# Fierykev/RayTraceBVH

Measured on AMD Instinct MI355X. Metric: Mrays/s primary+1-bounce (BASELINE.json's metric, on its config C5: 3840x2160, the 1/2/4/8-GPU config; the metric's @1080p config C3 is the line c3_1080p); BVH build Mtris/s under build, higher is better.
Workload: dtype f32; 1 GPU; C5: synthetic 10M tris (seed 0x5EED0005, box 100x100x50), 3840x2160, primary+1 bounce; width=3840, height=2160, bounces=1, triangles=10000000, parallelism=single GPU

## Files before the change

include/rtbvh.h:

```cpp
#ifndef RTBVH_H
#define RTBVH_H

#include <stddef.h>
#include <stdint.h>

#ifdef __cplusplus
extern "C" {
#endif

#define RTBVH_ABI_VERSION 8

typedef enum {
    RTBVH_OK = 0,
    RTBVH_ERR_INVALID_ARG = 1,
    RTBVH_ERR_HIP = 2,
    RTBVH_ERR_OOM = 3,
    RTBVH_ERR_NOT_READY = 4,
    RTBVH_ERR_STACK_OVERFLOW = 5,
    RTBVH_ERR_IO = 6,
    RTBVH_ERR_NO_DEVICE = 7,
    RTBVH_ERR_COMM = 8
} rtbvh_status;


// ... 7 lines not shown
    float ambient[4];
    float diffuse[4];
    float specular[4];
    float shininess;
    float optical_density;
    float alpha;
    uint32_t specularb;
    int32_t tex_num;
} rtbvh_material;

typedef struct {
    uint32_t parent, child_l, child_r, code;
    float bb_min[3], bb_max[3];
    uint32_t index;
} rtbvh_node;

typedef struct {
    float intensity;
    float origin[3], direction[3], inv_direction[3];
    float color[4];
} rtbvh_ray_present;

typedef struct {
    uint32_t width, height;
    const uint8_t* rgba8;
} rtbvh_texture;

enum {
    RTBVH_MORTON_CPUTESTS = 0,
    RTBVH_MORTON_HLSL = 1
};
enum {
    RTBVH_DELTA_CLZ64 = 0,
    RTBVH_DELTA_CPUTESTS = 1
};
enum {
    RTBVH_FLAG_TIMING = 1u << 0,
    RTBVH_FLAG_COUNT_VISITS = 1u << 1,
    RTBVH_FLAG_REFRACT_RECORDS = 1u << 2,
    RTBVH_FLAG_SORT_BOUNCE = 1u << 3,
    RTBVH_FLAG_NEAREST_FIRST = 1u << 4,
    RTBVH_FLAG_PACKET_PRIMARY = 1u << 5,
    RTBVH_FLAG_REFILL_BOUNCE = 1u << 6,
    RTBVH_FLAG_WIDE_BVH = 1u << 7,
    RTBVH_FLAG_AUTO_WALK = 1u << 8,
    RTBVH_FLAG_BINNED_PRIMARY = 1u << 9,
    RTBVH_FLAG_CERTIFIED = 1u << 10,
    RTBVH_FLAG_MULTI_KERNEL_BUILD = 1u << 16,
    RTBVH_FLAG_SPLIT_SHIFT = 17,
    RTBVH_FLAG_GRAPH = 1u << 20
};

typedef struct {
    int32_t device;
    uint32_t morton_mode;
    uint32_t delta_mode;
    uint32_t flags;
    float scene_bb_min[3];
    float scene_bb_max[3];
    void* stream;
    uint32_t stack_limit;
    uint32_t reserved;
} rtbvh_config;

typedef struct {
    uint32_t num_tris, num_nodes, width, height;
    uint64_t primary_rays, bounce_rays;
    uint64_t internal_visits[2], leaf_visits[2], hits[2];
    uint64_t textured_hits, stack_overflows;
    uint32_t timed_builds, timed_traces;
    float ms_build, ms_trace;
    float ms_stage[8];
    uint64_t trav_wave_steps, trav_mixed_steps, trav_active_lanes;
    uint64_t trav_max_steps, trav_steps_log2[32];
    uint64_t graph_captures;
    uint32_t walk_flags;
    uint32_t walk_state;
    uint64_t packet_steps[2];
    uint64_t cert_traces, redo_total;
    uint64_t bin_entries[2];
    uint64_t redo_rays[2];
    uint64_t trav_longest;
    uint64_t redo_deferred;
} rtbvh_stats;
typedef struct rtbvh_ctx rtbvh_ctx;

void rtbvh_config_default(rtbvh_config* cfg);
rtbvh_status rtbvh_create(const rtbvh_config* cfg, rtbvh_ctx** out);
void rtbvh_destroy(rtbvh_ctx* ctx);
const char* rtbvh_last_error(const rtbvh_ctx* ctx);
int rtbvh_abi_version(void);
uint32_t rtbvh_stats_size(void);

rtbvh_status rtbvh_set_scene(rtbvh_ctx* ctx, const rtbvh_vertex* verts, uint32_t nverts,
                             const uint32_t* indices, uint32_t nidx, const uint32_t* mat_idx,
                             const rtbvh_material* mats, uint32_t nmats,
                             const rtbvh_texture* textures, uint32_t ntex);
rtbvh_status rtbvh_set_camera(rtbvh_ctx* ctx, const float wvp[16], const float wv[16]);

rtbvh_status rtbvh_build(rtbvh_ctx* ctx);
rtbvh_status rtbvh_build_async(rtbvh_ctx* ctx);
rtbvh_status rtbvh_trace(rtbvh_ctx* ctx, uint32_t width, uint32_t height, uint32_t bounces);
rtbvh_status rtbvh_trace_async(rtbvh_ctx* ctx, uint32_t width, uint32_t height, uint32_t bounces);
rtbvh_status rtbvh_compute_bvh(rtbvh_ctx* ctx, uint32_t width, uint32_t height, uint32_t bounces);
rtbvh_status rtbvh_trace_band_async(rtbvh_ctx* ctx, uint32_t width, uint32_t height, uint32_t bounces,
                                    uint32_t rank, uint32_t nranks, float* dev_out, void* stream);
uint32_t rtbvh_band_rows(uint32_t height, uint32_t rank, uint32_t nranks);
uint32_t rtbvh_deal_bands(uint32_t height, uint32_t rank, uint32_t nranks, uint32_t root_share, uint32_t* bands,
                          uint32_t capacity);
uint32_t rtbvh_deal_rows(uint32_t height, uint32_t rank, uint32_t nranks, uint32_t root_share);
rtbvh_status rtbvh_set_band_deal(rtbvh_ctx* ctx, uint32_t root_share);
rtbvh_status rtbvh_verify_walk(rtbvh_ctx* ctx, uint32_t width, uint32_t height, uint32_t bounces,
                               uint64_t* differing_pixels);
rtbvh_status rtbvh_assemble_bands(rtbvh_ctx* ctx, uint32_t width, uint32_t height, uint32_t nranks,
                                  const float* dev_bands, uint32_t stride_rows, float* dev_frame, void* stream);

#define RTBVH_COMM_ID_BYTES 128
rtbvh_status rtbvh_comm_unique_id(uint8_t id[RTBVH_COMM_ID_BYTES]);
rtbvh_status rtbvh_comm_init(rtbvh_ctx* ctx, uint32_t nranks, uint32_t rank, const uint8_t id[RTBVH_COMM_ID_BYTES],
                             void** comm);
rtbvh_status rtbvh_comm_destroy(void* comm);
rtbvh_status rtbvh_trace_tiles(rtbvh_ctx* ctx, uint32_t width, uint32_t height, uint32_t bounces, uint32_t rank,
                               uint32_t nranks, void* comm);
rtbvh_status rtbvh_synchronize(rtbvh_ctx* ctx);

rtbvh_status rtbvh_update_vertices_async(rtbvh_ctx* ctx, const float* dev_positions, uint32_t pos_stride,
                                         const float* dev_normals, uint32_t nrm_stride,
                                         uint32_t first, uint32_t count, void* stream);
rtbvh_status rtbvh_update_vertices_host(rtbvh_ctx* ctx, const float* positions, uint32_t pos_stride,
                                        const float* normals, uint32_t nrm_stride,
                                        uint32_t first, uint32_t count);
rtbvh_status rtbvh_refit_async(rtbvh_ctx* ctx);
rtbvh_status rtbvh_refit(rtbvh_ctx* ctx);

typedef struct {
    float origin[3];
    float t_max;
    float direction[3];
    uint32_t reserved;
} rtbvh_ray;
typedef struct {
    float t, u, v;
    uint32_t tri;
} rtbvh_hit;
enum {
    RTBVH_QUERY_CLOSEST = 0,
    RTBVH_QUERY_ANY = 1u << 0,
    RTBVH_QUERY_SORT = 1u << 1,
    RTBVH_QUERY_COUNT = 1u << 2,
    RTBVH_QUERY_CERTIFIED = 1u << 8
};
rtbvh_status rtbvh_query_async(rtbvh_ctx* ctx, const rtbvh_ray* dev_rays, uint64_t n, rtbvh_hit* dev_hits,
                               uint32_t mode, void* stream);
rtbvh_status rtbvh_query_host(rtbvh_ctx* ctx, const rtbvh_ray* rays, uint64_t n, rtbvh_hit* hits, uint32_t mode);
rtbvh_status rtbvh_query_counts(rtbvh_ctx* ctx, uint64_t out[4]);
rtbvh_status rtbvh_query_walk_counts(rtbvh_ctx* ctx, uint64_t out[4]);

typedef struct {
    float point[3];
    float max_dist2;
} rtbvh_point;
typedef struct {
    float point[3];
    float dist2;
    float u, v;
    uint32_t tri;
// ... 58 lines not shown
                               rtbvh_hit* dev_hits, uint32_t mode, void* stream);
rtbvh_status rtbvh_khits_host(rtbvh_ctx* ctx, const rtbvh_ray* rays, uint64_t n, uint32_t k, rtbvh_hit* hits,
                              uint32_t mode);
rtbvh_status rtbvh_khits_counts(rtbvh_ctx* ctx, uint64_t out[4]);

enum {
    RTBVH_COLLIDE_COUNT = 1u << 2,
    RTBVH_COLLIDE_TRIANGLE = 1u << 3,
    RTBVH_COLLIDE_SIZES = 1u << 4,
    RTBVH_COLLIDE_FILL = 1u << 5,
    RTBVH_COLLIDE_SYMMETRIC = 1u << 6
};
rtbvh_status rtbvh_collide_async(rtbvh_ctx* ctx, uint64_t* dev_offsets, uint32_t* dev_ids, uint64_t capacity,
                                 uint32_t mode, void* stream);
rtbvh_status rtbvh_collide_host(rtbvh_ctx* ctx, uint64_t* offsets, uint32_t* ids, uint64_t capacity, uint32_t mode);
rtbvh_status rtbvh_collide_counts(rtbvh_ctx* ctx, uint64_t out[4]);

typedef struct {
    float v0[3];
    uint32_t reserved0;
    float v1[3];
    uint32_t reserved1;
    float v2[3];
    uint32_t reserved2;
} rtbvh_tri;
enum {
    RTBVH_CROSS_SORT = 1u << 1,
    RTBVH_CROSS_COUNT = 1u << 2,
    RTBVH_CROSS_SIZES = 1u << 4,
    RTBVH_CROSS_FILL = 1u << 5
};
rtbvh_status rtbvh_cross_async(rtbvh_ctx* ctx, const rtbvh_tri* dev_tris, uint64_t n, uint64_t* dev_offsets,
                               uint32_t* dev_ids, uint64_t capacity, uint32_t mode, void* stream);
rtbvh_status rtbvh_cross_host(rtbvh_ctx* ctx, const rtbvh_tri* tris, uint64_t n, uint64_t* offsets, uint32_t* ids,
                              uint64_t capacity, uint32_t mode);
rtbvh_status rtbvh_cross_first_async(rtbvh_ctx* ctx, const rtbvh_tri* dev_tris, uint64_t n, uint32_t* dev_first,
                                     uint32_t mode, void* stream);
rtbvh_status rtbvh_cross_first_host(rtbvh_ctx* ctx, const rtbvh_tri* tris, uint64_t n, uint32_t* first,
                                    uint32_t mode);
rtbvh_status rtbvh_cross_counts(rtbvh_ctx* ctx, uint64_t out[4]);

typedef struct {
    float lo[3];
    uint32_t reserved0;
    float hi[3];
    uint32_t reserved1;
} rtbvh_box;
enum {
    RTBVH_OVERLAP_SORT = 1u << 1,
    RTBVH_OVERLAP_COUNT = 1u << 2,
    RTBVH_OVERLAP_TRIANGLE = 1u << 3,
    RTBVH_OVERLAP_SIZES = 1u << 4,
    RTBVH_OVERLAP_FILL = 1u << 5
};
rtbvh_status rtbvh_overlap_async(rtbvh_ctx* ctx, const rtbvh_box* dev_boxes, uint64_t n, uint64_t* dev_offsets,
                                 uint32_t* dev_ids, uint64_t capacity, uint32_t mode, void* stream);
rtbvh_status rtbvh_overlap_host(rtbvh_ctx* ctx, const rtbvh_box* boxes, uint64_t n, uint64_t* offsets,
                                uint32_t* ids, uint64_t capacity, uint32_t mode);
rtbvh_status rtbvh_overlap_counts(rtbvh_ctx* ctx, uint64_t out[4]);

typedef struct {
    float point[3]; float dist2;
    float u, v; uint32_t tri;
    uint32_t flags;
} rtbvh_signed;
enum { RTBVH_SIGNED_SORT = 1u << 1, RTBVH_SIGNED_COUNT = 1u << 2,
       RTBVH_SIGNED_VOTE3 = 1u << 3,
       RTBVH_SIGNED_INSIDE_ONLY = 1u << 4
        };
rtbvh_status rtbvh_signed_async(rtbvh_ctx* ctx, const rtbvh_point* dev_points, uint64_t n, rtbvh_signed* dev_out,
                                uint32_t mode, void* stream);
rtbvh_status rtbvh_signed_host(rtbvh_ctx* ctx, const rtbvh_point* points, uint64_t n, rtbvh_signed* out,
                               uint32_t mode);
rtbvh_status rtbvh_signed_counts(rtbvh_ctx* ctx, uint64_t out[4]);

rtbvh_status rtbvh_read_framebuffer(rtbvh_ctx* ctx, float* rgba);
rtbvh_status rtbvh_read_intensity(rtbvh_ctx* ctx, float* intensity);
rtbvh_status rtbvh_present(rtbvh_ctx* ctx, uint8_t* rgba8);
rtbvh_status rtbvh_save_bmp(const char* path, const uint8_t* rgba8, uint32_t width, uint32_t height);
const float* rtbvh_framebuffer_device(rtbvh_ctx* ctx);
rtbvh_status rtbvh_read_bvh(rtbvh_ctx* ctx, rtbvh_node* out, uint32_t capacity);
rtbvh_status rtbvh_read_wide(rtbvh_ctx* ctx, uint32_t* records, uint64_t capacity);
rtbvh_status rtbvh_read_qnodes(rtbvh_ctx* ctx, uint32_t* nodes, uint64_t capacity);
rtbvh_status rtbvh_read_morton(rtbvh_ctx* ctx, uint32_t* codes);
rtbvh_status rtbvh_read_sorted(rtbvh_ctx* ctx, uint32_t* sorted_codes, uint32_t* tri_ids);
rtbvh_status rtbvh_read_rays(rtbvh_ctx* ctx, rtbvh_ray_present* reflect_out, rtbvh_ray_present* refract_out);
rtbvh_status rtbvh_get_stats(rtbvh_ctx* ctx, rtbvh_stats* out);
rtbvh_status rtbvh_reset_stats(rtbvh_ctx* ctx);
rtbvh_status rtbvh_set_flags(rtbvh_ctx* ctx, uint32_t flags);
uint64_t rtbvh_bin_builds(rtbvh_ctx* ctx);
uint32_t rtbvh_bin_sets(rtbvh_ctx* ctx);

rtbvh_status rtbvh_sort_pairs_async(rtbvh_ctx* ctx, uint32_t* keys_in, uint32_t* vals_in,
                                    uint32_t* keys_out, uint32_t* vals_out, uint32_t n,
                                    uint32_t key_bits);
rtbvh_status rtbvh_sort_pairs_host(rtbvh_ctx* ctx, const uint32_t* keys, const uint32_t* vals,
                                   uint32_t* keys_out, uint32_t* vals_out, uint32_t n, uint32_t key_bits);
rtbvh_status rtbvh_build_from_codes(rtbvh_ctx* ctx, const uint32_t* sorted_codes,
                                    const float* leaf_boxes, uint32_t n, rtbvh_node* out);

rtbvh_status rtbvh_texture_load_bmp(const char* path, rtbvh_texture* out);
rtbvh_status rtbvh_texture_load_jpeg(const char* path, rtbvh_texture* out);
rtbvh_status rtbvh_texture_decode_jpeg(const uint8_t* data, size_t size, rtbvh_texture* out);
rtbvh_status rtbvh_texture_load(const char* path, rtbvh_texture* out);
void rtbvh_texture_free(rtbvh_texture* tex);
void rtbvh_srgb_table(float out[256]);
typedef struct rtbvh_scene rtbvh_scene;
rtbvh_status rtbvh_scene_load_obj(const char* path, rtbvh_scene** out);
rtbvh_status rtbvh_scene_synthetic(uint64_t seed, uint32_t ntris, const float half_extent[3],
                                   rtbvh_scene** out);
void rtbvh_scene_free(rtbvh_scene* s);
uint32_t rtbvh_scene_num_vertices(const rtbvh_scene* s);
uint32_t rtbvh_scene_num_indices(const rtbvh_scene* s);
uint32_t rtbvh_scene_num_materials(const rtbvh_scene* s);
uint32_t rtbvh_scene_num_textures(const rtbvh_scene* s);
const rtbvh_vertex* rtbvh_scene_vertices(const rtbvh_scene* s);
const uint32_t* rtbvh_scene_indices(const rtbvh_scene* s);
const uint32_t* rtbvh_scene_mat_indices(const rtbvh_scene* s);
const rtbvh_material* rtbvh_scene_materials(const rtbvh_scene* s);
const char* rtbvh_scene_texture_path(const rtbvh_scene* s, uint32_t k);
rtbvh_status rtbvh_set_scene_obj(rtbvh_ctx* ctx, const rtbvh_scene* s, const rtbvh_texture* textures,
                                 uint32_t ntex);
void rtbvh_camera_reference(uint32_t width, uint32_t height, float wvp[16], float wv[16]);
void rtbvh_camera_look(const float eye[3], uint32_t width, uint32_t height, float wvp[16], float wv[16]);
void rtbvh_camera_orbit(float eye[3], uint32_t key);

#ifdef __cplusplus
}
#endif
#endif
```

raytracebvh_amd/_lib.py:

```python
from __future__ import annotations

import ctypes
import os

import numpy as np

HERE = os.path.dirname(os.path.abspath(__file__))
LIB_PATH = os.environ.get("RTBVH_LIB") or os.path.join(HERE, "librtbvh.so")

OK, ERR_INVALID_ARG, ERR_HIP, ERR_OOM, ERR_NOT_READY, ERR_STACK_OVERFLOW, ERR_IO, ERR_NO_DEVICE = range(8)
MORTON_CPUTESTS, MORTON_HLSL = 0, 1
DELTA_CLZ64, DELTA_CPUTESTS = 0, 1
FLAG_TIMING, FLAG_COUNT_VISITS, FLAG_REFRACT_RECORDS, FLAG_SORT_BOUNCE, FLAG_NEAREST_FIRST = 1, 2, 4, 8, 16
FLAG_PACKET_PRIMARY = 1 << 5
FLAG_REFILL_BOUNCE = 1 << 6
FLAG_WIDE_BVH = 1 << 7
FLAG_BINNED_PRIMARY = 1 << 9
FLAG_CERTIFIED = 1 << 10
FLAG_MULTI_KERNEL_BUILD = 1 << 16
FLAG_AUTO_WALK = 1 << 8
FLAG_SPLIT_SHIFT = 17
FLAG_GRAPH = 1 << 20

EXPORTS = [
    "rtbvh_config_default", "rtbvh_create", "rtbvh_destroy", "rtbvh_last_error", "rtbvh_abi_version", "rtbvh_stats_size",
    "rtbvh_set_scene", "rtbvh_set_camera", "rtbvh_build", "rtbvh_build_async", "rtbvh_trace",
    "rtbvh_trace_async", "rtbvh_compute_bvh", "rtbvh_trace_band_async", "rtbvh_band_rows", "rtbvh_verify_walk",
    "rtbvh_deal_bands", "rtbvh_deal_rows", "rtbvh_set_band_deal",
    "rtbvh_synchronize", "rtbvh_read_framebuffer", "rtbvh_read_intensity", "rtbvh_framebuffer_device",
    "rtbvh_read_bvh", "rtbvh_read_wide", "rtbvh_read_qnodes", "rtbvh_read_morton", "rtbvh_read_sorted", "rtbvh_read_rays", "rtbvh_get_stats",
    "rtbvh_reset_stats", "rtbvh_set_flags", "rtbvh_bin_builds", "rtbvh_bin_sets",
    "rtbvh_sort_pairs_async", "rtbvh_sort_pairs_host", "rtbvh_build_from_codes", "rtbvh_scene_load_obj",
    "rtbvh_scene_synthetic", "rtbvh_scene_free", "rtbvh_scene_num_vertices", "rtbvh_scene_num_indices",
    "rtbvh_scene_num_materials", "rtbvh_scene_num_textures", "rtbvh_scene_vertices", "rtbvh_scene_indices",
    "rtbvh_scene_mat_indices", "rtbvh_scene_materials", "rtbvh_scene_texture_path", "rtbvh_set_scene_obj",
    "rtbvh_camera_reference", "rtbvh_camera_look", "rtbvh_camera_orbit", "rtbvh_texture_load_bmp", "rtbvh_texture_load_jpeg", "rtbvh_texture_decode_jpeg",
    "rtbvh_texture_load", "rtbvh_texture_free", "rtbvh_srgb_table",
    "rtbvh_present", "rtbvh_save_bmp", "rtbvh_assemble_bands", "rtbvh_comm_unique_id", "rtbvh_comm_init",
    "rtbvh_comm_destroy", "rtbvh_trace_tiles",
    "rtbvh_query_async", "rtbvh_query_host", "rtbvh_query_counts", "rtbvh_query_walk_counts",
    "rtbvh_nearest_async", "rtbvh_nearest_host", "rtbvh_nearest_counts",
    "rtbvh_within_async", "rtbvh_within_host", "rtbvh_within_counts",
    "rtbvh_knn_async", "rtbvh_knn_host", "rtbvh_knn_counts",
    "rtbvh_allhits_async", "rtbvh_allhits_host", "rtbvh_allhits_counts",
    "rtbvh_overlap_async", "rtbvh_overlap_host", "rtbvh_overlap_counts",
    "rtbvh_signed_async", "rtbvh_signed_host", "rtbvh_signed_counts",
    "rtbvh_khits_async", "rtbvh_khits_host", "rtbvh_khits_counts",
    "rtbvh_collide_async", "rtbvh_collide_host", "rtbvh_collide_counts",
    "rtbvh_cross_async", "rtbvh_cross_host", "rtbvh_cross_first_async", "rtbvh_cross_first_host", "rtbvh_cross_counts",
    "rtbvh_update_vertices_async", "rtbvh_update_vertices_host", "rtbvh_refit_async", "rtbvh_refit",
]
COMM_ID_BYTES = 128

NODE_DTYPE = np.dtype([("parent", "<u4"), ("child_l", "<u4"), ("child_r", "<u4"), ("code", "<u4"),
                       ("bb_min", "<f4", (3,)), ("bb_max", "<f4", (3,)), ("index", "<u4")])
MATERIAL_DTYPE = np.dtype([("ambient", "<f4", (4,)), ("diffuse", "<f4", (4,)), ("specular", "<f4", (4,)),
                           ("shininess", "<f4"), ("optical_density", "<f4"), ("alpha", "<f4"),
                           ("specularb", "<u4"), ("tex_num", "<i4")])
assert NODE_DTYPE.itemsize == 44 and MATERIAL_DTYPE.itemsize == 68
RAY_DTYPE = np.dtype([("origin", "<f4", (3,)), ("t_max", "<f4"), ("direction", "<f4", (3,)), ("reserved", "<u4")])
HIT_DTYPE = np.dtype([("t", "<f4"), ("u", "<f4"), ("v", "<f4"), ("tri", "<u4")])
assert RAY_DTYPE.itemsize == 32 and HIT_DTYPE.itemsize == 16
QUERY_CLOSEST, QUERY_ANY, QUERY_SORT, QUERY_COUNT = 0, 1, 2, 4
QUERY_CERTIFIED = 1 << 8
POINT_DTYPE = np.dtype([("point", "<f4", (3,)), ("max_dist2", "<f4")])
NEAREST_DTYPE = np.dtype([("point", "<f4", (3,)), ("dist2", "<f4"), ("u", "<f4"), ("v", "<f4"), ("tri", "<u4"),
                          ("reserved", "<u4")])
assert POINT_DTYPE.itemsize == 16 and NEAREST_DTYPE.itemsize == 32
NEAREST_SORT, NEAREST_COUNT = 2, 4
PAIR_DTYPE = np.dtype([("tri", "<u4"), ("dist2", "<f4")])
assert PAIR_DTYPE.itemsize == 8
WITHIN_SORT, WITHIN_COUNT, WITHIN_SIZES, WITHIN_FILL = 2, 4, 16, 32
KNN_SORT, KNN_COUNT = 2, 4
KNN_MAX_K = 32
ALLHITS_SORT, ALLHITS_COUNT, ALLHITS_BY_T, ALLHITS_SIZES, ALLHITS_FILL = 2, 4, 8, 16, 32
BOX_DTYPE = np.dtype([("lo", "<f4", (3,)), ("reserved0", "<u4"), ("hi", "<f4", (3,)), ("reserved1", "<u4")])
assert BOX_DTYPE.itemsize == 32
OVERLAP_SORT, OVERLAP_COUNT, OVERLAP_TRIANGLE, OVERLAP_SIZES, OVERLAP_FILL = 2, 4, 8, 16, 32
SIGNED_DTYPE = np.dtype([("point", "<f4", (3,)), ("dist2", "<f4"), ("u", "<f4"), ("v", "<f4"), ("tri", "<u4"),
                         ("flags", "<u4")])
assert SIGNED_DTYPE.itemsize == 32
SIGNED_SORT, SIGNED_COUNT, SIGNED_VOTE3, SIGNED_INSIDE_ONLY = 2, 4, 8, 16
KHITS_SORT, KHITS_COUNT = 2, 4
KHITS_MAX_K = 16
COLLIDE_COUNT, COLLIDE_TRIANGLE, COLLIDE_SIZES, COLLIDE_FILL, COLLIDE_SYMMETRIC = 4, 8, 16, 32, 64
TRI_DTYPE = np.dtype([("v0", "<f4", (3,)), ("reserved0", "<u4"), ("v1", "<f4", (3,)), ("reserved1", "<u4"),
                      ("v2", "<f4", (3,)), ("reserved2", "<u4")])
assert TRI_DTYPE.itemsize == 48
CROSS_SORT, CROSS_COUNT, CROSS_SIZES, CROSS_FILL = 2, 4, 16, 32


class Config(ctypes.Structure):
    _fields_ = [("device", ctypes.c_int32), ("morton_mode", ctypes.c_uint32), ("delta_mode", ctypes.c_uint32),
                ("flags", ctypes.c_uint32), ("scene_bb_min", ctypes.c_float * 3),
                ("scene_bb_max", ctypes.c_float * 3), ("stream", ctypes.c_void_p),
                ("stack_limit", ctypes.c_uint32), ("reserved", ctypes.c_uint32)]


class Ray(ctypes.Structure):
    _fields_ = [("origin", ctypes.c_float * 3), ("t_max", ctypes.c_float), ("direction", ctypes.c_float * 3),
                ("reserved", ctypes.c_uint32)]


class Hit(ctypes.Structure):
    _fields_ = [("t", ctypes.c_float), ("u", ctypes.c_float), ("v", ctypes.c_float), ("tri", ctypes.c_uint32)]


class Point(ctypes.Structure):
    _fields_ = [("point", ctypes.c_float * 3), ("max_dist2", ctypes.c_float)]


class Nearest(ctypes.Structure):
    _fields_ = [("point", ctypes.c_float * 3), ("dist2", ctypes.c_float), ("u", ctypes.c_float), ("v", ctypes.c_float),
                ("tri", ctypes.c_uint32), ("reserved", ctypes.c_uint32)]


class Texture(ctypes.Structure):
    _fields_ = [("width", ctypes.c_uint32), ("height", ctypes.c_uint32), ("rgba8", ctypes.c_void_p)]


class Stats(ctypes.Structure):
    _fields_ = [("num_tris", ctypes.c_uint32), ("num_nodes", ctypes.c_uint32), ("width", ctypes.c_uint32),
                ("height", ctypes.c_uint32), ("primary_rays", ctypes.c_uint64), ("bounce_rays", ctypes.c_uint64),
                ("internal_visits", ctypes.c_uint64 * 2), ("leaf_visits", ctypes.c_uint64 * 2),
                ("hits", ctypes.c_uint64 * 2), ("textured_hits", ctypes.c_uint64),
                ("stack_overflows", ctypes.c_uint64), ("timed_builds", ctypes.c_uint32),
                ("timed_traces", ctypes.c_uint32), ("ms_build", ctypes.c_float), ("ms_trace", ctypes.c_float),
                ("ms_stage", ctypes.c_float * 8), ("trav_wave_steps", ctypes.c_uint64),
                ("trav_mixed_steps", ctypes.c_uint64), ("trav_active_lanes", ctypes.c_uint64),
                ("trav_max_steps", ctypes.c_uint64), ("trav_steps_log2", ctypes.c_uint64 * 32),
                ("graph_captures", ctypes.c_uint64), ("walk_flags", ctypes.c_uint32),
                ("walk_state", ctypes.c_uint32), ("packet_steps", ctypes.c_uint64 * 2),
                ("cert_traces", ctypes.c_uint64), ("redo_total", ctypes.c_uint64),
                ("bin_entries", ctypes.c_uint64 * 2), ("redo_rays", ctypes.c_uint64 * 2),
                ("trav_longest", ctypes.c_uint64), ("redo_deferred", ctypes.c_uint64)]

    def as_dict(self) -> dict:
        d = {}
        for k, _ in self._fields_:
            v = getattr(self, k)
            d[k] = list(v) if hasattr(v, "__len__") else v
        return d


class RtbvhError(RuntimeError):
    def __init__(self, status: int, msg: str):
        super().__init__(f"rtbvh status {status}: {msg}")
        self.status = status


_lib = None


def lib() -> ctypes.CDLL:
    global _lib
    if _lib is not None:
        return _lib
    if not os.path.exists(LIB_PATH):
        raise ImportError(f"{LIB_PATH} is not built: run `python -c 'import __graft_entry__ as g; g.build()'` "
                          "(there is no CPU fallback for the HIP path)")
    try:
        import torch
    except ImportError:
        pass
    L = ctypes.CDLL(LIB_PATH)
    vp, u32, u64, i32 = ctypes.c_void_p, ctypes.c_uint32, ctypes.c_uint64, ctypes.c_int
    sig = {
        "rtbvh_config_default": (None, [ctypes.POINTER(Config)]),
        "rtbvh_create": (i32, [ctypes.POINTER(Config), ctypes.POINTER(vp)]),
        "rtbvh_destroy": (None, [vp]),
        "rtbvh_last_error": (ctypes.c_char_p, [vp]),
        "rtbvh_abi_version": (i32, []),
        "rtbvh_stats_size": (ctypes.c_uint32, []),
        "rtbvh_set_scene": (i32, [vp, vp, u32, vp, u32, vp, vp, u32, vp, u32]),
        "rtbvh_set_camera": (i32, [vp, vp, vp]),
        "rtbvh_build": (i32, [vp]),
        "rtbvh_build_async": (i32, [vp]),
        "rtbvh_trace": (i32, [vp, u32, u32, u32]),
        "rtbvh_trace_async": (i32, [vp, u32, u32, u32]),
        "rtbvh_compute_bvh": (i32, [vp, u32, u32, u32]),
        "rtbvh_trace_band_async": (i32, [vp, u32, u32, u32, u32, u32, vp, vp]),
        "rtbvh_band_rows": (u32, [u32, u32, u32]),
        "rtbvh_deal_bands": (u32, [u32, u32, u32, u32, vp, u32]),
        "rtbvh_deal_rows": (u32, [u32, u32, u32, u32]),
        "rtbvh_set_band_deal": (i32, [vp, u32]),
        "rtbvh_verify_walk": (i32, [vp, u32, u32, u32, ctypes.POINTER(u64)]),
        "rtbvh_assemble_bands": (i32, [vp, u32, u32, u32, vp, u32, vp, vp]),
        "rtbvh_comm_unique_id": (i32, [vp]),
        "rtbvh_comm_init": (i32, [vp, u32, u32, vp, ctypes.POINTER(vp)]),
        "rtbvh_comm_destroy": (i32, [vp]),
        "rtbvh_trace_tiles": (i32, [vp, u32, u32, u32, u32, u32, vp]),
        "rtbvh_synchronize": (i32, [vp]),
        "rtbvh_read_framebuffer": (i32, [vp, vp]),
        "rtbvh_read_intensity": (i32, [vp, vp]),
        "rtbvh_framebuffer_device": (vp, [vp]),
        "rtbvh_read_bvh": (i32, [vp, vp, u32]),
        "rtbvh_read_morton": (i32, [vp, vp]),
        "rtbvh_read_wide": (i32, [vp, vp, ctypes.c_uint64]),
        "rtbvh_read_qnodes": (i32, [vp, vp, ctypes.c_uint64]),
        "rtbvh_read_sorted": (i32, [vp, vp, vp]),
        "rtbvh_read_rays": (i32, [vp, vp, vp]),
        "rtbvh_get_stats": (i32, [vp, ctypes.POINTER(Stats)]),
        "rtbvh_reset_stats": (i32, [vp]),
        "rtbvh_set_flags": (i32, [vp, u32]),
        "rtbvh_bin_builds": (u64, [vp]),
        "rtbvh_bin_sets": (u32, [vp]),
        "rtbvh_sort_pairs_async": (i32, [vp, vp, vp, vp, vp, u32, u32]),
        "rtbvh_sort_pairs_host": (i32, [vp, vp, vp, vp, vp, u32, u32]),
        "rtbvh_build_from_codes": (i32, [vp, vp, vp, u32, vp]),
        "rtbvh_scene_load_obj": (i32, [ctypes.c_char_p, ctypes.POINTER(vp)]),
        "rtbvh_scene_synthetic": (i32, [u64, u32, vp, ctypes.POINTER(vp)]),
        "rtbvh_scene_free": (None, [vp]),
        "rtbvh_scene_num_vertices": (u32, [vp]),
        "rtbvh_scene_num_indices": (u32, [vp]),
        "rtbvh_scene_num_materials": (u32, [vp]),
        "rtbvh_scene_num_textures": (u32, [vp]),
        "rtbvh_scene_vertices": (vp, [vp]),
        "rtbvh_scene_indices": (vp, [vp]),
        "rtbvh_scene_mat_indices": (vp, [vp]),
        "rtbvh_scene_materials": (vp, [vp]),
        "rtbvh_scene_texture_path": (ctypes.c_char_p, [vp, u32]),
        "rtbvh_set_scene_obj": (i32, [vp, vp, vp, u32]),
        "rtbvh_camera_reference": (None, [u32, u32, vp, vp]),
        "rtbvh_camera_look": (None, [vp, u32, u32, vp, vp]),
        "rtbvh_camera_orbit": (None, [vp, u32]),
        "rtbvh_texture_load_bmp": (i32, [ctypes.c_char_p, vp]),
        "rtbvh_texture_load_jpeg": (i32, [ctypes.c_char_p, vp]),
        "rtbvh_texture_decode_jpeg": (i32, [vp, ctypes.c_size_t, vp]),
        "rtbvh_texture_load": (i32, [ctypes.c_char_p, vp]),
        "rtbvh_texture_free": (None, [vp]),
        "rtbvh_srgb_table": (None, [vp]),
        "rtbvh_present": (i32, [vp, vp]),
        "rtbvh_save_bmp": (i32, [ctypes.c_char_p, vp, u32, u32]),
        "rtbvh_query_async": (i32, [vp, vp, u64, vp, u32, vp]),
        "rtbvh_query_host": (i32, [vp, vp, u64, vp, u32]),
        "rtbvh_query_counts": (i32, [vp, vp]),
        "rtbvh_query_walk_counts": (i32, [vp, vp]),
        "rtbvh_nearest_async": (i32, [vp, vp, u64, vp, u32, vp]),
        "rtbvh_nearest_host": (i32, [vp, vp, u64, vp, u32]),
        "rtbvh_nearest_counts": (i32, [vp, vp]),
        "rtbvh_within_async": (i32, [vp, vp, u64, vp, vp, u64, u32, vp]),
        "rtbvh_within_host": (i32, [vp, vp, u64, vp, vp, u64, u32]),
        "rtbvh_within_counts": (i32, [vp, vp]),
        "rtbvh_knn_async": (i32, [vp, vp, u64, u32, vp, u32, vp]),
        "rtbvh_knn_host": (i32, [vp, vp, u64, u32, vp, u32]),
        "rtbvh_knn_counts": (i32, [vp, vp]),
        "rtbvh_signed_async": (i32, [vp, vp, u64, vp, u32, vp]),
        "rtbvh_signed_host": (i32, [vp, vp, u64, vp, u32]),
        "rtbvh_signed_counts": (i32, [vp, vp]),
        "rtbvh_khits_async": (i32, [vp, vp, u64, u32, vp, u32, vp]),
        "rtbvh_khits_host": (i32, [vp, vp, u64, u32, vp, u32]),
        "rtbvh_khits_counts": (i32, [vp, vp]),
        "rtbvh_allhits_async": (i32, [vp, vp, u64, vp, vp, u64, u32, vp]),
        "rtbvh_allhits_host": (i32, [vp, vp, u64, vp, vp, u64, u32]),
        "rtbvh_allhits_counts": (i32, [vp, vp]),
        "rtbvh_overlap_async": (i32, [vp, vp, u64, vp, vp, u64, u32, vp]),
        "rtbvh_overlap_host": (i32, [vp, vp, u64, vp, vp, u64, u32]),
        "rtbvh_overlap_counts": (i32, [vp, vp]),
        "rtbvh_collide_async": (i32, [vp, vp, vp, u64, u32, vp]),
        "rtbvh_collide_host": (i32, [vp, vp, vp, u64, u32]),
        "rtbvh_collide_counts": (i32, [vp, vp]),
        "rtbvh_cross_async": (i32, [vp, vp, u64, vp, vp, u64, u32, vp]),
        "rtbvh_cross_host": (i32, [vp, vp, u64, vp, vp, u64, u32]),
        "rtbvh_cross_first_async": (i32, [vp, vp, u64, vp, u32, vp]),
        "rtbvh_cross_first_host": (i32, [vp, vp, u64, vp, u32]),
        "rtbvh_cross_counts": (i32, [vp, vp]),
        "rtbvh_update_vertices_async": (i32, [vp, vp, u32, vp, u32, u32, u32, vp]),
        "rtbvh_update_vertices_host": (i32, [vp, vp, u32, vp, u32, u32, u32]),
        "rtbvh_refit_async": (i32, [vp]),
        "rtbvh_refit": (i32, [vp]),
    }
    for name, (res, args) in sig.items():
        f = getattr(L, name)
        f.restype = res
        f.argtypes = args
    _lib = L
    return L


def ptr(a: np.ndarray):
    if a is None:
        return None
# ... 9 lines not shown
```

raytracebvh_amd/csrc/api.hip:

```cpp
#include <dlfcn.h>
#include <rccl/rccl.h>

#include <algorithm>
#include <cstdio>
#include <cstring>
#include <deque>
#include <new>
#include <string>
#include <type_traits>
#include <utility>
#include <vector>

#include "../../include/rtbvh.h"
#include "rtbvh_internal.h"

using namespace rtbvh;

#ifndef RTBVH_MAXSPLIT
#define RTBVH_MAXSPLIT 4
#endif

template <typename H, void (*Del)(H)>
struct Owner {
    H h{};
// ... 92 lines not shown
    DevBuf<float2> hit;
    Grown<uint32_t> redo, defer;
    PbBufs pb;
    Grown<unsigned long long> pbkeys;
    uint32_t* qcount = nullptr;
    uint32_t* next = nullptr;
    unsigned long long* counters = nullptr;
    unsigned long long* ovf = nullptr;
};

struct LastTrace {
    bool traced = false;
    uint32_t W = 0, H = 0, bounces = 0, rank = 0, nranks = 1;
    uint32_t nsplit = 1;
    uint32_t slot = 0;
    size_t rec_P = 0;
    uint32_t walk = 0;
    uint32_t walk_state = 0;
    bool cert = false;
    bool frame_here = false;
    bool intensity_here = false;
};

struct rtbvh_ctx {
    rtbvh_config cfg{};
    Stream own_stream, side;
    static constexpr uint32_t MAXSPLIT = RTBVH_MAXSPLIT;
    TraceSet sets[MAXSPLIT];
    hipStream_t stream = nullptr;
    std::string err;

    uint32_t V = 0, T = 0, nmat = 0;
    DevBuf<float4> d_opos;
    DevBuf<float> d_verts;
    DevBuf<uint32_t> d_idx, d_matidx;
    DevBuf<Mat> d_mats;
    float wvp[16], wv[16];
    DevBuf<float> d_cam;
    bool cam_dirty = false;
    bool have_scene = false, have_camera = false;
    Tree tree;
    Event ev_update;
    bool update_pending = false;
    bool stale = false;

    uint32_t cap_T = 0;
    DevBuf<uint32_t> d_codes, d_ids, d_ka, d_va, d_kb, d_vb, d_sort_scratch;
    DevBuf<float4> d_tclip, d_leaf;
    Grown<float4> d_band;
    DevBuf<Inner> d_inner;
    DevBuf<uint4> d_topo;
    DevBuf<Inner> d_rec;
    DevBuf<QNode> d_qnode;
    DevBuf<uint4> d_lfp;
    DevBuf<uint32_t> d_texels;
    DevBuf<uint4> d_texinfo;
    DevBuf<float> d_srgb;
    uint32_t ntex = 0;
    Grown<float> d_refl_rec;
    Grown<float> d_refr_rec;
    DevBuf<uint32_t> d_pleaf, d_pint, d_cnt;
    DevBuf<uint32_t> d_xlist, d_xcnt;
    DevBuf<uint32_t> d_qlate;
    DevBuf<unsigned long long> d_ovf;
    Pinned<unsigned long long> h_ovf;
    unsigned long long ovf_seen = 0;
    DevBuf<float> d_bounds, d_rootbox, d_zpart;
    Event ev_leaf, ev_prim;
    DevBuf<float> d_nbox;
    bool tail_pending = false;
    bool leaf_pending = false;
    SortResult sorted{nullptr, nullptr};

    size_t cap_P = 0;
    DevBuf<float4> d_color;
    DevBuf<float> d_intensity;
    DevBuf<uint32_t> d_bkin, d_bvin, d_bka, d_bva, d_bkb, d_bvb, d_bscratch;
    DevBuf<uint32_t> d_qcount;
    DevBuf<uint32_t> d_next;
    DevBuf<unsigned long long> d_counters;
    size_t cap_split = 0;
    Event ev_fork;
    uint64_t bins_epoch = 1;
    uint64_t bin_builds = 0;
    bool knob_bins_reuse = true;
    LastTrace last;

    static constexpr int RING = 32;
    Event evb[RING][6];
    Event evt[RING][5];
    bool evt_trav[RING] = {};
    uint32_t n_builds = 0, n_traces = 0;
    Event ev_built;
    bool slots_used = false;
    hipGraph_t graph = nullptr;
    hipGraphExec_t graph_exec = nullptr;
    uint64_t graph_key[5] = {};
    bool capturing = false;
    uint64_t graph_captures = 0;
    LastTrace graph_trace;
    Tree graph_tree;
    uint64_t cert_traces = 0;
    uint64_t small_key = 0;
    uint32_t small_flags = 0;
    bool small_packet = false;
    Event ev_small[2];
    uint32_t knob_bounce_blocks = 0;
    bool knob_overlap = false, knob_side_priority = true, knob_keep_records = false, knob_no_early_shade = false,
         knob_no_small_tiles = false;
    uint32_t root_share = 16;
    struct DealTab {
        uint32_t H, nranks, share;
        DevBuf<uint32_t> d;
        std::vector<uint32_t> off;
        Pinned<uint32_t> h;
        Event ready;
    };
    std::deque<DealTab> deals;
    static constexpr size_t MAX_DEALS = 8;
    DevBuf<uint32_t> d_qscratch;
    Grown<uint32_t> d_qsort;
    Grown<uint32_t> d_qsort_scratch;
    Grown<uint32_t> d_qredo;
    Grown<unsigned long long> d_qscan;
    Grown<uint32_t> d_qorder;
    Event ev_query;
    bool query_busy = false;
    bool query_ovf = false;
    bool query_counted = false;
    uint64_t query_fallback = 0;
    bool nearest_counted = false;
    bool within_counted = false;
    bool allhits_counted = false;
    bool overlap_counted = false;
    bool knn_counted = false;
    bool signed_counted = false;
    bool khits_counted = false;
    bool collide_counted = false;
    bool cross_counted = false;
};

namespace {

std::string g_create_error;

rtbvh_status fail(rtbvh_ctx* c, rtbvh_status st, const std::string& msg) {
    if (c) c->err = msg;
    else g_create_error = msg;
    return st;
}

#define HIPC(ctx, expr)                                                                          \
    do {                                                                                         \
        hipError_t _e = (expr);                                                                  \
        if (_e != hipSuccess)                                                                    \
            return fail(ctx, _e == hipErrorOutOfMemory ? RTBVH_ERR_OOM : RTBVH_ERR_HIP,          \
                        std::string(#expr) + ": " + hipGetErrorString(_e));                      \
    } while (0)
#define TRY(expr)                                      \
    do {                                               \
        if (rtbvh_status _st = (expr)) return _st;     \
    } while (0)

void drop_graph(rtbvh_ctx* c) {
    if (c->graph_exec) (void)hipGraphExecDestroy(c->graph_exec);
    if (c->graph) (void)hipGraphDestroy(c->graph);
// ... 399 lines not shown
struct Rccl {
    bool ok = false;
    std::string err;
    ncclResult_t (*GetUniqueId)(ncclUniqueId*) = nullptr;
    ncclResult_t (*CommInitRank)(ncclComm_t*, int, ncclUniqueId, int) = nullptr;
    ncclResult_t (*CommDestroy)(ncclComm_t) = nullptr;
    ncclResult_t (*Send)(const void*, size_t, ncclDataType_t, int, ncclComm_t, hipStream_t) = nullptr;
    ncclResult_t (*Recv)(void*, size_t, ncclDataType_t, int, ncclComm_t, hipStream_t) = nullptr;
    ncclResult_t (*GroupStart)() = nullptr;
    ncclResult_t (*GroupEnd)() = nullptr;
    const char* (*GetErrorString)(ncclResult_t) = nullptr;
};
const Rccl& rccl() {
    static const Rccl lib = [] {
        Rccl r;
        void* h = dlopen("librccl.so.1", RTLD_NOW | RTLD_GLOBAL);
        if (!h) {
            const char* e = dlerror();
            r.err = std::string("RCCL not available: ") + (e ? e : "dlopen(librccl.so.1) failed");
            return r;
        }
        bool all = true;
        auto sym = [&](auto& f, const char* name) {
            f = reinterpret_cast<std::remove_reference_t<decltype(f)>>(dlsym(h, name));
            if (!f) all = false;
        };
        sym(r.GetUniqueId, "ncclGetUniqueId");
        sym(r.CommInitRank, "ncclCommInitRank");
        sym(r.CommDestroy, "ncclCommDestroy");
        sym(r.Send, "ncclSend");
        sym(r.Recv, "ncclRecv");
        sym(r.GroupStart, "ncclGroupStart");
        sym(r.GroupEnd, "ncclGroupEnd");
        sym(r.GetErrorString, "ncclGetErrorString");
        r.ok = all;
        if (!all) r.err = "RCCL: librccl.so.1 lacks a required symbol";
        return r;
    }();
    return lib;
}

rtbvh_status sync_camera(rtbvh_ctx* c, hipStream_t s) {
    if (!c->cam_dirty) return RTBVH_OK;
    TRY(wait_slots(c, c->stream));
    launch_set_camera(c->wvp, c->wv, c->d_cam, c->stream);
    HIPC(c, hipGetLastError());
    c->cam_dirty = false;
    return order_after_context(c, s);
}

rtbvh_status before_tree_write(rtbvh_ctx* c, hipStream_t s) {
    TRY(wait_slots(c, s));
    TRY(wait_queries(c, s));
    TRY(wait_update(c, s));
    TRY(sync_camera(c, s));
    c->bins_epoch++;
    return RTBVH_OK;
}

struct TailGuard {
    rtbvh_ctx* c;
    bool pending;
    void run() {
        if (pending) launch_refit_tail(build_args(c), c->stream);
        pending = false;
    }
    ~TailGuard() { run(); }
};

struct WalkPlan {
    hipStream_t s;
    uint32_t slot, bounces;
    bool cert;
    bool leaf_pending;
    bool count, timing, records;
    Walks wk;
    PrimaryKind pkind;
    Form nodes;
    uint32_t P, rows;
    uint32_t nsplit, Pg;
    uint32_t tblocks;
    uint32_t ntx, nty;
    bool inflight, fuse_tail, overlap, small_tiles, early_shade;
    uint32_t bset;
    bool fill_bins;
};

WalkPlan plan_walks(const rtbvh_ctx* c, const TraceArgs& a, uint32_t bounces, hipStream_t s, uint32_t slot,
                    uint32_t flags, bool cert, bool timed, bool tail_pending, bool leaf_pending) {
    WalkPlan p{s, slot, bounces, cert, leaf_pending};
    p.bset = slot;
    p.count = (c->cfg.flags & RTBVH_FLAG_COUNT_VISITS) != 0;
    p.timing = timed && (c->cfg.flags & RTBVH_FLAG_TIMING) != 0 && s == c->stream && !c->capturing;
    p.wk = choose_walks(flags);
    p.records = (flags & RTBVH_FLAG_REFRACT_RECORDS) != 0;
    p.P = a.W * deal_rows(a.H, a.rank, a.nranks, c->root_share);
    p.rows = p.P / a.W;
#ifndef RTBVH_BOUNCE_GRID
#define RTBVH_BOUNCE_GRID (256 * BOUNCE_WAVES)
#endif
    p.inflight = slot != 0;
    for (uint32_t k = 1; k < rtbvh_ctx::MAXSPLIT && !p.inflight && !c->capturing; k++)
        p.inflight = c->sets[k].busy && hipEventQuery(c->sets[k].done) == hipErrorNotReady;
    p.tblocks = p.P < (1u << 22) ? (!p.inflight ? 1536 : p.P < (3u << 20) ? 512 : 1024) : RTBVH_BOUNCE_GRID;
    if (c->knob_bounce_blocks) p.tblocks = c->knob_bounce_blocks;
    const bool binned = p.wk.primary == PrimaryKind::BINNED;
    p.pkind = binned && (a.W > 32768u || a.H > 32768u)
                  ? (cert ? PrimaryKind::LANE_REFERENCE : PrimaryKind::PACKET_WIDE)
                  : p.wk.primary;
    p.nsplit = trace_split(c);
    if (p.wk.sort || a.my_bands < p.nsplit || slot || c->slots_used || binned) p.nsplit = 1;
    p.Pg = p.nsplit == 1 ? p.P : a.W * 8 * ((a.my_bands + p.nsplit - 1) / p.nsplit);
    p.nodes = cert ? NBOX : RECORDS;
    p.fuse_tail = tail_pending && p.pkind == PrimaryKind::BINNED && s == c->stream && slot == 0 && p.rows > 0 &&
                  (c->tree.valid & p.nodes);
    p.overlap = p.pkind == PrimaryKind::BINNED && leaf_pending && s == c->stream && slot == 0 && p.nsplit == 1;
    p.ntx = pb_tiles_x(a.W);
    p.nty = pb_tiles_y(p.rows);
    p.small_tiles = !p.inflight && !c->knob_no_small_tiles && (size_t)a.W * p.rows < (3u << 19);
    p.early_shade = cert && !p.inflight && !c->knob_no_early_shade;
    return p;
}

rtbvh_status prepare_walks(rtbvh_ctx* c, WalkPlan& p, TraceArgs& a, const rtbvh_ctx::DealTab* deal, TailGuard& tail) {
    hipStream_t s = p.s;
    TraceSet& mine = c->sets[p.slot];
    const size_t P = p.P;
    if (p.records) {
        if (!(c->d_refl_rec.has(14 * P) && c->d_refr_rec.has(14 * P))) {
            drop_graph(c);
            HIPC(c, c->d_refl_rec.reserve(14 * P));
            HIPC(c, c->d_refr_rec.reserve(14 * P));
        }
        a.refl_rec = c->d_refl_rec;
        a.refr_rec = c->d_refr_rec;
    }
    if (!p.fuse_tail && tail.pending) {
        tail.run();
        TRY(order_after_context(c, s));
    }
    TRY(ensure_form(c, p.nodes, s));
    a.nb = p.cert;
    TRY(ensure_split_capacity(c, p.slot ? p.slot + 1 : p.nsplit, p.Pg));
    if (p.bounces > 0 && p.wk.refill && p.wk.bounce == BounceWalk::WIDE_QUANTIZED) TRY(ensure_form(c, QNODES, s));
    if (p.pkind == PrimaryKind::PACKET_REFERENCE || p.pkind == PrimaryKind::PACKET_NEAREST ||
        p.pkind == PrimaryKind::PACKET_WIDE)
        TRY(ensure_form(c, PSEUDO, s));
    if (p.cert && p.bounces > 0 && !mine.defer.has(P)) {
        drop_graph(c);
        HIPC(c, mine.defer.reserve(P));
        if (hipMemsetAsync(mine.defer, 0, sizeof(uint32_t) * P, c->stream) != hipSuccess) {
            mine.defer.reset();
            return fail(c, RTBVH_ERR_HIP, "clearing the deferred-ray list failed");
        }
        TRY(order_after_context(c, s));
    }
    if (p.cert && !mine.redo.has(P)) {
        drop_graph(c);
        HIPC(c, mine.redo.reserve(P));
    }
    if (p.pkind != PrimaryKind::BINNED || p.rows == 0) return RTBVH_OK;
    const size_t px = (size_t)a.W * p.rows;
    if (pb_keys_used() && !mine.pbkeys.has(px)) {
        drop_graph(c);
        HIPC(c, mine.pbkeys.reserve(px));
    }
// ... 25 lines not shown
    return RTBVH_OK;
}

rtbvh_status launch_walks(rtbvh_ctx* c, const WalkPlan& p, const TraceArgs& a, TailGuard& tail) {
    hipStream_t s = p.s;
    TraceSet& mine = c->sets[p.slot];
    const uint32_t bounces = p.bounces, nsplit = p.nsplit;
    const bool count = p.count, cert = p.cert, refill = p.wk.refill;
    Event* ev = c->evt[c->n_traces % rtbvh_ctx::RING];
    ZeroList z{};
    z.ptr[0] = reinterpret_cast<uint32_t*>(mine.counters);
    z.words[0] = 64 * 2;
    z.ptr[1] = mine.qcount;
    z.words[1] = 32 * nsplit;
    if (refill && bounces) {
        z.ptr[2] = mine.next;
        z.words[2] = (size_t)NEXT_WORDS * nsplit;
    }
    if (p.fill_bins) {
        z.ptr[3] = mine.pb.off;
        z.words[3] = (size_t)p.ntx * p.nty * PB_NZ + 1;
        if (a.nranks > 1) {
            z.ptr[4] = mine.pb.list;
            z.words[4] = (size_t)PB_LISTS * PB_LIST_STRIDE;
        }
    }
    hipStream_t sp = s;
    if (p.overlap) {
        sp = c->side;
        HIPC(c, hipStreamWaitEvent(sp, c->ev_leaf, 0));
    }
    launch_zero(z, sp);
    if (p.timing) HIPC(c, hipEventRecord(ev[0], sp));
    if (nsplit > 1) HIPC(c, hipEventRecord(c->ev_fork, s));
    for (uint32_t g = 0; g < nsplit; g++) {
        TraceSet& set = c->sets[p.slot + g];
        hipStream_t sg = g ? set.chain : s;
        if (g) HIPC(c, hipStreamWaitEvent(sg, c->ev_fork, 0));
        TraceArgs ag = a;
        ag.band0 = g;
        ag.bstep = nsplit;
        ag.pb_list = p.fill_bins && a.nranks > 1 ? mine.pb.list : nullptr;
        RayQ* q[2] = {set.q[0], set.q[1]};
        uint32_t* qc = set.qcount;
        const bool tg = p.timing && g == 0;
        if (p.pkind == PrimaryKind::BINNED) {
            PbBufs& pbb = c->sets[p.bset].pb;
            const PrimBins pb{pbb.off, pbb.cur, pbb.bins, mine.pbkeys, pbb.sums, pbb.cap_bins, p.ntx, p.nty};
            if (p.rows) {
                const BuildArgs ba = build_args(c);
                const Redo rd{mine.redo, &qc[16]};
                if (p.fill_bins) {
                    launch_pb_bins(ag, pb, p.rows, true, sp, p.fuse_tail ? &ba : nullptr);
                    c->bin_builds++;
                    if (c->knob_bins_reuse && !c->capturing) {
                        if (!pbb.filled) HIPC(c, hipEventCreateWithFlags(pbb.filled.out(), hipEventDisableTiming));
                        HIPC(c, hipEventRecord(pbb.filled, sp));
                        pbb.valid = true;
                    }
                }
                launch_pb_raster(ag, pb, p.rows, q[0], &qc[0], count, bounces > 0, sp, cert ? &rd : nullptr,
                                 p.small_tiles);
                if (p.fuse_tail) tail.pending = false;
            }
            if (p.overlap) {
                HIPC(c, hipEventRecord(c->ev_prim, sp));
                HIPC(c, hipStreamWaitEvent(sg, c->ev_prim, 0));
            }
            if (p.rows) launch_pb_gate(ag, pb, q[0], &qc[0], count, bounces > 0, sg, cert);
        } else
            launch_primary(ag, q[0], &qc[0], count, bounces > 0, p.pkind, sg);
        if (tg) HIPC(c, hipEventRecord(ev[1], sg));
        for (uint32_t b = 0; b < bounces; b++) {
            const uint32_t* perm = nullptr;
            if (p.wk.sort) {
                launch_bounce_keys(q[b & 1], &qc[b], c->d_rootbox, p.P, c->d_bkin, c->d_bvin, sg);
                perm = radix_sort_pairs(c->d_bkin, c->d_bvin, c->d_bka, c->d_bva, c->d_bkb, c->d_bvb, p.P, 30,
                                        c->d_bscratch, sg).vals;
            }
            if (refill) {
                if (tg && b == 0) HIPC(c, hipEventRecord(ev[3], sg));
                uint32_t* nxb = set.next + (size_t)NEXT_SEGS * NEXT_STRIDE * b;
                const BounceShade es{q[(b + 1) & 1], &qc[b + 1], b + 1 < bounces, mine.redo, &qc[17 + b], p.Pg};
                launch_bounce_traverse(ag, q[b & 1], &qc[b], perm, count, p.wk.bounce, set.hit, nxb, p.tblocks, sg, cert,
                                       mine.defer, p.early_shade ? &es : nullptr);
                if (tg && b == 0) HIPC(c, hipEventRecord(ev[4], sg));
                const Redo rd{mine.redo, &qc[17 + b], mine.defer, nxb};
                launch_bounce_shade(ag, q[b & 1], &qc[b], set.hit, q[(b + 1) & 1], &qc[b + 1], count, b + 1 < bounces,
                                    p.Pg, sg, cert ? &rd : nullptr);
            } else
                launch_bounce(ag, q[b & 1], &qc[b], perm, q[(b + 1) & 1], &qc[b + 1], count, b + 1 < bounces,
                              p.wk.nearest, sg);
        }
        if (g) {
            HIPC(c, hipEventRecord(set.join, sg));
            HIPC(c, hipStreamWaitEvent(s, set.join, 0));
        }
    }
    HIPC(c, hipMemcpyAsync(mine.ovf, c->d_ovf, sizeof(unsigned long long), hipMemcpyDeviceToHost, s));
    if (p.timing) {
        HIPC(c, hipEventRecord(ev[2], s));
        c->evt_trav[c->n_traces % rtbvh_ctx::RING] = refill && bounces > 0;
        c->n_traces++;
    }
    return RTBVH_OK;
}

rtbvh_status enqueue_walks(rtbvh_ctx* c, uint32_t W, uint32_t H, uint32_t bounces, uint32_t rank, uint32_t nranks,
                           float4* color, float* inten, hipStream_t s, uint32_t slot, uint32_t flags, bool timed,
                           uint32_t walk_state, bool cert = false) {
    const bool leaf_pending = c->leaf_pending;
    c->leaf_pending = false;
    TailGuard tail{c, c->tail_pending};
    c->tail_pending = false;
    if (!c->tree.built) return fail(c, RTBVH_ERR_NOT_READY, "trace before build");
    if (c->stale) return fail_stale(c, "trace");
    if (W == 0 || H == 0 || nranks == 0 || rank >= nranks || bounces > 14)
        return fail(c, RTBVH_ERR_INVALID_ARG, "bad trace dimensions");
    TRY(ensure_trace_capacity(c, (size_t)W * H));
    if (!color) color = c->d_color;
    TraceArgs a = trace_args(c, W, H, rank, nranks, color, inten);
    const rtbvh_ctx::DealTab* deal = nullptr;
    TRY(get_deal(c, H, nranks, &deal, s));
    if (deal) {
        a.my_bands = deal->off[rank + 1] - deal->off[rank];
        a.band_list = deal->d + deal->off[rank];
        a.band_slots = deal->d + (H + 7) / 8;
    }
    a.counters = c->sets[slot].counters;
    if ((flags & RTBVH_FLAG_REFRACT_RECORDS) && slot)
        return fail(c, RTBVH_ERR_INVALID_ARG, "ray records are traced on the context stream only");
    WalkPlan p = plan_walks(c, a, bounces, s, slot, flags, cert, timed, tail.pending, leaf_pending);
    TRY(prepare_walks(c, p, a, deal, tail));
    TRY(launch_walks(c, p, a, tail));
    const bool frame_here = color == c->d_color && nranks == 1;
    c->last = LastTrace{true, W, H, bounces, rank, nranks, p.nsplit, slot, p.records ? p.P : 0, flags & WALK_FLAGS,
                        walk_state, cert, frame_here, frame_here && inten != nullptr};
    return check_launch(c, "trace kernels");
}

struct TracePlan {
    uint32_t flags;
    bool cert;
    uint32_t state;
};
TracePlan plan_trace(const rtbvh_ctx* c, uint32_t f) {
    if (!(f & (RTBVH_FLAG_AUTO_WALK | RTBVH_FLAG_CERTIFIED))) return TracePlan{f, false, 0};
    const uint32_t ref = f & ~WALK_FLAGS;
    const bool limited = c->cfg.stack_limit != 0 && c->cfg.stack_limit < (uint32_t)STACK_SIZE;
    const bool want = (f & RTBVH_FLAG_CERTIFIED) || auto_checked(c);
    if (!want || !c->tree.clz64 || limited) return TracePlan{ref, false, 0};
    return TracePlan{ref | RTBVH_FLAG_NEAREST_FIRST | RTBVH_FLAG_REFILL_BOUNCE | RTBVH_FLAG_WIDE_BVH |
                         RTBVH_FLAG_BINNED_PRIMARY,
                     true, 2};
}

rtbvh_status enqueue_trace(rtbvh_ctx* c, uint32_t W, uint32_t H, uint32_t bounces, uint32_t rank, uint32_t nranks,
                           float4* color, float* inten, hipStream_t s, uint32_t slot = 0) {
    if (!c->tree.built) return fail(c, RTBVH_ERR_NOT_READY, "trace before build");
    if (c->stale) return fail_stale(c, "trace");
    TRY(sync_camera(c, s));
    TracePlan p = plan_trace(c, c->cfg.flags);
    if (p.cert && !c->capturing) c->cert_traces++;
    const uint32_t f = c->cfg.flags;
    const bool limited = c->cfg.stack_limit != 0 && c->cfg.stack_limit < (uint32_t)STACK_SIZE;
    if ((f & RTBVH_FLAG_AUTO_WALK) && !p.cert && c->tree.clz64 && !limited) {
        const uint64_t key = (uint64_t)W << 48 | (uint64_t)H << 32 | c->T;
        const uint32_t fw = f & (WALK_FLAGS | RTBVH_FLAG_AUTO_WALK | RTBVH_FLAG_CERTIFIED | RTBVH_FLAG_SORT_BOUNCE);
        if ((c->small_key != key || c->small_flags != fw) && !c->capturing && s == c->stream && slot == 0 &&
            nranks == 1) {
            Event* ev = c->ev_small;
            for (int k = 0; k < 2; k++)
                if (!ev[k]) HIPC(c, hipEventCreate(ev[k].out()));
            float best[2] = {INFINITY, INFINITY};
            for (int round = 0; round < 2; round++)
                for (int k = 0; k < 2; k++) {
                    HIPC(c, hipEventRecord(ev[0], s));
                    TRY(enqueue_walks(c, W, H, 0, 0, 1, color, inten, s, 0,
                                      p.flags | (k ? RTBVH_FLAG_PACKET_PRIMARY : 0u), false, p.state));
                    HIPC(c, hipEventRecord(ev[1], s));
                    HIPC(c, hipEventSynchronize(ev[1]));
                    float ms = 0.f;
                    HIPC(c, hipEventElapsedTime(&ms, ev[0], ev[1]));
                    best[k] = std::min(best[k], ms);
                }
            c->small_packet = best[1] < 0.95f * best[0];
            c->small_key = key;
            c->small_flags = fw;
        }
        if (c->small_key == key && c->small_flags == fw && c->small_packet) p.flags |= RTBVH_FLAG_PACKET_PRIMARY;
    }
    return enqueue_walks(c, W, H, bounces, rank, nranks, color, inten, s, slot, p.flags, true, p.state, p.cert);
}

}

extern "C" {

int rtbvh_abi_version(void) { return RTBVH_ABI_VERSION; }
uint32_t rtbvh_stats_size(void) { return (uint32_t)sizeof(rtbvh_stats); }

void rtbvh_config_default(rtbvh_config* cfg) {
    if (!cfg) return;
    memset(cfg, 0, sizeof(*cfg));
    cfg->device = 0;
    cfg->morton_mode = RTBVH_MORTON_CPUTESTS;
    cfg->delta_mode = RTBVH_DELTA_CLZ64;
    for (int k = 0; k < 3; k++) {
        cfg->scene_bb_min[k] = -700.f;
        cfg->scene_bb_max[k] = 700.f;
    }
}

rtbvh_status rtbvh_create(const rtbvh_config* cfg, rtbvh_ctx** out) {
    if (!out) return fail(nullptr, RTBVH_ERR_INVALID_ARG, "out is NULL");
    *out = nullptr;
    rtbvh_ctx* c = new (std::nothrow) rtbvh_ctx();
    if (!c) return fail(nullptr, RTBVH_ERR_OOM, "host allocation failed");
    if (cfg) c->cfg = *cfg;
    else rtbvh_config_default(&c->cfg);
    if (c->cfg.morton_mode > 1 || c->cfg.delta_mode > 1 || c->cfg.reserved != 0) {
        delete c;
        return fail(nullptr, RTBVH_ERR_INVALID_ARG, "bad morton/delta mode");
    }
    int ndev = 0;
    if (hipGetDeviceCount(&ndev) != hipSuccess || ndev <= 0) {
        delete c;
        return fail(nullptr, RTBVH_ERR_NO_DEVICE, "no HIP device");
    }
    if (c->cfg.device < 0 || c->cfg.device >= ndev || hipSetDevice(c->cfg.device) != hipSuccess) {
        delete c;
        return fail(nullptr, RTBVH_ERR_NO_DEVICE, "bad device ordinal");
    }
    if (c->cfg.stream) {
        c->stream = (hipStream_t)c->cfg.stream;
    } else {
        if (hipStreamCreateWithFlags(c->own_stream.out(), hipStreamNonBlocking) != hipSuccess) {
            delete c;
            return fail(nullptr, RTBVH_ERR_HIP, "hipStreamCreate failed");
        }
        c->stream = c->own_stream;
    }
    bool ev_ok = true;
    for (auto& row : c->evb)
        for (auto& e : row) ev_ok = ev_ok && hipEventCreate(e.out()) == hipSuccess;
    for (auto& row : c->evt)
        for (auto& e : row) ev_ok = ev_ok && hipEventCreate(e.out()) == hipSuccess;
    if (!ev_ok) {
        rtbvh_destroy(c);
        return fail(nullptr, RTBVH_ERR_HIP, "hipEventCreate failed");
    }
    if (hipEventCreateWithFlags(c->ev_built.out(), hipEventDisableTiming) != hipSuccess) {
        rtbvh_destroy(c);
        return fail(nullptr, RTBVH_ERR_HIP, "hipEventCreate failed");
    }
    if (c->d_ovf.alloc(1) != hipSuccess || hipMemset(c->d_ovf, 0, sizeof(unsigned long long)) != hipSuccess ||
        c->h_ovf.alloc(rtbvh_ctx::MAXSPLIT) != hipSuccess) {
        rtbvh_destroy(c);
        return fail(nullptr, RTBVH_ERR_OOM, "overflow counter allocation failed");
    }
    memset(c->h_ovf, 0, sizeof(unsigned long long) * rtbvh_ctx::MAXSPLIT);
    for (uint32_t b = 0; b < rtbvh_ctx::MAXSPLIT; b++) c->sets[b].ovf = c->h_ovf + b;
    if (c->d_cam.alloc(32) != hipSuccess ||
        hipMemset(c->d_cam, 0, 32 * sizeof(float)) != hipSuccess) {
        rtbvh_destroy(c);
        return fail(nullptr, RTBVH_ERR_OOM, "camera buffer allocation failed");
    }
    if (const char* e = getenv("RTBVH_BOUNCE_BLOCKS")) c->knob_bounce_blocks = (uint32_t)std::max(0, atoi(e));
    if (const char* e = getenv("RTBVH_OVERLAP")) c->knob_overlap = atoi(e) != 0;
    if (const char* e = getenv("RTBVH_SIDE_PRIORITY")) c->knob_side_priority = atoi(e) != 0;
    if (const char* e = getenv("RTBVH_KEEP_RECORDS")) c->knob_keep_records = atoi(e) != 0;
    if (const char* e = getenv("RTBVH_EARLY_SHADE")) c->knob_no_early_shade = atoi(e) == 0;
    if (const char* e = getenv("RTBVH_PB_SMALL_TILES")) c->knob_no_small_tiles = atoi(e) == 0;
    if (const char* e = getenv("RTBVH_BINS_REUSE")) c->knob_bins_reuse = atoi(e) != 0;
    *out = c;
    return RTBVH_OK;
}

void rtbvh_destroy(rtbvh_ctx* c) {
    if (!c) return;
    (void)hipSetDevice(c->cfg.device);
    (void)sync_all(c);
    drop_graph(c);
    delete c;
}

const char* rtbvh_last_error(const rtbvh_ctx* c) { return c ? c->err.c_str() : g_create_error.c_str(); }

rtbvh_status rtbvh_set_scene(rtbvh_ctx* c, const rtbvh_vertex* verts, uint32_t nverts, const uint32_t* indices,
                             uint32_t nidx, const uint32_t* mat_idx, const rtbvh_material* mats, uint32_t nmats,
                             const rtbvh_texture* textures, uint32_t ntex) {
    if (!c) return RTBVH_ERR_INVALID_ARG;
    drop_graph(c);
    if (ntex && !textures) return fail(c, RTBVH_ERR_INVALID_ARG, "set_scene: ntex > 0 without textures");
    for (uint32_t k = 0; k < ntex; k++)
        if (textures[k].width == 0 || textures[k].height == 0 || !textures[k].rgba8)
            return fail(c, RTBVH_ERR_INVALID_ARG, "set_scene: empty texture");
    if (!verts || !indices || !mat_idx || !mats || nverts == 0 || nidx == 0 || nidx % 3 != 0 || nmats == 0)
        return fail(c, RTBVH_ERR_INVALID_ARG, "set_scene: empty or ragged input");
    const uint32_t T = nidx / 3;
    if (T >= (1u << 30)) return fail(c, RTBVH_ERR_INVALID_ARG, "set_scene: too many triangles");
    for (uint32_t i = 0; i < nidx; i++)
        if (indices[i] >= nverts) return fail(c, RTBVH_ERR_INVALID_ARG, "set_scene: index out of range");
    for (uint32_t t = 0; t < T; t++)
        if (mat_idx[t] >= nmats) return fail(c, RTBVH_ERR_INVALID_ARG, "set_scene: material index out of range");
    HIPC(c, hipSetDevice(c->cfg.device));
    TRY(sync_all(c));
    c->query_busy = false;
    reset_tree(c);
    try {
        std::vector<float4> opos(nverts);
        for (uint32_t i = 0; i < nverts; i++)
            opos[i] = make_float4(verts[i].position[0], verts[i].position[1], verts[i].position[2], 0.f);
        HIPC(c, c->d_opos.alloc(nverts));
        HIPC(c, c->d_verts.alloc((size_t)nverts * 8));
        HIPC(c, c->d_idx.alloc(nidx));
        HIPC(c, c->d_matidx.alloc(T));
        HIPC(c, c->d_mats.alloc(nmats));
        HIPC(c, hipMemcpy(c->d_opos, opos.data(), sizeof(float4) * nverts, hipMemcpyHostToDevice));
        HIPC(c, hipMemcpy(c->d_verts, verts, sizeof(rtbvh_vertex) * nverts, hipMemcpyHostToDevice));
        HIPC(c, hipMemcpy(c->d_idx, indices, sizeof(uint32_t) * nidx, hipMemcpyHostToDevice));
        HIPC(c, hipMemcpy(c->d_matidx, mat_idx, sizeof(uint32_t) * T, hipMemcpyHostToDevice));
        HIPC(c, hipMemcpy(c->d_mats, mats, sizeof(rtbvh_material) * nmats, hipMemcpyHostToDevice));
        std::vector<uint4> info(ntex ? ntex : 1);
        size_t total = 0;
        for (uint32_t k = 0; k < ntex; k++) {
            info[k] = make_uint4((uint32_t)total, textures[k].width, textures[k].height, 0u);
            total += (size_t)textures[k].width * textures[k].height;
        }
        if (total >= (1ull << 32)) return fail(c, RTBVH_ERR_INVALID_ARG, "set_scene: textures too large");
        HIPC(c, c->d_texels.alloc(total ? total : 1));
        HIPC(c, c->d_texinfo.alloc(info.size()));
        for (uint32_t k = 0; k < ntex; k++)
            HIPC(c, hipMemcpy(c->d_texels + info[k].x, textures[k].rgba8,
                              (size_t)textures[k].width * textures[k].height * 4, hipMemcpyHostToDevice));
        HIPC(c, hipMemcpy(c->d_texinfo, info.data(), sizeof(uint4) * info.size(), hipMemcpyHostToDevice));
        if (!c->d_srgb) {
            float tab[256];
            rtbvh_srgb_table(tab);
            HIPC(c, c->d_srgb.alloc(256));
            HIPC(c, hipMemcpy(c->d_srgb, tab, sizeof(tab), hipMemcpyHostToDevice));
        }
        c->ntex = ntex;
    } catch (const std::bad_alloc&) {
        return fail(c, RTBVH_ERR_OOM, "set_scene: host allocation failed");
    }
    static_assert(sizeof(rtbvh_material) == sizeof(Mat), "material layout");
    c->V = nverts;
    c->T = T;
    c->nmat = nmats;
    TRY(ensure_build_capacity(c, T));
    if (c->cfg.morton_mode == RTBVH_MORTON_CPUTESTS) {
        BuildArgs a = build_args(c);
        launch_bounds(a, c->stream);
        TRY(check_launch(c, "mesh bounds"));
        HIPC(c, hipStreamSynchronize(c->stream));
    }
// ... 37 lines not shown
        c->leaf_pending = false;
        c->tail_pending = false;
        if (timing) for (int k = 1; k <= 5; k++) HIPC(c, hipEventRecord(ev[k], s));
        if (timing) c->n_builds++;
        if (!c->capturing) HIPC(c, hipEventRecord(c->ev_built, s));
        c->tree = Tree{true, clz64, RECORDS, RECORDS | PSEUDO | (qnodes ? QNODES : 0u)};
        c->stale = false;
        return check_launch(c, "build kernel");
    }
    if (timing) HIPC(c, hipEventRecord(ev[1], s));
    const Form nodes = records_skipped(c) ? NBOX : RECORDS;
    a.rec_on = nodes == RECORDS ? 1u : 0u;
    a.nbox = nodes == NBOX ? c->d_nbox.h : nullptr;
    if (c->T <= small_sort_max() && !(c->cfg.flags & RTBVH_FLAG_MULTI_KERNEL_BUILD)) {
        c->sorted = SortResult{c->d_ka, c->d_va};
        a.sorted_keys = c->d_ka;
        a.sorted_vals = c->d_va;
        launch_morton_sort_small(a, s);
        if (timing) HIPC(c, hipEventRecord(ev[2], s));
    } else {
        launch_morton(a, s);
        if (timing) HIPC(c, hipEventRecord(ev[2], s));
        c->sorted = radix_sort_pairs(c->d_codes, c->d_ids, c->d_ka, c->d_va, c->d_kb, c->d_vb, c->T, 30,
                                     c->d_sort_scratch, s);
    }
    if (timing) HIPC(c, hipEventRecord(ev[3], s));
    a.sorted_keys = c->sorted.keys;
    a.sorted_vals = c->sorted.vals;
    launch_karras(a, s);
    if (timing) HIPC(c, hipEventRecord(ev[4], s));
    launch_refit_leaves(a, s);
    c->leaf_pending = false;
    if (handoff & LEAF_EVENT) {
        if (!c->side) {
            int lo = 0, hi = 0;
            HIPC(c, hipDeviceGetStreamPriorityRange(&lo, &hi));
            if (!c->knob_side_priority) hi = lo;
            HIPC(c, hipStreamCreateWithPriority(c->side.out(), hipStreamNonBlocking, hi));
        }
        if (!c->ev_leaf) HIPC(c, hipEventCreateWithFlags(c->ev_leaf.out(), hipEventDisableTiming));
        if (!c->ev_prim) HIPC(c, hipEventCreateWithFlags(c->ev_prim.out(), hipEventDisableTiming));
        HIPC(c, hipEventRecord(c->ev_leaf, s));
        c->leaf_pending = true;
    }
    if ((handoff & TAIL_TO_TRACE) && !c->leaf_pending) c->tail_pending = true;
    else launch_refit_tail(a, s);
    if (timing) HIPC(c, hipEventRecord(ev[5], s));
    if (timing) c->n_builds++;
    if (!c->capturing) HIPC(c, hipEventRecord(c->ev_built, s));
    c->tree = Tree{true, clz64, nodes, (uint32_t)nodes | (a.pseudo ? PSEUDO : 0u) | QNODES};
    c->stale = false;
    return check_launch(c, "build kernels");
}

rtbvh_status rtbvh_build_async(rtbvh_ctx* c) { return c ? build_tree(c, 0) : RTBVH_ERR_INVALID_ARG; }

rtbvh_status rtbvh_build(rtbvh_ctx* c) {
    TRY(rtbvh_build_async(c));
    return rtbvh_synchronize(c);
}

rtbvh_status rtbvh_trace_async(rtbvh_ctx* c, uint32_t W, uint32_t H, uint32_t bounces) {
    if (!c) return RTBVH_ERR_INVALID_ARG;
    HIPC(c, hipSetDevice(c->cfg.device));
    TRY(ensure_trace_capacity(c, (size_t)W * H));
    return enqueue_trace(c, W, H, bounces, 0, 1, c->d_color, c->d_intensity, c->stream);
}

rtbvh_status rtbvh_trace(rtbvh_ctx* c, uint32_t W, uint32_t H, uint32_t bounces) {
    TRY(rtbvh_trace_async(c, W, H, bounces));
    return rtbvh_synchronize(c);
}

static rtbvh_status flush_tail(rtbvh_ctx* c, rtbvh_status st) {
    if (c->tail_pending) {
        launch_refit_tail(build_args(c), c->stream);
        c->tail_pending = false;
    }
    return st;
}

static rtbvh_status enqueue_frame(rtbvh_ctx* c, uint32_t W, uint32_t H, uint32_t bounces) {
    rtbvh_status st = build_tree(c, TAIL_TO_TRACE | (c->knob_overlap ? LEAF_EVENT : 0u));
    if (!st) st = rtbvh_trace_async(c, W, H, bounces);
    return flush_tail(c, st);
}

static rtbvh_status compute_graph(rtbvh_ctx* c, uint32_t W, uint32_t H, uint32_t bounces) {
    const uint64_t key[5] = {W, H, bounces, (uint64_t)c->cfg.flags | (uint64_t)c->T << 32,
                             (uint64_t)c->slots_used | (uint64_t)c->cfg.stack_limit << 1};
    if (!c->graph_exec || memcmp(key, c->graph_key, sizeof(key)) != 0) {
        drop_graph(c);
        rtbvh_status st = enqueue_frame(c, W, H, bounces);
        if (!st) st = rtbvh_synchronize(c);
        if (st && st != RTBVH_ERR_STACK_OVERFLOW) return st;
        HIPC(c, hipStreamBeginCapture(c->stream, hipStreamCaptureModeThreadLocal));
        c->capturing = true;
        st = enqueue_frame(c, W, H, bounces);
        hipGraph_t g = nullptr;
        const hipError_t e = hipStreamEndCapture(c->stream, &g);
        c->capturing = false;
        if (st || e != hipSuccess) {
            if (g) (void)hipGraphDestroy(g);
            return st ? st : fail(c, RTBVH_ERR_HIP, std::string("hipStreamEndCapture: ") + hipGetErrorString(e));
        }
        c->graph = g;
        HIPC(c, hipGraphInstantiate(&c->graph_exec, g, nullptr, nullptr, 0));
        memcpy(c->graph_key, key, sizeof(key));
        c->graph_trace = c->last;
        c->graph_tree = c->tree;
        c->graph_captures++;
    }
    TRY(before_tree_write(c, c->stream));
    HIPC(c, hipGraphLaunch(c->graph_exec, c->stream));
    HIPC(c, hipEventRecord(c->ev_built, c->stream));
    c->tree = c->graph_tree;
    c->stale = false;
    c->last = c->graph_trace;
    if (c->last.cert) c->cert_traces++;
    return rtbvh_synchronize(c);
}

rtbvh_status rtbvh_compute_bvh(rtbvh_ctx* c, uint32_t W, uint32_t H, uint32_t bounces) {
    if (!c) return RTBVH_ERR_INVALID_ARG;
    if (c->cfg.flags & RTBVH_FLAG_GRAPH) return compute_graph(c, W, H, bounces);
    TRY(enqueue_frame(c, W, H, bounces));
    return rtbvh_synchronize(c);
}

static rtbvh_status check_update(rtbvh_ctx* c, const float* positions, uint32_t pos_stride, const float* normals,
                                 uint32_t nrm_stride, uint32_t first, uint32_t count) {
    if (!positions) return fail(c, RTBVH_ERR_INVALID_ARG, "update_vertices: NULL positions");
    if (pos_stride < 3 || (normals && nrm_stride < 3))
        return fail(c, RTBVH_ERR_INVALID_ARG, "update_vertices: a stride below 3 floats");
    if (!c->have_scene) return fail(c, RTBVH_ERR_NOT_READY, "update_vertices before set_scene");
    if (first > c->V || count > c->V - first)
        return fail(c, RTBVH_ERR_INVALID_ARG, "update_vertices: first + count exceeds the scene's vertices");
    return RTBVH_OK;
}

rtbvh_status rtbvh_update_vertices_async(rtbvh_ctx* c, const float* dev_positions, uint32_t pos_stride,
                                         const float* dev_normals, uint32_t nrm_stride, uint32_t first,
                                         uint32_t count, void* stream) {
    if (!c) return RTBVH_ERR_INVALID_ARG;
    if (count == 0) return RTBVH_OK;
    TRY(check_update(c, dev_positions, pos_stride, dev_normals, nrm_stride, first, count));
    HIPC(c, hipSetDevice(c->cfg.device));
    hipStream_t s = stream ? (hipStream_t)stream : c->stream;
    if (!c->ev_update) HIPC(c, hipEventCreateWithFlags(c->ev_update.out(), hipEventDisableTiming));
    TRY(wait_slots(c, s));
    TRY(order_after_context(c, s));
    TRY(wait_update(c, s));
    VertexUpdate u{};
    u.pos = dev_positions;
    u.pos_stride = pos_stride;
    u.nrm = dev_normals;
    u.nrm_stride = nrm_stride;
    u.first = first;
    u.count = count;
    u.opos = c->d_opos;
    u.verts = c->d_verts;
    u.bounds = c->cfg.morton_mode == RTBVH_MORTON_CPUTESTS ? c->d_bounds.h : nullptr;
    u.V = c->V;
    launch_update_vertices(u, s);
    const rtbvh_status st = check_launch(c, "vertex update");
    HIPC(c, hipEventRecord(c->ev_update, s));
    c->update_pending = true;
// ... 365 lines not shown

rtbvh_status rtbvh_get_stats(rtbvh_ctx* c, rtbvh_stats* out) {
    if (!c || !out) return RTBVH_ERR_INVALID_ARG;
    memset(out, 0, sizeof(*out));
    if (rtbvh_status st = sync_all(c)) return st;
    out->num_tris = c->T;
    out->num_nodes = c->T ? 2 * c->T - 1 : 0;
    const LastTrace& t = c->last;
    const TraceSet& set = c->sets[t.slot];
    out->width = t.W;
    out->height = t.H;
    const uint32_t nb = c->n_builds < (uint32_t)rtbvh_ctx::RING ? c->n_builds : rtbvh_ctx::RING;
    for (uint32_t k = 0; k < nb; k++) {
        float ms;
        HIPC(c, hipEventElapsedTime(&ms, c->evb[k][0], c->evb[k][5]));
        out->ms_build += ms / nb;
        for (int st = 0; st < 5; st++) {
            HIPC(c, hipEventElapsedTime(&ms, c->evb[k][st], c->evb[k][st + 1]));
            out->ms_stage[st] += ms / nb;
        }
    }
    out->timed_builds = nb;
    const uint32_t nt = c->n_traces < (uint32_t)rtbvh_ctx::RING ? c->n_traces : rtbvh_ctx::RING;
    for (uint32_t k = 0; k < nt; k++) {
        float ms;
        HIPC(c, hipEventElapsedTime(&ms, c->evt[k][0], c->evt[k][2]));
        out->ms_trace += ms / nt;
        HIPC(c, hipEventElapsedTime(&ms, c->evt[k][0], c->evt[k][1]));
        out->ms_stage[5] += ms / nt;
        HIPC(c, hipEventElapsedTime(&ms, c->evt[k][1], c->evt[k][2]));
        out->ms_stage[6] += ms / nt;
        if (c->evt_trav[k]) {
            HIPC(c, hipEventElapsedTime(&ms, c->evt[k][3], c->evt[k][4]));
            out->ms_stage[7] += ms / nt;
        }
    }
    out->timed_traces = nt;
    if (t.traced && set.counters) {
        unsigned long long cnt[64];
        uint32_t q[32 * rtbvh_ctx::MAXSPLIT];
        HIPC(c, hipMemcpy(cnt, set.counters, sizeof(cnt), hipMemcpyDeviceToHost));
        HIPC(c, hipMemcpy(q, set.qcount, sizeof(uint32_t) * 32 * t.nsplit, hipMemcpyDeviceToHost));
        out->primary_rays = (uint64_t)t.W * deal_rows(t.H, t.rank, t.nranks, c->root_share);
        uint64_t b = 0;
        for (uint32_t g = 0; g < t.nsplit; g++)
            for (uint32_t k = 0; k < t.bounces; k++) b += q[32 * g + k];
        out->bounce_rays = b;
        for (int p = 0; p < 2; p++) {
            out->internal_visits[p] = cnt[2 + 3 * p];
            out->leaf_visits[p] = cnt[3 + 3 * p];
            out->hits[p] = cnt[4 + 3 * p];
        }
        out->stack_overflows = cnt[8];
        out->textured_hits = cnt[9];
        out->trav_wave_steps = cnt[10];
        out->trav_max_steps = cnt[13];
        out->trav_longest = cnt[20];
        for (int k = 0; k < 32; k++) out->trav_steps_log2[k] = cnt[32 + k];
        out->trav_mixed_steps = cnt[11];
        out->trav_active_lanes = cnt[12];
        for (int p = 0; p < 2; p++) {
            out->packet_steps[p] = cnt[14 + p];
            out->bin_entries[p] = cnt[16 + p];
        }
    }
    out->graph_captures = c->graph_captures;
    out->walk_flags = t.walk;
    out->walk_state = t.walk_state;
    out->cert_traces = c->cert_traces;
    if (t.traced && t.cert && set.qcount) {
        uint32_t q[32];
        HIPC(c, hipMemcpy(q, set.qcount, sizeof(q), hipMemcpyDeviceToHost));
        out->redo_rays[0] = q[16];
        for (uint32_t k = 0; k < t.bounces && k < 15; k++) out->redo_rays[1] += q[17 + k];
        for (uint32_t k = 0; k < t.bounces && k < 15; k++) {
            uint32_t nd = 0;
            HIPC(c, hipMemcpy(&nd, set.next + (size_t)NEXT_SEGS * NEXT_STRIDE * k + DEFER_COUNT, sizeof(nd),
                              hipMemcpyDeviceToHost));
            out->redo_rays[1] += nd;
            out->redo_deferred += nd;
        }
    }
    out->redo_total = out->redo_rays[0] + out->redo_rays[1];
    return RTBVH_OK;
}

uint64_t rtbvh_bin_builds(rtbvh_ctx* c) { return c ? c->bin_builds : 0; }

uint32_t rtbvh_bin_sets(rtbvh_ctx* c) {
    uint32_t n = 0;
    for (uint32_t k = 0; c && k < rtbvh_ctx::MAXSPLIT; k++) n += c->sets[k].pb.bins ? 1u : 0u;
    return n;
}

rtbvh_status rtbvh_set_flags(rtbvh_ctx* c, uint32_t flags) {
    if (!c) return RTBVH_ERR_INVALID_ARG;
    c->cfg.flags = flags;
    return RTBVH_OK;
}

rtbvh_status rtbvh_reset_stats(rtbvh_ctx* c) {
    if (!c) return RTBVH_ERR_INVALID_ARG;
    HIPC(c, hipStreamSynchronize(c->stream));
    c->n_builds = 0;
    c->n_traces = 0;
    return RTBVH_OK;
}

rtbvh_status rtbvh_sort_pairs_async(rtbvh_ctx* c, uint32_t* kin, uint32_t* vin, uint32_t* kout, uint32_t* vout,
                                    uint32_t n, uint32_t key_bits) {
    if (!c || (n && (!kin || !vin || !kout || !vout)) || key_bits == 0 || key_bits > 32)
        return RTBVH_ERR_INVALID_ARG;
    if (n == 0) return RTBVH_OK;
    HIPC(c, hipSetDevice(c->cfg.device));
    const uint32_t passes = (key_bits + RADIX_BITS - 1) / RADIX_BITS;
    uint32_t *tk = nullptr, *tv = nullptr, *scratch = nullptr;
    HIPC(c, hipMallocAsync((void**)&scratch, sort_scratch_words(n) * 4, c->stream));
    if (passes > 1) {
        HIPC(c, hipMallocAsync((void**)&tk, (size_t)n * 4, c->stream));
        HIPC(c, hipMallocAsync((void**)&tv, (size_t)n * 4, c->stream));
    }
    if (passes & 1) radix_sort_pairs(kin, vin, kout, vout, tk, tv, n, key_bits, scratch, c->stream);
    else radix_sort_pairs(kin, vin, tk, tv, kout, vout, n, key_bits, scratch, c->stream);
    rtbvh_status st = check_launch(c, "sort kernels");
    (void)hipFreeAsync(scratch, c->stream);
    if (tk) (void)hipFreeAsync(tk, c->stream);
    if (tv) (void)hipFreeAsync(tv, c->stream);
    return st;
}

rtbvh_status rtbvh_sort_pairs_host(rtbvh_ctx* c, const uint32_t* keys, const uint32_t* vals, uint32_t* kout,
                                   uint32_t* vout, uint32_t n, uint32_t key_bits) {
    if (!c || (n && (!keys || !vals || !kout || !vout))) return RTBVH_ERR_INVALID_ARG;
    if (n == 0) return RTBVH_OK;
    HIPC(c, hipSetDevice(c->cfg.device));
    uint32_t* d = nullptr;
    HIPC(c, hipMalloc((void**)&d, (size_t)n * 16));
    uint32_t *dk = d, *dv = d + n, *ok = d + 2 * (size_t)n, *ov = d + 3 * (size_t)n;
    rtbvh_status st = RTBVH_OK;
    if (hipMemcpy(dk, keys, (size_t)n * 4, hipMemcpyHostToDevice) != hipSuccess ||
        hipMemcpy(dv, vals, (size_t)n * 4, hipMemcpyHostToDevice) != hipSuccess)
        st = fail(c, RTBVH_ERR_HIP, "sort_pairs_host: upload failed");
    if (!st) st = rtbvh_sort_pairs_async(c, dk, dv, ok, ov, n, key_bits);
    if (!st && hipStreamSynchronize(c->stream) != hipSuccess) st = fail(c, RTBVH_ERR_HIP, "sort_pairs_host: sync");
    if (!st && (hipMemcpy(kout, ok, (size_t)n * 4, hipMemcpyDeviceToHost) != hipSuccess ||
                hipMemcpy(vout, ov, (size_t)n * 4, hipMemcpyDeviceToHost) != hipSuccess))
        st = fail(c, RTBVH_ERR_HIP, "sort_pairs_host: download failed");
    (void)hipFree(d);
    return st;
}

rtbvh_status rtbvh_build_from_codes(rtbvh_ctx* c, const uint32_t* sorted_codes, const float* leaf_boxes, uint32_t n,
                                    rtbvh_node* out) {
    if (!c || !sorted_codes || !leaf_boxes || !out || n == 0 || n >= (1u << 30)) return RTBVH_ERR_INVALID_ARG;
    HIPC(c, hipSetDevice(c->cfg.device));
    if (c->ev_query) HIPC(c, hipEventSynchronize(c->ev_query));
    c->query_busy = false;
    TRY(ensure_build_capacity(c, n));
    DevBuf<float> d_boxes;
    DevBuf<rtbvh_node> d_out;
    HIPC(c, d_boxes.alloc((size_t)n * 6));
    HIPC(c, d_out.alloc(2 * (size_t)n - 1));
    reset_tree(c);
    HIPC(c, hipMemcpy(c->d_ka, sorted_codes, (size_t)n * 4, hipMemcpyHostToDevice));
    HIPC(c, hipMemcpy(d_boxes, leaf_boxes, (size_t)n * 24, hipMemcpyHostToDevice));
    BuildArgs a = build_args(c);
// ... 1175 lines not shown
```

raytracebvh_amd/csrc/build.hip:

```cpp
#include "rtbvh_internal.h"

namespace rtbvh {
namespace {

#ifndef RTBVH_NT_STORES
#define RTBVH_NT_STORES 7
#endif
template <int BIT>
__device__ __forceinline__ void st_out(float4* p, float4 v) {
    typedef float v4 __attribute__((ext_vector_type(4)));
    if (RTBVH_NT_STORES & BIT) __builtin_nontemporal_store(v4{v.x, v.y, v.z, v.w}, reinterpret_cast<v4*>(p));
    else *p = v;
}

constexpr uint32_t BLOCK = 256;
#ifndef RTBVH_REFIT_BLOCK
#define RTBVH_REFIT_BLOCK 512
#endif
constexpr uint32_t RBLOCK = RTBVH_REFIT_BLOCK;
#ifndef RTBVH_REFIT_PROBE
#define RTBVH_REFIT_PROBE 0
#endif
#ifndef RTBVH_QSKIP
#define RTBVH_QSKIP 1
// ... 616 lines not shown
    if (n == 3) P[3] = E[0];
    const bool absent1 = n == 2, absent3 = n < 4;
    float lx[4], ly[4], lz[4], hx[4], hy[4], hz[4];
    uint32_t id[4];
#pragma unroll
    for (int k = 0; k < 4; k++) {
        lx[k] = P[k].b[0]; ly[k] = P[k].b[1]; lz[k] = P[k].b[2];
        hx[k] = P[k].b[3]; hy[k] = P[k].b[4]; hz[k] = P[k].b[5];
        id[k] = (P[k].id & LEAF_BIT) ? P[k].id : P[k].slot;
    }
    if (absent1) id[1] = INVALID;
    if (absent3) id[3] = INVALID;
#pragma unroll
    for (int k = 0; k < 4; k++) ent[k] = P[k].id;
    if (absent1) ent[1] = INVALID;
    if (absent3) ent[3] = INVALID;
    qnode_words(lx, ly, lz, hx, hy, hz, make_uint4(id[0], id[1], id[2], id[3]), edge, out);
}
__device__ __forceinline__ void record_kids(const Inner* __restrict__ rec, uint32_t slot, QEnt& c0, QEnt& c1) {
    const float4* r = reinterpret_cast<const float4*>(rec + slot);
    const float4 w0 = r[0], w1 = r[1], w2 = r[2], w3 = r[3];
    const uint32_t own = __float_as_uint(w3.z);
    c0.id = __float_as_uint(w3.x);
    c1.id = __float_as_uint(w3.y);
    c0.slot = 2 * own;
    c1.slot = 2 * own + 1;
    c0.b[0] = w0.x; c0.b[1] = w0.y; c0.b[2] = w2.x; c0.b[3] = w0.z; c0.b[4] = w0.w; c0.b[5] = w2.y;
    c1.b[0] = w1.x; c1.b[1] = w1.y; c1.b[2] = w2.z; c1.b[3] = w1.z; c1.b[4] = w1.w; c1.b[5] = w2.w;
}
__device__ __forceinline__ void nbox_kids(const BuildArgs& a, uint32_t k, QEnt& c0, QEnt& c1) {
    const uint4 t = a.topo[k];
    c0.id = t.x;
    c1.id = t.y;
    c0.slot = 2 * k;
    c1.slot = 2 * k + 1;
    child_box(a, t.x, c0.b);
    child_box(a, t.y, c1.b);
}
template <bool PSEUDO_NOGRID = false>
__device__ __forceinline__ void qnode_from_records(Inner* __restrict__ rec, uint32_t slot, float E, QNode* dst) {
    QEnt e0, e1;
    record_kids(rec, slot, e0, e1);
    float4 w[4];
    uint32_t ent[4];
    greedy_qnode_words(e0, e1, [&](const QEnt& e, QEnt& c0, QEnt& c1) { record_kids(rec, e.slot, c0, c1); }, E, w,
                       ent);
    store4(dst, w);
    if (PSEUDO_NOGRID && w[0].w == 0.f) {
        f3 lo, hi;
        if (e0.id & LEAF_BIT) { ld_box(e0.b, lo, hi); store_pseudo_record(rec + e0.slot, e0.id, lo, hi); }
        if (e1.id & LEAF_BIT) { ld_box(e1.b, lo, hi); store_pseudo_record(rec + e1.slot, e1.id, lo, hi); }
    }
}

__global__ __launch_bounds__(BLOCK) void k_qnodes(Inner* __restrict__ rec, const uint32_t* __restrict__ pint,
                                                  const Inner* __restrict__ inner, QNode* __restrict__ qn, uint32_t T) {
    const uint32_t k = blockIdx.x * BLOCK + threadIdx.x;
    if (k + 1 >= T) return;
    const uint32_t slot = slot_of(pint[k], T);
    qnode_from_records(rec, slot, __uint_as_float(inner[k].aux0), qn + slot);
}

__device__ __forceinline__ void qnode_cross(const BuildArgs& a, uint32_t k) {
    const uint32_t slot = slot_of(a.pint[k], a.T);
    const float E = *node_edge(a, k);
    if (!a.rec_on) {
        QEnt e0, e1;
        nbox_kids(a, k, e0, e1);
        float4 w[4];
        uint32_t ent[4];
        greedy_qnode_words(e0, e1, [&](const QEnt& e, QEnt& c0, QEnt& c1) { nbox_kids(a, e.id, c0, c1); }, E, w, ent);
        store4(a.qnode + slot, w);
    } else if (a.pseudo) {
        qnode_from_records<false>(a.rec, slot, E, a.qnode + slot);
    } else {
        qnode_from_records<true>(a.rec, slot, E, a.qnode + slot);
    }
}
__global__ __launch_bounds__(BLOCK) void k_qnodes_late(BuildArgs a) {
    const uint32_t n = a.qlate[0];
    for (uint32_t j = blockIdx.x * BLOCK + threadIdx.x; j < n; j += gridDim.x * BLOCK) qnode_cross(a, a.qlate[1 + j]);
}

__global__ __launch_bounds__(BLOCK) void k_records(BuildArgs a) {
    const uint32_t k = blockIdx.x * BLOCK + threadIdx.x;
    if (k + 1 >= a.T) return;
    const uint4 t = a.topo[k];
    float l[6], r[6];
    child_box(a, t.x, l);
    child_box(a, t.y, r);
    f3 l0, l1, r0, r1;
    ld_box(l, l0, l1);
    ld_box(r, r0, r1);
    const uint32_t slot = slot_of(a.pint[k], a.T);
    store_record(a.rec + slot, l0, l1, r0, r1, t.x, t.y, k);
    if (a.qnode && reinterpret_cast<const float4*>(a.qnode + slot)[0].w == 0.f) {
        if (t.x & LEAF_BIT) store_leaf_record(a.rec, k, 0, t.x, l0, l1);
        if (t.y & LEAF_BIT) store_leaf_record(a.rec, k, 1, t.y, r0, r1);
    }
}
__global__ __launch_bounds__(BLOCK) void k_nbox(BuildArgs a) {
    const uint32_t k = blockIdx.x * BLOCK + threadIdx.x;
    if (k + 1 >= a.T) return;
    const Inner* r = a.rec + slot_of(a.pint[k], a.T);
    float l[6], q[6];
    record_box(r, 0, l);
    record_box(r, 1, q);
    f3 l0, l1, r0, r1;
    ld_box(l, l0, l1);
    ld_box(q, r0, r1);
    st_nbox(a.nbox, k, vmin(l0, r0), vmax(l1, r1));
}

template <bool PSEUDO>
__global__ __launch_bounds__(RBLOCK) void k_refit(BuildArgs a) {
    __shared__ uint32_t s_cnt[RBLOCK];
    __shared__ __align__(16) float s_box[RBLOCK * 12 >= RTBVH_REFIT_STAGE_SLOTS * 16 ? RBLOCK
                                                                                  : RTBVH_REFIT_STAGE_SLOTS * 16 / 12 + 1][2][6];
    static_assert(sizeof(float) * 12 * RBLOCK >= 16 * 128 * (RBLOCK / 64), "leaf staging fits in s_box");
    __shared__ uint4 s_topo[RBLOCK];
    __shared__ uint32_t s_pint[RBLOCK];
    __shared__ uint32_t s_xn;
    __shared__ uint32_t s_own[RTBVH_REFIT_STAGE_SLOTS / 32];
    __shared__ float s_topo_z[3 * (RBLOCK / 64)];
    const uint32_t T = a.T;
    const uint32_t base = blockIdx.x * RBLOCK, tid = threadIdx.x;
    const uint32_t i = base + tid;
    const uint32_t end = base + RBLOCK;
    s_cnt[tid] = 0;
    if (tid == 0) s_xn = 0;
    if (i == 0 && a.qlate) a.qlate[0] = 0;
    if (i + 1 < T) {
        s_topo[tid] = a.topo[i];
        s_pint[tid] = a.pint[i];
    }
    f3 lo = mk(0.f, 0.f, 0.f), hi = lo;
    uint32_t e = INVALID;
    float emax = 0.f;
    {
        float4 r[4] = {};
        if (i < T) {
            leaf_record_words(a, i, lo, hi, r);
            float zkey;
#if RTBVH_REFIT_PROBE == 5
            zkey = lo.z;
#else
            leaf_margin(r, lo.z, hi.z, emax, zkey);
            a.lfp[i] = leaf_footprint(lo, hi, zkey);
#endif
        }
        const uint32_t w0 = base + (tid & ~63u);
        if (RTBVH_REFIT_PROBE != 4) staged_records(a.leaf + 4 * (size_t)w0, T > w0 ? min(64u, T - w0) : 0u, r,
                       reinterpret_cast<float4*>(&s_box[0][0][0]) + 128 * (tid >> 6));
    }
    if (i < T) {
        if (T == 1) st_rootbox(a, lo, hi);
        else e = a.pleaf[i];
    }
    {
        float zl = i < T ? lo.z : INFINITY, zh = i < T ? hi.z : -INFINITY, em = emax < INFINITY ? emax : 0.f;
        reduce_zrange_block<RBLOCK / 64>(zl, zh, em, s_topo_z);
        if (tid == 0) {
            a.zpart[ZPART * blockIdx.x] = zl;
            a.zpart[ZPART * blockIdx.x + 1] = zh;
            a.zpart[ZPART * blockIdx.x + 2] = em;
        }
// ... 568 lines not shown
    if (r < T) {
        e = T == 1 ? INVALID : a.pleaf[r];
        o.child_l = INVALID;
        o.child_r = INVALID;
        o.code = a.sorted_keys[r];
        o.index = a.leaf ? 3u * (__float_as_uint(a.leaf[4 * (size_t)r + 2].y) & ~LEAF_BIT) : 0u;
    } else {
        const uint32_t k = r - T;
        e = a.pint[k];
        const uint32_t cl = a.topo[k].x, cr = a.topo[k].y;
        o.child_l = (cl & LEAF_BIT) ? (cl & ~LEAF_BIT) : T + cl;
        o.child_r = (cr & LEAF_BIT) ? (cr & ~LEAF_BIT) : T + cr;
        o.code = 0;
        o.index = 0;
    }
    if (e == INVALID) {
        o.parent = INVALID;
        for (int k = 0; k < 6; k++) box[k] = a.rootbox[k];
    } else {
        o.parent = (e >> 1) + T;
        if (a.rec_on) record_box(a.rec + slot_of(a.pint[e >> 1], T), e & 1u, box);
        else child_box(a, r < T ? LEAF_BIT | r : r - T, box);
    }
    for (int k = 0; k < 3; k++) { o.bb_min[k] = box[k]; o.bb_max[k] = box[3 + k]; }
    out[r] = o;
}

inline uint32_t blocks_for(size_t n) { return (uint32_t)((n + BLOCK - 1) / BLOCK); }

}

void launch_bounds(const BuildArgs& a, hipStream_t s) {
    uint32_t blocks = blocks_for(a.V);
    if (blocks > BOUNDS_BLOCKS) blocks = BOUNDS_BLOCKS;
    if (blocks == 0) blocks = 1;
    hipLaunchKernelGGL(k_bounds, dim3(blocks), dim3(BLOCK), 0, s, a.opos, a.V, a.bounds);
    hipLaunchKernelGGL(k_bounds_final, dim3(1), dim3(BLOCK), 0, s, a.bounds, blocks);
}
void launch_update_vertices(const VertexUpdate& u, hipStream_t s) {
    uint32_t blocks = blocks_for(u.count);
    if (blocks > BOUNDS_BLOCKS) blocks = BOUNDS_BLOCKS;
    if (u.bounds && u.first == 0 && u.count == u.V) {
        hipLaunchKernelGGL(k_update_vertices<true>, dim3(blocks), dim3(BLOCK), 0, s, u);
        hipLaunchKernelGGL(k_bounds_final, dim3(1), dim3(BLOCK), 0, s, u.bounds, blocks);
        return;
    }
    hipLaunchKernelGGL(k_update_vertices<false>, dim3(blocks), dim3(BLOCK), 0, s, u);
    if (u.bounds) {
        BuildArgs a{};
        a.opos = u.opos;
        a.V = u.V;
        a.bounds = u.bounds;
        launch_bounds(a, s);
    }
}
void launch_morton(const BuildArgs& a, hipStream_t s) {
    hipLaunchKernelGGL(k_morton<true>, dim3(blocks_for(a.T)), dim3(BLOCK), 0, s, a);
}
void launch_clip(const BuildArgs& a, hipStream_t s) {
    hipLaunchKernelGGL(k_morton<false>, dim3(blocks_for(a.T)), dim3(BLOCK), 0, s, a);
}
void launch_karras(const BuildArgs& a, hipStream_t s) {
    if (a.T < 2) return;
    if (a.delta_mode == 0) hipLaunchKernelGGL(k_karras<0>, dim3(blocks_for(a.T)), dim3(BLOCK), 0, s, a);
    else hipLaunchKernelGGL(k_karras<1>, dim3(blocks_for(a.T)), dim3(BLOCK), 0, s, a);
}
uint32_t small_build_max() { return SMALL_T; }
uint32_t small_sort_max() { return 8 * SMALL_BLOCK; }
static void launch_one_workgroup(void (*kernel)(BuildArgs, uint32_t*, uint32_t*), const BuildArgs& a, hipStream_t s) {
    hipLaunchKernelGGL(kernel, dim3(1), dim3(SMALL_BLOCK), 0, s, a, const_cast<uint32_t*>(a.sorted_keys),
                       const_cast<uint32_t*>(a.sorted_vals));
}
void launch_morton_sort_small(const BuildArgs& a, hipStream_t s) {
    launch_one_workgroup(a.T <= 4 * SMALL_BLOCK ? k_morton_sort_small<4> : k_morton_sort_small<8>, a, s);
}
void launch_build_small(const BuildArgs& a, hipStream_t s) {
    launch_one_workgroup(a.delta_mode == 0 ? k_build_small<0> : k_build_small<1>, a, s);
}
void launch_qnodes(const BuildArgs& a, hipStream_t s) {
    if (a.T > 1)
        hipLaunchKernelGGL(k_qnodes, dim3((a.T - 1 + BLOCK - 1) / BLOCK), dim3(BLOCK), 0, s, a.rec, a.pint, a.inner,
                           a.qnode, a.T);
}
uint32_t refit_blocks(uint32_t T) { return (T + RBLOCK - 1) / RBLOCK; }
__global__ __launch_bounds__(1024) void k_zrange(const float* __restrict__ zpart, uint32_t nb, float* __restrict__ rootbox) {
    __shared__ float s_z[3 * 16];
    float zl = INFINITY, zh = -INFINITY, em = 0.f;
    for (uint32_t b = threadIdx.x; b < nb; b += 1024) {
        zl = fminf(zl, zpart[ZPART * b]);
        zh = fmaxf(zh, zpart[ZPART * b + 1]);
        em = fmaxf(em, zpart[ZPART * b + 2]);
    }
    reduce_zrange_block<16>(zl, zh, em, s_z);
    if (threadIdx.x == 0) {
        rootbox[6] = zl;
        rootbox[7] = zh;
        rootbox[8] = em;
    }
}
void launch_refit_leaves(const BuildArgs& a, hipStream_t s) {
    const uint32_t nb = refit_blocks(a.T);
    if (a.pseudo) hipLaunchKernelGGL(k_refit<true>, dim3(nb), dim3(RBLOCK), 0, s, a);
    else hipLaunchKernelGGL(k_refit<false>, dim3(nb), dim3(RBLOCK), 0, s, a);
    hipLaunchKernelGGL(k_zrange, dim3(1), dim3(1024), 0, s, a.zpart, nb, a.rootbox);
}
static uint32_t launch_refit_group(const BuildArgs& a, hipStream_t s) {
    if (a.T <= RBLOCK) return 0;
    const uint32_t nb = refit_blocks(a.T);
    hipLaunchKernelGGL(k_refit_group, dim3((nb + RGROUP - 1) / RGROUP), dim3(GBLOCK), 0, s, a);
    return min(1024u, (nb + 15) / 16);
}
void launch_pb_count_top(const BuildArgs& b, const TraceArgs& a, uint32_t* off, uint32_t* cur, uint4* bins, uint32_t cap,
                         uint32_t ntx, uint32_t leaf_blocks, hipStream_t s) {
    const uint32_t nlate = launch_refit_group(b, s);
    hipLaunchKernelGGL(k_pb_count_late, dim3(nlate + leaf_blocks), dim3(BLOCK), 0, s, b, a, nlate, off, cur, bins, cap, ntx);
}
void launch_refit_tail(const BuildArgs& a, hipStream_t s) {
    const uint32_t nlate = launch_refit_group(a, s);
    if (nlate) hipLaunchKernelGGL(k_qnodes_late, dim3(nlate), dim3(BLOCK), 0, s, a);
}
__global__ __launch_bounds__(BLOCK) void k_pseudo(const float4* __restrict__ leaf, const uint32_t* __restrict__ pleaf,
                                                  Inner* __restrict__ rec, uint32_t T) {
    const uint32_t j = blockIdx.x * BLOCK + threadIdx.x;
    if (j >= T) return;
    const float4 b0 = leaf[4 * (size_t)j + 2], b1 = leaf[4 * (size_t)j + 3];
    store_pseudo_record(rec + pleaf[j], LEAF_BIT | j, mk(b0.z, b0.w, b1.x), mk(b1.y, b1.z, b1.w));
}
void launch_pseudo(const BuildArgs& a, hipStream_t s) {
    if (a.T > 1) hipLaunchKernelGGL(k_pseudo, dim3((a.T + BLOCK - 1) / BLOCK), dim3(BLOCK), 0, s, a.leaf, a.pleaf, a.rec, a.T);
}
void launch_records(const BuildArgs& a, hipStream_t s) {
    if (a.T > 1) hipLaunchKernelGGL(k_records, dim3(blocks_for(a.T - 1)), dim3(BLOCK), 0, s, a);
}
void launch_nbox(const BuildArgs& a, hipStream_t s) {
    if (a.T > 1) hipLaunchKernelGGL(k_nbox, dim3(blocks_for(a.T - 1)), dim3(BLOCK), 0, s, a);
}
void launch_export(const BuildArgs& a, void* out, hipStream_t s) {
    hipLaunchKernelGGL(k_export, dim3(blocks_for(2 * (size_t)a.T - 1)), dim3(BLOCK), 0, s, a, (RefNode*)out);
}
void launch_from_codes(const BuildArgs& a, const float* leaf_boxes, hipStream_t s) {
    launch_karras(a, s);
    if (a.T > 1) (void)hipMemsetAsync(a.refit_cnt, 0, sizeof(uint32_t) * (a.T - 1), s);
    hipLaunchKernelGGL(k_refit_boxes, dim3(blocks_for(a.T)), dim3(BLOCK), 0, s, a, leaf_boxes);
    launch_qnodes(a, s);
}

}
```

raytracebvh_amd/csrc/rtbvh_internal.h:

```cpp
#pragma once
#include <hip/hip_runtime.h>
#include <stdint.h>

#include "rtbvh_device.h"

namespace rtbvh {

#ifndef RTBVH_BOUNCE_WAVES
#define RTBVH_BOUNCE_WAVES 8
#endif
constexpr uint32_t BOUNCE_WAVES = RTBVH_BOUNCE_WAVES;

constexpr uint32_t SORT_BLOCK = 256;
#ifndef RTBVH_SORT_ITEMS
#define RTBVH_SORT_ITEMS 16
#endif
constexpr uint32_t SORT_ITEMS = RTBVH_SORT_ITEMS;
constexpr uint32_t SORT_TILE = SORT_BLOCK * SORT_ITEMS;
#ifndef RTBVH_RADIX_BITS
#define RTBVH_RADIX_BITS 8
#endif
constexpr uint32_t RADIX_BITS = RTBVH_RADIX_BITS;
constexpr uint32_t RADIX = 1u << RADIX_BITS;
constexpr size_t BOUNDS_WORDS = 8 + 6 * 1024;
constexpr uint32_t ROOTBOX_WORDS = 16;
constexpr uint32_t ZPART = 3;

inline uint32_t sort_tiles(uint32_t n) { return (n + SORT_TILE - 1) / SORT_TILE; }
inline size_t sort_scratch_words(uint32_t n) { return (size_t)RADIX * sort_tiles(n) + RADIX; }

struct SortResult { uint32_t* keys; uint32_t* vals; };
SortResult radix_sort_pairs(const uint32_t* kin, const uint32_t* vin, uint32_t* ka, uint32_t* va, uint32_t* kb,
                            uint32_t* vb, uint32_t n, uint32_t key_bits, uint32_t* scratch, hipStream_t s);

struct BuildArgs {
    const float4* opos;
    const uint32_t* idx;
    const uint32_t* matidx;
    uint32_t V, T;
    int morton_mode, delta_mode;
    const float* cam;
    float smin[3], smax[3];
    float* bounds;
    uint32_t* keys;
    uint32_t* vals;
    float4* tclip;
    const uint32_t* sorted_keys;
    const uint32_t* sorted_vals;
    float4* leaf;
    Inner* inner;
    uint4* topo;
    Inner* rec;
    uint32_t* pleaf;
    uint32_t* pint;
    uint32_t* refit_cnt;
    uint32_t* xlist;
    uint32_t* xcnt;
    float* rootbox;
    QNode* qnode;
    uint4* lfp;
    float* zpart;
    uint32_t pseudo;
    uint32_t rec_on;
    uint32_t* qlate;
    float* nbox;
};
void launch_bounds(const BuildArgs& a, hipStream_t s);
void launch_morton(const BuildArgs& a, hipStream_t s);
void launch_clip(const BuildArgs& a, hipStream_t s);
struct VertexUpdate {
    const float* pos;
    uint32_t pos_stride;
    const float* nrm;
    uint32_t nrm_stride;
    uint32_t first, count;
    float4* opos;
    float* verts;
    float* bounds;
    uint32_t V;
};
void launch_update_vertices(const VertexUpdate& u, hipStream_t s);
void launch_karras(const BuildArgs& a, hipStream_t s);
void launch_refit_leaves(const BuildArgs& a, hipStream_t s);
void launch_refit_tail(const BuildArgs& a, hipStream_t s);
void launch_pseudo(const BuildArgs& a, hipStream_t s);
uint32_t refit_blocks(uint32_t T);
void launch_qnodes(const BuildArgs& a, hipStream_t s);
uint32_t small_build_max();
void launch_build_small(const BuildArgs& a, hipStream_t s);
uint32_t small_sort_max();
void launch_morton_sort_small(const BuildArgs& a, hipStream_t s);
void launch_records(const BuildArgs& a, hipStream_t s);
void launch_nbox(const BuildArgs& a, hipStream_t s);
void launch_export(const BuildArgs& a, void* out_nodes, hipStream_t s);
void launch_from_codes(const BuildArgs& a, const float* leaf_boxes, hipStream_t s);

struct TraceArgs {
    const Inner* inner;
    const uint4* topo;
    const float* nbox;
    bool nb;
    const float4* leaf;
    const float4* tclip;
    const float* verts;
    const uint32_t* idx;
    const uint32_t* matidx;
    const Mat* mats;
    const uint32_t* texels;
    const uint4* texinfo;
    const float* srgb;
    uint32_t ntex;
    uint32_t T, W, H, rank, nranks;
    uint32_t band0, bstep;
    uint32_t my_bands;
    const uint32_t* band_list;
    const uint32_t* band_slots;
    const uint32_t* pb_gate;
    uint32_t pb_cap, pb_ntx;
    const float* rootbox;
    const uint4* lfp;
    const float* cam;
    float4* color;
    float* intensity;
    unsigned long long* counters;
    unsigned long long* overflow;
    int stack_limit, stack_limit4;
    int stack_limit4b;
    bool limited;
    bool acyclic;
    float* refl_rec;
    float* refr_rec;
    const QNode* qnode;
    uint32_t* pb_list;
};
enum class PrimaryKind { LANE_REFERENCE, LANE_NEAREST, PACKET_REFERENCE, PACKET_NEAREST, PACKET_WIDE, BINNED };
enum class BounceWalk { REFERENCE, NEAREST, WIDE_QUANTIZED };
void launch_primary(const TraceArgs& a, RayQ* q, uint32_t* qcount, bool count, bool emit, PrimaryKind kind,
                    hipStream_t s);
struct Redo {
    uint32_t* list;
    uint32_t* count;
    uint32_t* defer = nullptr;
    const uint32_t* dnext = nullptr;
};
constexpr uint32_t REDO_BLOCKS = 512;
constexpr uint32_t PB_TILE = 32;
constexpr uint32_t PB_NZ = 16;
constexpr uint32_t PB_LEAVES = 1024;
constexpr uint32_t PB_LISTS = 16, PB_LIST_STRIDE = 32;
inline __host__ __device__ uint32_t pb_list_cap(uint32_t T) {
    return ((T + PB_LEAVES - 1) / PB_LEAVES + PB_LISTS - 1) / PB_LISTS * PB_LEAVES;
}
inline size_t pb_list_words(uint32_t T) { return (size_t)PB_LISTS * PB_LIST_STRIDE + (size_t)PB_LISTS * pb_list_cap(T); }
struct PrimBins {
    uint32_t* off;
    uint32_t* cur;
    uint4* bins;
    unsigned long long* keys;
    uint32_t* sums;
    uint32_t cap, ntx, nty;
};
inline uint32_t pb_tiles_x(uint32_t W) { return (W + PB_TILE - 1) / PB_TILE; }
inline uint32_t pb_tiles_y(uint32_t rows) { return (rows + PB_TILE - 1) / PB_TILE; }
void launch_pb_bins(const TraceArgs& a, const PrimBins& pb, uint32_t rows, bool zeroed, hipStream_t s,
                    const BuildArgs* tail = nullptr);
void launch_pb_raster(const TraceArgs& a, const PrimBins& pb, uint32_t rows, RayQ* q, uint32_t* qcount, bool count,
                      bool emit, hipStream_t s, const Redo* redo = nullptr, bool small_tiles = false);
bool pb_keys_used();
void launch_pb_count_top(const BuildArgs& b, const TraceArgs& a, uint32_t* off, uint32_t* cur, uint4* bins, uint32_t cap,
                         uint32_t ntx, uint32_t leaf_blocks, hipStream_t s);
void launch_pb_gate(const TraceArgs& a, const PrimBins& pb, RayQ* q, uint32_t* qcount, bool count, bool emit,
                    hipStream_t s, bool reference);
struct ZeroList {
    static constexpr int N = 5;
    uint32_t* ptr[N];
    size_t words[N];
};
void launch_zero(const ZeroList& z, hipStream_t s);
void launch_bounce(const TraceArgs& a, const RayQ* qin, const uint32_t* qin_count, const uint32_t* perm, RayQ* qout,
                   uint32_t* qout_count, bool count, bool emit, bool nearest, hipStream_t s);
#ifndef RTBVH_NEXT_SEGS
#define RTBVH_NEXT_SEGS 64
#endif
constexpr uint32_t NEXT_SEGS = RTBVH_NEXT_SEGS;
constexpr uint32_t NEXT_STRIDE = 32;
constexpr uint32_t NEXT_WORDS = 16 * NEXT_SEGS * NEXT_STRIDE;
constexpr uint32_t DEFER_CLAIM = 1, DEFER_COUNT = 2;
constexpr uint32_t DEFER_VALID = 0x80000000u;
struct BounceShade {
    RayQ* qout;
    uint32_t* qout_count;
    bool emit;
    uint32_t* redo;
    uint32_t* redo_count;
    uint32_t P;
};
void launch_bounce_traverse(const TraceArgs& a, const RayQ* qin, const uint32_t* qin_count, const uint32_t* perm,
                            bool count, BounceWalk walk, float2* hitrec, uint32_t* next, uint32_t blocks,
                            hipStream_t s, bool cert = false, uint32_t* defer = nullptr, const BounceShade* es = nullptr);
void launch_bounce_shade(const TraceArgs& a, const RayQ* qin, const uint32_t* qin_count, const float2* hitrec,
                         RayQ* qout, uint32_t* qout_count, bool count, bool emit, uint32_t P, hipStream_t s,
                         const Redo* redo = nullptr);
struct CameraWords { float w[32]; };
void launch_set_camera(const float* wvp, const float* wv, float* cam, hipStream_t s);
void launch_count_diff(const float4* a, const float4* b, size_t n, unsigned long long* diff, hipStream_t s);
void launch_assemble(const float4* bands, const uint32_t* slots, uint32_t stride_rows, uint32_t W, uint32_t H,
                     uint32_t nranks,
                     float4* frame, hipStream_t s);
void launch_present(const float4* color, uint32_t W, uint32_t H, uint32_t* out, hipStream_t s);
void launch_bounce_keys(const RayQ* q, const uint32_t* count, const float* box, uint32_t P, uint32_t* keys,
                        uint32_t* vals, hipStream_t s);

struct QueryArgs {
    const Inner* inner;
    const uint4* topo;
    const float* nbox;
    bool nb;
    const float4* leaf;
    uint32_t T;
    const float4* rays;
    float4* hits;
    uint32_t n;
    const uint32_t* perm;
    uint32_t* next;
    unsigned long long* counts;
    unsigned long long* overflow;
    int stack_limit;
    const uint32_t* n_dev;
    const QNode* qnode;
    const float4* tclip;
    uint32_t* redo;
    uint32_t* redo_n;
    uint32_t* next2;
    unsigned long long* walk;
};
constexpr uint32_t QUERY_COUNT_WORDS = 4;
constexpr uint32_t QUERY_COUNTS_AT = NEXT_SEGS * NEXT_STRIDE, QUERY_WALK_AT = QUERY_COUNTS_AT + 2 * QUERY_COUNT_WORDS;
constexpr uint32_t QUERY_REDO_N_AT = QUERY_WALK_AT + 2 * QUERY_COUNT_WORDS;
constexpr uint32_t QUERY_NEXT2_AT = QUERY_REDO_N_AT + NEXT_STRIDE;
constexpr uint32_t QUERY_SCRATCH_WORDS = QUERY_NEXT2_AT + NEXT_SEGS * NEXT_STRIDE;
void launch_query(const QueryArgs& a, bool any, bool count, hipStream_t s);
void launch_query_certified(const QueryArgs& a, bool any, bool count, hipStream_t s);
void launch_query_keys(const float4* rays, uint32_t n, const float* box, uint32_t* keys, uint32_t* vals,
                       hipStream_t s);

struct NearestArgs {
    const Inner* inner;
    const uint4* topo;
    const float* nbox;
    bool nb;
    const float4* leaf;
    uint32_t T;
    const float4* points;
    float4* out;
    uint32_t n;
    const uint32_t* perm;
    uint32_t* next;
    unsigned long long* counts;
    unsigned long long* overflow;
    int stack_limit;
};
constexpr uint32_t QUERY_NEAREST_AT = QUERY_SCRATCH_WORDS;
static_assert(QUERY_NEAREST_AT % 2 == 0, "the count block's 8-byte words");
void launch_nearest(const NearestArgs& a, bool count, hipStream_t s);
void launch_nearest_keys(const float4* points, uint32_t n, const float* box, uint32_t* keys, uint32_t* vals,
                         hipStream_t s);

struct WithinArgs {
    const Inner* inner;
    const uint4* topo;
    const float* nbox;
    bool nb;
    const float4* leaf;
    uint32_t T;
    const float4* points;
    unsigned long long* offsets;
    uint2* pairs;
    unsigned long long capacity;
    uint32_t n;
    const uint32_t* perm;
    uint32_t* next;
    unsigned long long* counts;
// ... 188 lines not shown
```

raytracebvh_amd/csrc/trace.hip:

```cpp
#include "rtbvh_internal.h"

#include <type_traits>

namespace rtbvh {
namespace {

constexpr uint32_t BLOCK = 256;
constexpr float EPSILON = 0.01f;

struct Counts { uint32_t internal, leaf, overflow, wint, wleaf; };

typedef float f2v __attribute__((ext_vector_type(2)));
typedef float v4f __attribute__((ext_vector_type(4)));

__device__ __forceinline__ uint32_t child_slot(uint32_t id, uint32_t own, uint32_t side) {
    return (id & LEAF_BIT) ? id : 2 * own + side;
}
__device__ __forceinline__ uint32_t root_slot(uint32_t T) { return T == 1 ? LEAF_BIT : 2 * T - 2; }

__device__ __forceinline__ void pin(float4& a) {
    float x = a.x, y = a.y, z = a.z, w = a.w;
    asm volatile("" : "+v"(x), "+v"(y), "+v"(z), "+v"(w));
    a = make_float4(x, y, z, w);
}
// ... 1395 lines not shown
        const HitInfo h = shade_hit_tri(a, tri, o, d, t);
        tex = h.textured;
        col = make_float4(lerpf(col.x, h.color.x, intensity), lerpf(col.y, h.color.y, intensity),
                          lerpf(col.z, h.color.z, intensity), lerpf(col.w, h.color.w, intensity));
        intensity *= h.shininess / 1000.f * 1;
        const f3 ro = add(h.hitp, mul(h.nrm, .0001f));
        const f3 rd = normalize(reflect(d, h.nrm));
        e.intensity = intensity;
        e.ox = ro.x; e.oy = ro.y; e.oz = ro.z;
        e.dx = rd.x; e.dy = rd.y; e.dz = rd.z;
        live = 0 < intensity;
        if (a.refl_rec) put_record(a.refl_rec, e.idx, intensity, true, ro, rd, col);
    } else {
        col = make_float4(lerpf(col.x, .5f, intensity), lerpf(col.y, .5f, intensity),
                          lerpf(col.z, .5f, intensity), lerpf(col.w, 1.f, intensity));
        intensity = 0.f;
        if (a.refl_rec) {
            float* r = a.refl_rec + 14 * (size_t)e.idx;
            r[0] = 0.f;
            r[10] = col.x; r[11] = col.y; r[12] = col.z; r[13] = col.w;
        }
    }
    a.color[e.idx] = col;
    if (a.intensity) a.intensity[e.idx] = intensity;
    return live;
}

__device__ __forceinline__ void leaf_clip_box(const float4* __restrict__ tclip, uint32_t tri, f3& lo, f3& hi) {
    const float4* P = tclip + TCS * (size_t)tri;
    const float4 a0 = P[0], a1 = P[1], a2 = P[2];
    const f3 v0 = mk(a0.x, a0.y, a0.z), v1 = mk(a1.x, a1.y, a1.z), v2 = mk(a2.x, a2.y, a2.z);
    lo = vmin(vmin(v0, v1), v2);
    hi = vmax(vmax(v0, v1), v2);
}
__device__ __forceinline__ bool leaf_certified(const TraceArgs& a, uint32_t tri, f3 o, f3 inv, float t) {
    f3 lo, hi;
    leaf_clip_box(a.tclip, tri, lo, hi);
    float tm;
    return ray_box(o, inv, lo.x, lo.y, lo.z, hi.x, hi.y, hi.z, true, t, tm);
}

template <bool CERT>
__device__ __forceinline__ void bounce_shade_ray(const TraceArgs& a, const RayQ* __restrict__ qin, uint32_t i, float2 h2,
                                                 bool valid, RayQ& e, bool& live, bool& flagged, uint32_t& hits,
                                                 uint32_t& tex) {
    live = false;
    flagged = false;
    if (!valid) return;
    e = qin[i];
    uint32_t tri = __float_as_uint(h2.y);
    bool skip = false;
    if (CERT) {
        flagged = hit_flagged(tri);
        tri = (tri & LEAF_BIT) ? INVALID : tri & ~HIT_FLAG;
        if (signbit(h2.x)) {
            skip = flagged;
            flagged = false;
            h2.x = -h2.x;
        } else if (!flagged && tri != INVALID) {
            f3 o, d, inv;
            load_ray(&e, o, d, inv);
            flagged = !leaf_certified(a, tri, o, inv, h2.x);
        }
    }
    if (!flagged && !skip) live = bounce_apply(a, e, tri, h2.x, hits, tex);
}
template <bool CERT>
__device__ __forceinline__ void bounce_shade_emit(const TraceArgs& a, const RayQ* qin, uint32_t i, float2 h2, bool valid,
                                                  RayQ* qout, uint32_t* qout_count, int emit, uint32_t* redo,
                                                  uint32_t* redo_count, uint32_t& hits, uint32_t& tex) {
    RayQ e;
    bool live, flagged;
    uint32_t h1 = 0, t1 = 0;
    bounce_shade_ray<CERT>(a, qin, i, h2, valid, e, live, flagged, h1, t1);
    hits += h1;
    tex += t1;
    if (CERT) {
        const uint32_t rs = wave_append(flagged, redo_count);
        if (flagged) redo[rs] = i;
    }
    const uint32_t qs = wave_append(emit && live, qout_count);
    if (emit && live) qout[qs] = e;
}
template <bool COUNT, int MODE, bool LIM, bool GUARD, bool CERT = false, bool ES = false>
__global__ __launch_bounds__(BLOCK, BOUNCE_WAVES) void k_bounce_trav(const Inner* __restrict__ inner,
                                                          const QNode* __restrict__ qn,
                                                          const float4* __restrict__ leaf, uint32_t T,
                                                          const RayQ* __restrict__ qin,
                                                          const uint32_t* __restrict__ qin_count,
                                                          const uint32_t* __restrict__ perm,
                                                          float2* __restrict__ hitrec, uint32_t* __restrict__ next,
                                                          unsigned long long* __restrict__ counters,
                                                          unsigned long long* __restrict__ overflow, int stack_limit,
                                                          uint32_t* __restrict__ defer, const uint4* __restrict__ topo,
                                                          const float* __restrict__ nbox, uint32_t nwalk, TraceArgs ta,
                                                          RayQ* __restrict__ qout, uint32_t* __restrict__ qout_count,
                                                          int emit, uint32_t* __restrict__ redo,
                                                          uint32_t* __restrict__ redo_count) {
    constexpr bool NEAREST = MODE >= 1, WIDE = MODE == 2;
    static_assert(!CERT || (WIDE && !LIM), "the certified walk is the 4-wide one, without a stack limit");
    const int limit = LIM ? stack_limit : WIDE ? STACK4B : STACK_SIZE;
    const uint32_t n = *qin_count;
    if (n == 0) return;
    const uint32_t lane = lane_id();
    Counts c = {0, 0, 0, 0, 0};
    constexpr bool wt = CERT && ES && RTBVH_EARLY_SHADE;
    if (CERT && ES && RTBVH_EARLY_SHADE && blockIdx.x >= nwalk) {
        const uint32_t b0 = (blockIdx.x - nwalk) * ESHADE_RAYS;
        uint32_t hits = 0, tex = 0;
        for (uint32_t base = b0; base < b0 + ESHADE_RAYS && base < n; base += BLOCK) {
            const uint32_t i = base + threadIdx.x;
            bool valid = false;
            float2 h2 = make_float2(0.f, 0.f);
            if (i < n) {
                unsigned long long* hp = reinterpret_cast<unsigned long long*>(hitrec + i);
                const unsigned long long v = __hip_atomic_load(hp, __ATOMIC_RELAXED, __HIP_MEMORY_SCOPE_AGENT);
                const uint32_t xb = (uint32_t)v, yb = (uint32_t)(v >> 32);
                const bool ready = xb != HIT_NOT_READY && xb != HIT_SHADED &&
                                   !(xb == 0xFF800000u && yb == (INVALID ^ HIT_FLAG));
                if (ready) {
                    unsigned long long exp = v;
                    valid = __hip_atomic_compare_exchange_strong(
                        hp, &exp, (unsigned long long)HIT_SHADED | (unsigned long long)yb << 32, __ATOMIC_RELAXED,
                        __ATOMIC_RELAXED, __HIP_MEMORY_SCOPE_AGENT);
                }
                h2 = make_float2(__uint_as_float(xb), __uint_as_float(yb));
            }
            bounce_shade_emit<true>(ta, qin, i, h2, valid, qout, qout_count, emit, redo, redo_count, hits, tex);
        }
        if (COUNT) flush_counts<COUNT>(ta, c, hits, tex, 5);
        return;
    }
#ifdef RTBVH_TAIL_PROBE
    const uint64_t t_start = __builtin_amdgcn_s_memrealtime();
#endif
    if (CERT && DEFER_WORKERS && blockIdx.x < DEFER_WORKERS && gridDim.x > 2 * DEFER_WORKERS && threadIdx.x < 64) {
        for (;;) {
            defer_walk_all<COUNT>(next, defer, inner, topo, nbox, leaf, T, qin, hitrec, c, wt);
            bool used = true;
            for (uint32_t seg = lane; seg < NEXT_SEGS; seg += 64) {
                uint32_t s0, len;
                segment_bounds(n, seg, s0, len);
                used = used && __hip_atomic_load(next + NEXT_STRIDE * seg, __ATOMIC_RELAXED, __HIP_MEMORY_SCOPE_AGENT) >= len;
            }
            if (__ballot(!used) == 0) break;
            __builtin_amdgcn_s_sleep(64);
        }
        defer_walk_all<COUNT>(next, defer, inner, topo, nbox, leaf, T, qin, hitrec, c, wt);
        if (COUNT) {
            unsigned long long v[2] = {c.internal, c.leaf};
            wave_sum(v);
            if (lane == 0) {
                atomicAdd(&counters[5], v[0]);
                atomicAdd(&counters[6], v[1]);
            }
        }
        return;
    }
    bool has = false, qfast = false;
    uint32_t r = 0;
    Walk w{0u, INVALID, 0, false, 0.f, 0u, 0u};
    uint32_t& node = w.node;
    int& sp = w.sp;
    uint32_t& guard = w.guard;
    uint32_t btri = 0;
    uint64_t key = NO_HIT;
    f3 o = mk(0.f, 0.f, 0.f), d = o, inv = o;
    const MtNodeK nk = mt_node_consts();
    bool flg = false;
    __shared__ uint32_t s_stk[WIDE ? 1 : SB][WIDE ? 1 : BLOCK];
    uint32_t stack[WIDE ? 1 : STACK_SIZE - SB];
    const uint32_t tid = threadIdx.x;
    BlockStack st{&s_stk[0][0] + (WIDE ? 0u : tid), stack};
#define RTBVH_WIDE_PART 1
#include "wide_walk.inc"
    Refill rf;
    unsigned long long wsteps = 0, mixed = 0, active_lanes = 0;
    while (true) {
        refill_claim(rf, next, n, has, [&](uint32_t p) {
            r = perm ? perm[p] : p;
            load_ray(qin + r, o, d, inv);
            qfast = WIDE && qnode_fast_ray(o, inv);
            has = true;
            w = walk_start(root_slot(T), T);
            key = NO_HIT;
            if (CERT) {
                flg = !(qfast && dot(d, d) <= MT_DD);
                if (flg) {
                    const float2 mk_def = make_float2(-__builtin_inff(), __uint_as_float(INVALID ^ HIT_FLAG));
                    if (wt) st_hitrec(hitrec + r, mk_def);
                    else hitrec[r] = mk_def;
                    const uint32_t k = atomicAdd(next + DEFER_COUNT, 1u);
                    __hip_atomic_store(defer + k, r | DEFER_VALID, __ATOMIC_RELEASE, __HIP_MEMORY_SCOPE_AGENT);
                    has = false;
                    flg = false;
                }
            }
        });
        if (__ballot(has) == 0 && rf.drained) break;
        if (COUNT) {
            const uint64_t act = __ballot(has);
            const uint64_t lf = __ballot(has && (node & LEAF_BIT) != 0);
            wsteps++;
            active_lanes += (uint32_t)__popcll(act);
            mixed += (lf != 0 && lf != act);
        }
        if (!has) continue;
        bool done = false;
        if (WIDE) {
#ifdef RTBVH_DEBUG_PIXEL
            const bool wide_dbg = COUNT && qin[r].idx == (uint32_t)RTBVH_DEBUG_PIXEL;
#endif
#define RTBVH_WIDE_PART 2
#include "wide_walk.inc"
        } else {
            const bool isleaf = (node & LEAF_BIT) != 0;
            const v4f* rr = isleaf ? reinterpret_cast<const v4f*>(leaf + 4 * (size_t)(node & ~LEAF_BIT))
                                   : reinterpret_cast<const v4f*>(inner + node);
            v4f q0 = rr[0], q1 = rr[1], q2 = rr[2], q3 = rr[3];
            pin(q0); pin(q1); pin(q2); pin(q3);
            if (GUARD && --guard == 0) {
                c.overflow++;
                done = true;
            } else {
                if (isleaf) {
                    if (walk_leaf<COUNT>(w, st, WalkRule<NEAREST>{}, c, o, d, node & ~LEAF_BIT, mk(q0.x, q0.y, q0.z),
                                         mk(q0.w, q1.x, q1.y), mk(q1.z, q1.w, q2.x)))
                        btri = __float_as_uint(q2.y) & ~LEAF_BIT;
                } else {
                    const uint32_t own = __float_as_uint(q3.z);
                    walk_node<COUNT>(w, st, WalkRule<NEAREST>{}, c, o, inv, limit,
                                     record_children(q0, q1, q2, child_slot(__float_as_uint(q3.x), own, 0),
                                                     child_slot(__float_as_uint(q3.y), own, 1)));
                }
                done = sp == -1;
            }
        }
        if (done) {
            if (WIDE) {
                uint32_t id = key != NO_HIT ? btri : INVALID;
                if (CERT && flg) id ^= HIT_FLAG;
// ... 2060 lines not shown
    if (most == 0) return;
    size_t blocks = (most + BLOCK - 1) / BLOCK;
    if (blocks > 1024) blocks = 1024;
    hipLaunchKernelGGL(k_zero, dim3((uint32_t)blocks, ZeroList::N), dim3(BLOCK), 0, s, z);
}

bool pb_keys_used() { return !RTBVH_PB_FUSE; }

void launch_pb_bins(const TraceArgs& a, const PrimBins& pb, uint32_t rows, bool zeroed, hipStream_t s,
                    const BuildArgs* tail) {
    if (rows == 0 || a.W == 0 || a.T == 0) return;
    const uint32_t keys = pb.ntx * pb.nty * PB_NZ;
    if (!zeroed) (void)hipMemsetAsync(pb.off, 0, ((size_t)keys + 1) * sizeof(uint32_t), s);
    if (!zeroed && a.pb_list) (void)hipMemsetAsync(a.pb_list, 0, (size_t)PB_LISTS * PB_LIST_STRIDE * sizeof(uint32_t), s);
    const dim3 lg((a.T + PB_LEAVES - 1) / PB_LEAVES);
    if (tail) launch_pb_count_top(*tail, a, pb.off, pb.cur, pb.bins, pb.cap, pb.ntx, lg.x, s);
    else hipLaunchKernelGGL((k_pb_bin<false>), lg, dim3(BLOCK), 0, s, a, pb.off, pb.cur, pb.bins, pb.cap, pb.ntx);
    const uint32_t sb = (keys + PB_SCAN - 1) / PB_SCAN;
    hipLaunchKernelGGL(k_pb_sums, dim3(sb), dim3(PB_SCAN), 0, s, pb.off, pb.sums, keys);
    hipLaunchKernelGGL(k_pb_scan, dim3(sb), dim3(PB_SCAN), 0, s, pb.off, pb.cur, pb.sums, keys);
    hipLaunchKernelGGL((k_pb_bin<true>), lg, dim3(BLOCK), 0, s, a, pb.off, pb.cur, pb.bins, pb.cap, pb.ntx);
}

void launch_pb_raster(const TraceArgs& a, const PrimBins& pb, uint32_t rows, RayQ* q, uint32_t* qcount, bool count,
                      bool emit, hipStream_t s, const Redo* redo, bool small_tiles) {
    if (rows == 0 || a.W == 0 || a.T == 0) return;
    const dim3 grid(pb.ntx, pb.nty);
    uint32_t* rl = redo ? redo->list : nullptr;
    uint32_t* rc = redo ? redo->count : nullptr;
    const bool rec = a.refl_rec || a.refr_rec;
    const auto raster = [&](auto* kernel, uint32_t rb) {
        hipLaunchKernelGGL(kernel, grid, dim3(rb), 0, s, a, pb.off, pb.bins, pb.cap, pb.ntx, rows, pb.keys, q, qcount,
                           (int)emit, rl, rc);
    };
#if RTBVH_PB_FUSE
    with_bools([&](auto COUNT, auto CERT) {
        if (rec) raster(k_primary_binned<COUNT, CERT, true, true>, PB_RASTER_BLOCK);
        else if (small_tiles)
            raster(k_primary_binned<COUNT, CERT, true, false, PB_RASTER_BLOCK_SMALL>, PB_RASTER_BLOCK_SMALL);
        else raster(k_primary_binned<COUNT, CERT, true, false>, PB_RASTER_BLOCK);
    }, count, redo != nullptr);
#else
    (void)rec;
    (void)small_tiles;
    with_bools([&](auto COUNT) { raster(k_primary_binned<COUNT, false, false, true>, PB_RASTER_BLOCK); }, count);
    with_bools([&](auto COUNT, auto CERT) {
        hipLaunchKernelGGL((k_pb_shade<COUNT, CERT>), grid, dim3(PB_SHADE_BLOCK), 0, s, a, pb.off, pb.cap, pb.ntx, rows,
                           pb.keys, q, qcount, (int)emit, rl, rc);
    }, count, redo != nullptr);
#endif
    if (redo) {
        with_bools([&](auto COUNT) {
            hipLaunchKernelGGL((k_primary_redo<COUNT>), dim3(REDO_BLOCKS), dim3(BLOCK), 0, s, a, rl, rc, q, qcount, (int)emit);
        }, count);
    }
}

void launch_pb_gate(const TraceArgs& a, const PrimBins& pb, RayQ* q, uint32_t* qcount, bool count, bool emit,
                    hipStream_t s, bool reference) {
    if (a.W == 0 || a.T == 0) return;
    TraceArgs g = a;
    g.pb_gate = pb.off;
    g.pb_cap = pb.cap;
    g.pb_ntx = pb.ntx;
    launch_primary(g, q, qcount, count, emit, reference ? PrimaryKind::LANE_REFERENCE : PrimaryKind::LANE_NEAREST, s);
}

void launch_bounce(const TraceArgs& a, const RayQ* qin, const uint32_t* qin_count, const uint32_t* perm, RayQ* qout,
                   uint32_t* qout_count, bool count, bool emit, bool nearest, hipStream_t s) {
    const uint32_t blocks = 2048;
    with_bools([&](auto COUNT, auto NEAREST, auto LIM) {
        hipLaunchKernelGGL((k_bounce<COUNT, NEAREST, LIM>), dim3(blocks), dim3(BLOCK), 0, s, a, qin, qin_count, perm, qout,
                           qout_count, (int)emit);
    }, count, nearest, a.limited);
}

void launch_bounce_keys(const RayQ* q, const uint32_t* count, const float* box, uint32_t P, uint32_t* keys,
                        uint32_t* vals, hipStream_t s) {
    hipLaunchKernelGGL(k_bounce_keys, dim3((P + BLOCK - 1) / BLOCK), dim3(BLOCK), 0, s, q, count, box, P, keys, vals);
}

void launch_bounce_traverse(const TraceArgs& a, const RayQ* qin, const uint32_t* qin_count, const uint32_t* perm,
                            bool count, BounceWalk walk, float2* hitrec, uint32_t* next, uint32_t blocks,
                            hipStream_t s, bool cert, uint32_t* defer, const BounceShade* es) {
    if (blocks == 0) blocks = 2048;
    const bool wide = walk == BounceWalk::WIDE_QUANTIZED;
    const bool certified = wide && cert;
    const bool early = RTBVH_EARLY_SHADE && certified && es;
    const uint32_t nshade = early ? (es->P + ESHADE_RAYS - 1) / ESHADE_RAYS : 0u;
    if (early) hipLaunchKernelGGL(k_hit_init, dim3(1024), dim3(BLOCK), 0, s, hitrec, qin_count);
    const auto launch = [&](auto* kernel) {
        hipLaunchKernelGGL(kernel, dim3(blocks + nshade), dim3(BLOCK), 0, s, a.inner, a.qnode, a.leaf, a.T, qin, qin_count,
                           perm, hitrec, next, a.counters, a.overflow, wide ? a.stack_limit4b : a.stack_limit, defer,
                           a.topo, a.nb ? a.nbox : nullptr, blocks, a, early ? es->qout : nullptr,
                           early ? es->qout_count : nullptr, early ? (int)es->emit : 0, early ? es->redo : nullptr,
                           early ? es->redo_count : nullptr);
    };
    const bool guard = count || !a.acyclic;
    if (certified)
        with_bools([&](auto COUNT, auto GUARD, auto ES) { launch(k_bounce_trav<COUNT, 2, false, GUARD, true, ES>); }, count,
                   guard, early);
    else if (wide)
        with_bools([&](auto COUNT, auto LIM, auto GUARD) { launch(k_bounce_trav<COUNT, 2, LIM, GUARD>); }, count, a.limited,
                   guard);
    else
        with_bools([&](auto COUNT, auto NEAREST, auto LIM, auto GUARD) {
            launch(k_bounce_trav<COUNT, NEAREST ? 1 : 0, LIM, GUARD>);
        }, count, walk == BounceWalk::NEAREST, a.limited, guard);
}

void launch_bounce_shade(const TraceArgs& a, const RayQ* qin, const uint32_t* qin_count, const float2* hitrec,
                         RayQ* qout, uint32_t* qout_count, bool count, bool emit, uint32_t P, hipStream_t s,
                         const Redo* redo) {
    if (P == 0) return;
    uint32_t* rl = redo ? redo->list : nullptr;
    uint32_t* rc = redo ? redo->count : nullptr;
    const dim3 g((P + BLOCK - 1) / BLOCK);
    with_bools([&](auto COUNT, auto CERT) {
        hipLaunchKernelGGL((k_bounce_shade<COUNT, CERT>), g, dim3(BLOCK), 0, s, a, qin, qin_count, hitrec, qout, qout_count,
                           (int)emit, rl, rc);
    }, count, redo != nullptr);
    if (redo)
        with_bools([&](auto COUNT) {
            hipLaunchKernelGGL((k_bounce_redo<COUNT>), dim3(REDO_BLOCKS), dim3(BLOCK), 0, s, a, qin, rl, rc, qout,
                               qout_count, (int)emit, redo->defer, redo->dnext);
        }, count);
}

void launch_assemble(const float4* bands, const uint32_t* slots, uint32_t stride_rows, uint32_t W, uint32_t H,
                     uint32_t nranks, float4* frame, hipStream_t s) {
    const size_t n = (size_t)W * H;
    hipLaunchKernelGGL(k_assemble, dim3((uint32_t)((n + BLOCK - 1) / BLOCK)), dim3(BLOCK), 0, s, bands, slots,
                       stride_rows, W, H, nranks, frame);
}

void launch_present(const float4* color, uint32_t W, uint32_t H, uint32_t* out, hipStream_t s) {
    const size_t n = (size_t)W * H;
    if (n) hipLaunchKernelGGL(k_present, dim3((uint32_t)((n + BLOCK - 1) / BLOCK)), dim3(BLOCK), 0, s, color, W, H, out);
}

__global__ __launch_bounds__(64) void k_set_camera(CameraWords m, float* __restrict__ cam) {
    if (threadIdx.x < 32) cam[threadIdx.x] = m.w[threadIdx.x];
}

void launch_set_camera(const float* wvp, const float* wv, float* cam, hipStream_t s) {
    CameraWords m;
    for (int i = 0; i < 16; i++) {
        m.w[i] = wvp[i];
        m.w[16 + i] = wv[i];
    }
    hipLaunchKernelGGL(k_set_camera, dim3(1), dim3(64), 0, s, m, cam);
}

void launch_count_diff(const float4* a, const float4* b, size_t n, unsigned long long* diff, hipStream_t s) {
    if (n == 0) return;
    size_t blocks = (n + BLOCK - 1) / BLOCK;
    if (blocks > 4096) blocks = 4096;
    hipLaunchKernelGGL(k_count_diff, dim3((uint32_t)blocks), dim3(BLOCK), 0, s, reinterpret_cast<const uint4*>(a),
                       reinterpret_cast<const uint4*>(b), n, diff);
}

}
```

raytracebvh_amd/graphics.py:

```python
from __future__ import annotations

import ctypes
import os

import numpy as np

from . import _lib as _L
from .scene import EYE_REFERENCE, Scene, camera_look, camera_orbit, camera_reference


def _is_tensor(x) -> bool:
    return type(x).__module__.split(".")[0] == "torch" and hasattr(x, "data_ptr")


def make_rays(origins, directions, t_max=float("inf")):
    if _is_tensor(origins) or _is_tensor(directions):
        import torch
        dev = origins.device if _is_tensor(origins) else directions.device
        o = torch.as_tensor(origins, dtype=torch.float32, device=dev).reshape(-1, 3)
        d = torch.as_tensor(directions, dtype=torch.float32, device=dev).reshape(-1, 3)
        if o.shape != d.shape:
            raise ValueError(f"make_rays: {tuple(o.shape)} origins and {tuple(d.shape)} directions")
        rays = torch.zeros((o.shape[0], 8), dtype=torch.float32, device=dev)
        rays[:, 0:3] = o
# ... 906 lines not shown
        if hasattr(stream, "cuda_stream"):
            return stream
        return torch.cuda.ExternalStream(int(stream), device=device) if int(stream) else torch.cuda.default_stream(device)

    def _signed_on_stream(self, pts, mode, stream, read):
        import torch
        ts = self._torch_stream(stream, pts.device)
        with torch.cuda.stream(ts):
            rec = torch.empty((len(pts), 8), dtype=torch.float32, device=pts.device)
            self.signed(pts, None, mode, out=rec, stream=ts)
            return read(rec)

    def signed_distance(self, points, max_dist2=None, mode: int = 0, stream=None):
        mode = mode & ~_L.SIGNED_INSIDE_ONLY
        if _is_tensor(points):
            import torch
            _, pts = check_nearest_points(points, float("inf") if max_dist2 is None else max_dist2,
                                          getattr(self, "device", None))

            def read(rec):
                d2 = rec[:, 3]
                d = torch.where(d2 < 0, torch.full_like(d2, float("nan")), torch.sqrt(d2.clamp(min=0)))
                inside = (rec[:, 7].contiguous().view(torch.int32) & 1) != 0
                return torch.where(inside, -d, d)
            return self._signed_on_stream(pts, mode, stream, read)
        rec = self.signed(points, max_dist2, mode)
        with np.errstate(invalid="ignore"):
            d = np.where(rec["tri"] == 0xFFFFFFFF, np.float32(np.nan), np.sqrt(rec["dist2"]))
        return np.where(rec["flags"] & 1, -d, d).astype(np.float32)

    def inside(self, points, vote3: bool = False, mode: int = 0, stream=None):
        mode = mode | _L.SIGNED_INSIDE_ONLY | (_L.SIGNED_VOTE3 if vote3 else 0)
        if _is_tensor(points):
            import torch
            _, pts = check_nearest_points(points, float("inf"), getattr(self, "device", None))
            return self._signed_on_stream(pts, mode, stream,
                                          lambda rec: (rec[:, 7].contiguous().view(torch.int32) & 1) != 0)
        return (self.signed(points, None, mode)["flags"] & 1).astype(bool)

    def signed_counts(self) -> dict:
        out = np.zeros(4, np.uint64)
        self._check(_L.lib().rtbvh_signed_counts(self._h, _L.ptr(out)))
        return dict(zip(("points", "inside", "internal_steps", "leaf_steps"), (int(v) for v in out)))

    def read_framebuffer(self) -> np.ndarray:
        out = np.zeros((self.height, self.width, 4), np.float32)
        self._check(_L.lib().rtbvh_read_framebuffer(self._h, _L.ptr(out)))
        return out

    def read_rays(self):
        refl = np.zeros((self.height, self.width, 14), np.float32)
        refr = np.zeros((self.height, self.width, 14), np.float32)
        self._check(_L.lib().rtbvh_read_rays(self._h, _L.ptr(refl), _L.ptr(refr)))
        return refl, refr

    def present(self) -> np.ndarray:
        out = np.zeros((self.height, self.width, 4), np.uint8)
        self._check(_L.lib().rtbvh_present(self._h, _L.ptr(out)))
        return out

    def read_intensity(self) -> np.ndarray:
        out = np.zeros((self.height, self.width), np.float32)
        self._check(_L.lib().rtbvh_read_intensity(self._h, _L.ptr(out)))
        return out

    def framebuffer_device_ptr(self) -> int:
        return _L.lib().rtbvh_framebuffer_device(self._h) or 0

    def read_bvh(self) -> np.ndarray:
        out = np.zeros(2 * self.num_tris - 1, dtype=_L.NODE_DTYPE)
        self._check(_L.lib().rtbvh_read_bvh(self._h, ctypes.c_void_p(out.ctypes.data), len(out)))
        return out

    def read_wide(self) -> np.ndarray:
        out = np.zeros((max(2 * (self.num_tris - 1), 0), 16), np.uint32)
        self._check(_L.lib().rtbvh_read_wide(self._h, _L.ptr(out), len(out)))
        return out

    def read_qnodes(self) -> np.ndarray:
        out = np.zeros((max(2 * self.num_tris - 1, 0) if self.num_tris > 1 else 0, 16), np.uint32)
        self._check(_L.lib().rtbvh_read_qnodes(self._h, _L.ptr(out), len(out)))
        return out

    def read_morton(self) -> np.ndarray:
        out = np.zeros(self.num_tris, np.uint32)
        self._check(_L.lib().rtbvh_read_morton(self._h, _L.ptr(out)))
        return out

    def read_sorted(self):
        keys = np.zeros(self.num_tris, np.uint32)
        ids = np.zeros(self.num_tris, np.uint32)
        self._check(_L.lib().rtbvh_read_sorted(self._h, _L.ptr(keys), _L.ptr(ids)))
        return keys, ids

    def stats(self) -> dict:
        s = _L.Stats()
        self._check(_L.lib().rtbvh_get_stats(self._h, ctypes.byref(s)))
        return s.as_dict()

    def reset_stats(self):
        self._check(_L.lib().rtbvh_reset_stats(self._h))

    def set_flags(self, flags: int):
        self._check(_L.lib().rtbvh_set_flags(self._h, flags))

    def bin_builds(self) -> int:
        return int(_L.lib().rtbvh_bin_builds(self._h))

    def bin_sets(self) -> int:
        return int(_L.lib().rtbvh_bin_sets(self._h))

    def sort_pairs(self, keys: np.ndarray, vals: np.ndarray, key_bits: int = 32):
        keys = np.ascontiguousarray(keys, np.uint32)
        vals = np.ascontiguousarray(vals, np.uint32)
        ko = np.zeros_like(keys)
        vo = np.zeros_like(vals)
        self._check(_L.lib().rtbvh_sort_pairs_host(self._h, _L.ptr(keys), _L.ptr(vals), _L.ptr(ko), _L.ptr(vo),
                                                   len(keys), key_bits))
        return ko, vo

    def sort_pairs_device(self, keys_ptr: int, vals_ptr: int, keys_out_ptr: int, vals_out_ptr: int, n: int,
                          key_bits: int = 32):
        self._check(_L.lib().rtbvh_sort_pairs_async(self._h, ctypes.c_void_p(keys_ptr), ctypes.c_void_p(vals_ptr),
                                                    ctypes.c_void_p(keys_out_ptr), ctypes.c_void_p(vals_out_ptr),
                                                    n, key_bits))

    def build_from_codes(self, sorted_codes: np.ndarray, leaf_boxes: np.ndarray) -> np.ndarray:
        codes = np.ascontiguousarray(sorted_codes, np.uint32)
        boxes = np.ascontiguousarray(leaf_boxes, np.float32).reshape(-1, 6)
        out = np.zeros(2 * len(codes) - 1, dtype=_L.NODE_DTYPE)
        self._check(_L.lib().rtbvh_build_from_codes(self._h, _L.ptr(codes), _L.ptr(boxes), len(codes),
                                                    ctypes.c_void_p(out.ctypes.data)))
        return out


class Graphics:

    def __init__(self, width: int = 800, height: int = 800, bounces: int = 3, **ctx_kwargs):
        self.width, self.height, self.bounces = width, height, bounces
        self.eye = np.array(EYE_REFERENCE, np.float32)
        self.ctx = Context(**ctx_kwargs)

    def onInit(self, scene: Scene):
        self.ctx.set_scene(scene)

    def onUpdate(self):
        wvp, wv = camera_look(self.eye, self.width, self.height)
        self.ctx.set_camera(wvp, wv)
        self.computeBVH()

    def onKeyDown(self, key: int):
        self.eye = camera_orbit(self.eye, key)

    def computeBVH(self):
        self.ctx.compute_bvh(self.width, self.height, self.bounces)

    def framebuffer(self) -> np.ndarray:
        return self.ctx.read_framebuffer()

    def onRender(self) -> np.ndarray:
        return self.ctx.present()

    def save_bmp(self, path: str):
        save_bmp(path, self.onRender())

    def onDestroy(self):
# ... 17 lines not shown
```

Before: 5223 Mrays/s.

## Build binned-SAH walk tree after repeated traces and use it for bounce traversal

Adds a second, higher-quality BVH built top-down with binned SAH splits per level on the GPU. It is built lazily once a scene has been traced a set number of times (default 512) and is then used by the bounce traversal kernel in place of the Morton-built tree. The goal is fewer node visits for incoherent bounce rays, at the cost of a one-off build, extra device memory, and a fallback path when allocation fails. It is skipped inside enqueue_frame, during graph capture, or when certified tracing is off.

```diff
diff --git a/include/rtbvh.h b/include/rtbvh.h
--- a/include/rtbvh.h
+++ b/include/rtbvh.h
@@ -113,6 +113,8 @@
     uint64_t redo_rays[2];
     uint64_t trav_longest;
     uint64_t redo_deferred;
+    uint32_t walk_tree_state;
+    uint32_t walk_tree_depth;
 } rtbvh_stats;
 typedef struct rtbvh_ctx rtbvh_ctx;
 
@@ -337,6 +339,8 @@
 rtbvh_status rtbvh_read_bvh(rtbvh_ctx* ctx, rtbvh_node* out, uint32_t capacity);
 rtbvh_status rtbvh_read_wide(rtbvh_ctx* ctx, uint32_t* records, uint64_t capacity);
 rtbvh_status rtbvh_read_qnodes(rtbvh_ctx* ctx, uint32_t* nodes, uint64_t capacity);
+rtbvh_status rtbvh_read_walk_tree(rtbvh_ctx* ctx, uint32_t* children, float* boxes, uint32_t* parents, uint32_t* perm,
+                                  uint32_t* qnodes);
 rtbvh_status rtbvh_read_morton(rtbvh_ctx* ctx, uint32_t* codes);
 rtbvh_status rtbvh_read_sorted(rtbvh_ctx* ctx, uint32_t* sorted_codes, uint32_t* tri_ids);
 rtbvh_status rtbvh_read_rays(rtbvh_ctx* ctx, rtbvh_ray_present* reflect_out, rtbvh_ray_present* refract_out);
diff --git a/raytracebvh_amd/_lib.py b/raytracebvh_amd/_lib.py
--- a/raytracebvh_amd/_lib.py
+++ b/raytracebvh_amd/_lib.py
@@ -28,7 +28,7 @@
     "rtbvh_trace_async", "rtbvh_compute_bvh", "rtbvh_trace_band_async", "rtbvh_band_rows", "rtbvh_verify_walk",
     "rtbvh_deal_bands", "rtbvh_deal_rows", "rtbvh_set_band_deal",
     "rtbvh_synchronize", "rtbvh_read_framebuffer", "rtbvh_read_intensity", "rtbvh_framebuffer_device",
-    "rtbvh_read_bvh", "rtbvh_read_wide", "rtbvh_read_qnodes", "rtbvh_read_morton", "rtbvh_read_sorted", "rtbvh_read_rays", "rtbvh_get_stats",
+    "rtbvh_read_bvh", "rtbvh_read_wide", "rtbvh_read_qnodes", "rtbvh_read_walk_tree", "rtbvh_read_morton", "rtbvh_read_sorted", "rtbvh_read_rays", "rtbvh_get_stats",
     "rtbvh_reset_stats", "rtbvh_set_flags", "rtbvh_bin_builds", "rtbvh_bin_sets",
     "rtbvh_sort_pairs_async", "rtbvh_sort_pairs_host", "rtbvh_build_from_codes", "rtbvh_scene_load_obj",
     "rtbvh_scene_synthetic", "rtbvh_scene_free", "rtbvh_scene_num_vertices", "rtbvh_scene_num_indices",
@@ -133,7 +133,8 @@
                 ("walk_state", ctypes.c_uint32), ("packet_steps", ctypes.c_uint64 * 2),
                 ("cert_traces", ctypes.c_uint64), ("redo_total", ctypes.c_uint64),
                 ("bin_entries", ctypes.c_uint64 * 2), ("redo_rays", ctypes.c_uint64 * 2),
-                ("trav_longest", ctypes.c_uint64), ("redo_deferred", ctypes.c_uint64)]
+                ("trav_longest", ctypes.c_uint64), ("redo_deferred", ctypes.c_uint64),
+                ("walk_tree_state", ctypes.c_uint32), ("walk_tree_depth", ctypes.c_uint32)]
 
     def as_dict(self) -> dict:
         d = {}
@@ -198,6 +199,7 @@
         "rtbvh_read_morton": (i32, [vp, vp]),
         "rtbvh_read_wide": (i32, [vp, vp, ctypes.c_uint64]),
         "rtbvh_read_qnodes": (i32, [vp, vp, ctypes.c_uint64]),
+        "rtbvh_read_walk_tree": (i32, [vp, vp, vp, vp, vp, vp]),
         "rtbvh_read_sorted": (i32, [vp, vp, vp]),
         "rtbvh_read_rays": (i32, [vp, vp, vp]),
         "rtbvh_get_stats": (i32, [vp, ctypes.POINTER(Stats)]),
diff --git a/raytracebvh_amd/csrc/api.hip b/raytracebvh_amd/csrc/api.hip
--- a/raytracebvh_amd/csrc/api.hip
+++ b/raytracebvh_amd/csrc/api.hip
@@ -198,6 +198,24 @@
     size_t cap_split = 0;
     Event ev_fork;
     uint64_t bins_epoch = 1;
+    struct WalkTree {
+        uint32_t cap_T = 0;
+        DevBuf<float4> item[2];
+        DevBuf<uint32_t> own[2], act[2], range, bins, ctl, wperm;
+        DevBuf<uint4> dec, wtopo;
+        DevBuf<unsigned long long> flags, sums;
+        DevBuf<float> wbox;
+        DevBuf<QNode> wqnode;
+        uint64_t epoch = 0;
+        uint64_t counted = 0;
+        uint32_t traces = 0;
+        uint64_t no_memory = 0;
+        hipStream_t stream = nullptr;
+        Event ready;
+    } wt;
+    uint32_t knob_walk_tree = 512;
+    uint32_t knob_walk_tree_maxdepth = WT_MAX_DEPTH;
+    bool in_frame = false;
     uint64_t bin_builds = 0;
     bool knob_bins_reuse = true;
     LastTrace last;
@@ -763,6 +781,7 @@
     uint32_t tblocks;
     uint32_t ntx, nty;
     bool inflight, fuse_tail, overlap, small_tiles, early_shade;
+    bool walk_tree;
     uint32_t bset;
     bool fill_bins;
 };
@@ -954,8 +973,9 @@
                 if (tg && b == 0) HIPC(c, hipEventRecord(ev[3], sg));
                 uint32_t* nxb = set.next + (size_t)NEXT_SEGS * NEXT_STRIDE * b;
                 const BounceShade es{q[(b + 1) & 1], &qc[b + 1], b + 1 < bounces, mine.redo, &qc[17 + b], p.Pg};
+                const WalkTreeUse wu{c->wt.wqnode, c->wt.ctl + WT_STATE};
                 launch_bounce_traverse(ag, q[b & 1], &qc[b], perm, count, p.wk.bounce, set.hit, nxb, p.tblocks, sg, cert,
-                                       mine.defer, p.early_shade ? &es : nullptr);
+                                       mine.defer, p.early_shade ? &es : nullptr, p.walk_tree ? &wu : nullptr);
                 if (tg && b == 0) HIPC(c, hipEventRecord(ev[4], sg));
                 const Redo rd{mine.redo, &qc[17 + b], mine.defer, nxb};
                 launch_bounce_shade(ag, q[b & 1], &qc[b], set.hit, q[(b + 1) & 1], &qc[b + 1], count, b + 1 < bounces,
@@ -980,7 +1000,7 @@
 
 rtbvh_status enqueue_walks(rtbvh_ctx* c, uint32_t W, uint32_t H, uint32_t bounces, uint32_t rank, uint32_t nranks,
                            float4* color, float* inten, hipStream_t s, uint32_t slot, uint32_t flags, bool timed,
-                           uint32_t walk_state, bool cert = false) {
+                           uint32_t walk_state, bool cert = false, bool walk_tree = false) {
     const bool leaf_pending = c->leaf_pending;
     c->leaf_pending = false;
     TailGuard tail{c, c->tail_pending};
@@ -1003,6 +1023,7 @@
     if ((flags & RTBVH_FLAG_REFRACT_RECORDS) && slot)
         return fail(c, RTBVH_ERR_INVALID_ARG, "ray records are traced on the context stream only");
     WalkPlan p = plan_walks(c, a, bounces, s, slot, flags, cert, timed, tail.pending, leaf_pending);
+    p.walk_tree = walk_tree;
     TRY(prepare_walks(c, p, a, deal, tail));
     TRY(launch_walks(c, p, a, tail));
     const bool frame_here = color == c->d_color && nranks == 1;
@@ -1025,6 +1046,88 @@
     return TracePlan{ref | RTBVH_FLAG_NEAREST_FIRST | RTBVH_FLAG_REFILL_BOUNCE | RTBVH_FLAG_WIDE_BVH |
                          RTBVH_FLAG_BINNED_PRIMARY,
                      true, 2};
+}
+
+rtbvh_status ensure_walk_tree_capacity(rtbvh_ctx* c, uint32_t T) {
+    rtbvh_ctx::WalkTree& w = c->wt;
+    if (T <= w.cap_T && w.wqnode) return RTBVH_OK;
+    w.cap_T = 0;
+    const size_t n = T;
+    for (int k = 0; k < 2; k++) {
+        HIPC(c, w.item[k].alloc(2 * n));
+        HIPC(c, w.own[k].alloc(n));
+        HIPC(c, w.act[k].alloc(n / 2 + 1));
+    }
+    HIPC(c, w.range.alloc(16 * n));
+    HIPC(c, w.bins.alloc(walk_tree_table_words(T)));
+    HIPC(c, w.ctl.alloc(WT_CTL_WORDS));
+    HIPC(c, w.wperm.alloc(n));
+    HIPC(c, w.dec.alloc(n));
+    HIPC(c, w.wtopo.alloc(n));
+    HIPC(c, w.flags.alloc(n + 1));
+    HIPC(c, w.sums.alloc(scan_sums_words(T)));
+    HIPC(c, w.wbox.alloc(6 * n));
+    HIPC(c, w.wqnode.alloc(2 * n));
+    w.cap_T = T;
+    return RTBVH_OK;
+}
+WalkTreeArgs walk_tree_args(rtbvh_ctx* c) {
+    rtbvh_ctx::WalkTree& w = c->wt;
+    WalkTreeArgs a{};
+    a.leaf = c->d_leaf;
+    a.T = c->T;
+    a.maxdepth = c->knob_walk_tree_maxdepth;
+    for (int k = 0; k < 2; k++) {
+        a.item[k] = w.item[k];
+        a.own[k] = w.own[k];
+        a.act[k] = w.act[k];
+    }
+    a.range = w.range;
+    a.dec = w.dec;
+    a.flags = w.flags;
+    a.sums = w.sums;
+    a.bins = w.bins;
+    a.ctl = w.ctl;
+    a.wtopo = w.wtopo;
+    a.wbox = w.wbox;
+    a.wperm = w.wperm;
+    return a;
+}
+bool walk_tree_current(const rtbvh_ctx* c) { return c->wt.epoch == c->bins_epoch && c->tree.built && !c->stale; }
+
+rtbvh_status use_walk_tree(rtbvh_ctx* c, const TracePlan& p, uint32_t bounces, hipStream_t s, bool* use) {
+    *use = false;
+    rtbvh_ctx::WalkTree& w = c->wt;
+    if (!p.cert || bounces == 0 || c->knob_walk_tree == 0 || c->capturing || c->in_frame || c->T < 2) return RTBVH_OK;
+    if (w.counted != c->bins_epoch) {
+        w.counted = c->bins_epoch;
+        w.traces = 0;
+    }
+    ++w.traces;
+    if (w.epoch != c->bins_epoch && w.traces >= c->knob_walk_tree && w.no_memory != c->bins_epoch) {
+        if (ensure_walk_tree_capacity(c, c->T) != RTBVH_OK) {
+            w = rtbvh_ctx::WalkTree{};
+            w.counted = w.no_memory = c->bins_epoch;
+            (void)hipGetLastError();
+            c->err.clear();
+            return RTBVH_OK;
+        }
+        TRY(order_after_context(c, s));
+        const WalkTreeArgs a = walk_tree_args(c);
+        HIPC(c, hipMemsetAsync(w.wtopo, 0xFF, sizeof(uint4) * c->T, s));
+        HIPC(c, hipMemsetAsync(w.wqnode, 0, sizeof(QNode) * 2 * (size_t)c->T, s));
+        launch_walk_tree(a, s);
+        launch_walk_qnodes(build_args(c), a, w.wqnode, s);
+        TRY(check_launch(c, "walk tree kernels"));
+        if (!w.ready) HIPC(c, hipEventCreateWithFlags(w.ready.out(), hipEventDisableTiming));
+        HIPC(c, hipEventRecord(w.ready, s));
+        w.stream = s;
+        w.epoch = c->bins_epoch;
+    }
+    if (w.epoch != c->bins_epoch) return RTBVH_OK;
+    if (s != w.stream) HIPC(c, hipStreamWaitEvent(s, w.ready, 0));
+    *use = true;
+    return RTBVH_OK;
 }
 
 rtbvh_status enqueue_trace(rtbvh_ctx* c, uint32_t W, uint32_t H, uint32_t bounces, uint32_t rank, uint32_t nranks,
@@ -1062,7 +1165,10 @@
         }
         if (c->small_key == key && c->small_flags == fw && c->small_packet) p.flags |= RTBVH_FLAG_PACKET_PRIMARY;
     }
-    return enqueue_walks(c, W, H, bounces, rank, nranks, color, inten, s, slot, p.flags, true, p.state, p.cert);
+    bool walk_tree = false;
+    TRY(use_walk_tree(c, p, bounces, s, &walk_tree));
+    return enqueue_walks(c, W, H, bounces, rank, nranks, color, inten, s, slot, p.flags, true, p.state, p.cert,
+                         walk_tree);
 }
 
 }
@@ -1145,6 +1251,9 @@
     if (const char* e = getenv("RTBVH_EARLY_SHADE")) c->knob_no_early_shade = atoi(e) == 0;
     if (const char* e = getenv("RTBVH_PB_SMALL_TILES")) c->knob_no_small_tiles = atoi(e) == 0;
     if (const char* e = getenv("RTBVH_BINS_REUSE")) c->knob_bins_reuse = atoi(e) != 0;
+    if (const char* e = getenv("RTBVH_WALK_TREE")) c->knob_walk_tree = (uint32_t)std::max(0, atoi(e));
+    if (const char* e = getenv("RTBVH_WALK_TREE_MAXDEPTH"))
+        c->knob_walk_tree_maxdepth = (uint32_t)std::min(std::max(1, atoi(e)), (int)WT_MAX_DEPTH);
     *out = c;
     return RTBVH_OK;
 }
@@ -1348,7 +1457,9 @@
 
 static rtbvh_status enqueue_frame(rtbvh_ctx* c, uint32_t W, uint32_t H, uint32_t bounces) {
     rtbvh_status st = build_tree(c, TAIL_TO_TRACE | (c->knob_overlap ? LEAF_EVENT : 0u));
+    c->in_frame = true;
     if (!st) st = rtbvh_trace_async(c, W, H, bounces);
+    c->in_frame = false;
     return flush_tail(c, st);
 }
 
@@ -1880,6 +1991,37 @@
         }
     }
     out->redo_total = out->redo_rays[0] + out->redo_rays[1];
+    if (walk_tree_current(c)) {
+        uint32_t w[2];
+        HIPC(c, hipMemcpy(w, c->wt.ctl.h + WT_STATE, sizeof(w), hipMemcpyDeviceToHost));
+        out->walk_tree_state = w[0];
+        out->walk_tree_depth = w[1];
+    }
+    return RTBVH_OK;
+}
+
+rtbvh_status rtbvh_read_walk_tree(rtbvh_ctx* c, uint32_t* children, float* boxes, uint32_t* parents, uint32_t* perm,
+                                  uint32_t* qnodes) {
+    if (!c) return RTBVH_ERR_INVALID_ARG;
+    TRY(sync_all(c));
+    uint32_t state = 0;
+    if (walk_tree_current(c)) HIPC(c, hipMemcpy(&state, c->wt.ctl.h + WT_STATE, sizeof(state), hipMemcpyDeviceToHost));
+    if (state != 1) return fail(c, RTBVH_ERR_NOT_READY, "read_walk_tree: no walk tree in use");
+    const size_t n = c->T;
+    if (children || parents) {
+        std::vector<uint4> t(n - 1);
+        HIPC(c, hipMemcpy(t.data(), c->wt.wtopo, sizeof(uint4) * (n - 1), hipMemcpyDeviceToHost));
+        for (size_t k = 0; k + 1 < n; k++) {
+            if (children) {
+                children[2 * k] = t[k].x;
+                children[2 * k + 1] = t[k].y;
+            }
+            if (parents) parents[k] = t[k].z;
+        }
+    }
+    if (boxes) HIPC(c, hipMemcpy(boxes, c->wt.wbox, sizeof(float) * 6 * (n - 1), hipMemcpyDeviceToHost));
+    if (perm) HIPC(c, hipMemcpy(perm, c->wt.wperm, sizeof(uint32_t) * n, hipMemcpyDeviceToHost));
+    if (qnodes) HIPC(c, hipMemcpy(qnodes, c->wt.wqnode, sizeof(QNode) * (2 * n - 1), hipMemcpyDeviceToHost));
     return RTBVH_OK;
 }
 
diff --git a/raytracebvh_amd/csrc/build.hip b/raytracebvh_amd/csrc/build.hip
--- a/raytracebvh_amd/csrc/build.hip
+++ b/raytracebvh_amd/csrc/build.hip
@@ -722,6 +722,34 @@
     for (uint32_t j = blockIdx.x * BLOCK + threadIdx.x; j < n; j += gridDim.x * BLOCK) qnode_cross(a, a.qlate[1 + j]);
 }
 
+__global__ __launch_bounds__(BLOCK) void k_walk_qnodes(BuildArgs a, const uint32_t* __restrict__ ctl, QNode* __restrict__ wq) {
+    const uint32_t k = blockIdx.x * BLOCK + threadIdx.x;
+    if (k + 1 >= a.T || ctl[WT_STATE] != 1u) return;
+    const uint4 t = a.topo[k];
+    bool bad = false;
+    const auto kids = [&](uint32_t x, QEnt& c0, QEnt& c1) {
+        const uint4 tx = a.topo[x];
+        const auto in_tree = [&](uint32_t id) { return (id & LEAF_BIT) ? (id & ~LEAF_BIT) < a.T : id + 1 < a.T; };
+        if (in_tree(tx.x) && in_tree(tx.y)) {
+            nbox_kids(a, x, c0, c1);
+        } else {
+            bad = true;
+            c0.id = c1.id = LEAF_BIT;
+            c0.slot = c1.slot = 0;
+            for (int q = 0; q < 6; q++) c0.b[q] = c1.b[q] = 0.f;
+        }
+    };
+    QEnt e0, e1;
+    kids(k, e0, e1);
+    float4 w[4];
+    uint32_t ent[4];
+    greedy_qnode_words(e0, e1, [&](const QEnt& e, QEnt& c0, QEnt& c1) { kids(e.id, c0, c1); }, __uint_as_float(t.w), w,
+                       ent);
+    if (bad) w[0].w = 0.f;
+    const uint32_t slot = slot_of(t.z, a.T);
+    if (slot <= 2 * a.T - 2) store4(wq + slot, w);
+}
+
 __global__ __launch_bounds__(BLOCK) void k_records(BuildArgs a) {
     const uint32_t k = blockIdx.x * BLOCK + threadIdx.x;
     if (k + 1 >= a.T) return;
@@ -1456,6 +1484,13 @@
         hipLaunchKernelGGL(k_qnodes, dim3((a.T - 1 + BLOCK - 1) / BLOCK), dim3(BLOCK), 0, s, a.rec, a.pint, a.inner,
                            a.qnode, a.T);
 }
+void launch_walk_qnodes(const BuildArgs& a, const WalkTreeArgs& w, QNode* wqnode, hipStream_t s) {
+    if (a.T < 2) return;
+    BuildArgs b = a;
+    b.topo = w.wtopo;
+    b.nbox = w.wbox;
+    hipLaunchKernelGGL(k_walk_qnodes, dim3((a.T - 1 + BLOCK - 1) / BLOCK), dim3(BLOCK), 0, s, b, w.ctl, wqnode);
+}
 uint32_t refit_blocks(uint32_t T) { return (T + RBLOCK - 1) / RBLOCK; }
 __global__ __launch_bounds__(1024) void k_zrange(const float* __restrict__ zpart, uint32_t nb, float* __restrict__ rootbox) {
     __shared__ float s_z[3 * 16];
diff --git a/raytracebvh_amd/csrc/rtbvh_internal.h b/raytracebvh_amd/csrc/rtbvh_internal.h
--- a/raytracebvh_amd/csrc/rtbvh_internal.h
+++ b/raytracebvh_amd/csrc/rtbvh_internal.h
@@ -95,6 +95,31 @@
 void launch_export(const BuildArgs& a, void* out_nodes, hipStream_t s);
 void launch_from_codes(const BuildArgs& a, const float* leaf_boxes, hipStream_t s);
 
+constexpr uint32_t WT_STATE = 0, WT_DEPTH = 1, WT_ROOT = 2;
+constexpr uint32_t WT_NACT = 8;
+constexpr uint32_t WT_MAX_DEPTH = 64;
+constexpr uint32_t WT_CTL_WORDS = WT_NACT + WT_MAX_DEPTH + 8;
+struct WalkTreeArgs {
+    const float4* leaf;
+    uint32_t T;
+    uint32_t maxdepth;
+    float4* item[2];
+    uint32_t* own[2];
+    uint32_t* range;
+    uint4* dec;
+    unsigned long long* flags;
+    unsigned long long* sums;
+    uint32_t* act[2];
+    uint32_t* bins;
+    uint32_t* ctl;
+    uint4* wtopo;
+    float* wbox;
+    uint32_t* wperm;
+};
+size_t walk_tree_table_words(uint32_t T);
+void launch_walk_tree(const WalkTreeArgs& a, hipStream_t s);
+void launch_walk_qnodes(const BuildArgs& a, const WalkTreeArgs& w, QNode* wqnode, hipStream_t s);
+
 struct TraceArgs {
     const Inner* inner;
     const uint4* topo;
@@ -195,9 +220,14 @@
     uint32_t* redo_count;
     uint32_t P;
 };
+struct WalkTreeUse {
+    const QNode* wqnode;
+    const uint32_t* wstate;
+};
 void launch_bounce_traverse(const TraceArgs& a, const RayQ* qin, const uint32_t* qin_count, const uint32_t* perm,
                             bool count, BounceWalk walk, float2* hitrec, uint32_t* next, uint32_t blocks,
-                            hipStream_t s, bool cert = false, uint32_t* defer = nullptr, const BounceShade* es = nullptr);
+                            hipStream_t s, bool cert = false, uint32_t* defer = nullptr, const BounceShade* es = nullptr,
+                            const WalkTreeUse* wt = nullptr);
 void launch_bounce_shade(const TraceArgs& a, const RayQ* qin, const uint32_t* qin_count, const float2* hitrec,
                          RayQ* qout, uint32_t* qout_count, bool count, bool emit, uint32_t P, hipStream_t s,
                          const Redo* redo = nullptr);
diff --git a/raytracebvh_amd/csrc/trace.hip b/raytracebvh_amd/csrc/trace.hip
--- a/raytracebvh_amd/csrc/trace.hip
+++ b/raytracebvh_amd/csrc/trace.hip
@@ -1501,7 +1501,7 @@
     const uint32_t qs = wave_append(emit && live, qout_count);
     if (emit && live) qout[qs] = e;
 }
-template <bool COUNT, int MODE, bool LIM, bool GUARD, bool CERT = false, bool ES = false>
+template <bool COUNT, int MODE, bool LIM, bool GUARD, bool CERT = false, bool ES = false, bool WT = false>
 __global__ __launch_bounds__(BLOCK, BOUNCE_WAVES) void k_bounce_trav(const Inner* __restrict__ inner,
                                                           const QNode* __restrict__ qn,
                                                           const float4* __restrict__ leaf, uint32_t T,
@@ -1515,8 +1515,11 @@
                                                           const float* __restrict__ nbox, uint32_t nwalk, TraceArgs ta,
                                                           RayQ* __restrict__ qout, uint32_t* __restrict__ qout_count,
                                                           int emit, uint32_t* __restrict__ redo,
-                                                          uint32_t* __restrict__ redo_count) {
+                                                          uint32_t* __restrict__ redo_count,
+                                                          const QNode* __restrict__ wqnode,
+                                                          const uint32_t* __restrict__ wstate) {
     constexpr bool NEAREST = MODE >= 1, WIDE = MODE == 2;
+    static_assert(!WT || CERT, "the walk-only tree is the certified walk's");
     static_assert(!CERT || (WIDE && !LIM), "the certified walk is the 4-wide one, without a stack limit");
     const int limit = LIM ? stack_limit : WIDE ? STACK4B : STACK_SIZE;
     const uint32_t n = *qin_count;
@@ -1576,6 +1579,7 @@
         }
         return;
     }
+    if (WT && *wstate == 1u) qn = wqnode;
     bool has = false, qfast = false;
     uint32_t r = 0;
     Walk w{0u, INVALID, 0, false, 0.f, 0u, 0u};
@@ -3802,7 +3806,7 @@
 
 void launch_bounce_traverse(const TraceArgs& a, const RayQ* qin, const uint32_t* qin_count, const uint32_t* perm,
                             bool count, BounceWalk walk, float2* hitrec, uint32_t* next, uint32_t blocks,
-                            hipStream_t s, bool cert, uint32_t* defer, const BounceShade* es) {
+                            hipStream_t s, bool cert, uint32_t* defer, const BounceShade* es, const WalkTreeUse* wt) {
     if (blocks == 0) blocks = 2048;
     const bool wide = walk == BounceWalk::WIDE_QUANTIZED;
     const bool certified = wide && cert;
@@ -3814,10 +3818,13 @@
                            perm, hitrec, next, a.counters, a.overflow, wide ? a.stack_limit4b : a.stack_limit, defer,
                            a.topo, a.nb ? a.nbox : nullptr, blocks, a, early ? es->qout : nullptr,
                            early ? es->qout_count : nullptr, early ? (int)es->emit : 0, early ? es->redo : nullptr,
-                           early ? es->redo_count : nullptr);
+                           early ? es->redo_count : nullptr, wt ? wt->wqnode : nullptr, wt ? wt->wstate : nullptr);
     };
     const bool guard = count || !a.acyclic;
-    if (certified)
+    if (certified && wt)
+        with_bools([&](auto COUNT, auto GUARD, auto ES) { launch(k_bounce_trav<COUNT, 2, false, GUARD, true, ES, true>); },
+                   count, guard, early);
+    else if (certified)
         with_bools([&](auto COUNT, auto GUARD, auto ES) { launch(k_bounce_trav<COUNT, 2, false, GUARD, true, ES>); }, count,
                    guard, early);
     else if (wide)
diff --git a/raytracebvh_amd/csrc/walktree.hip b/raytracebvh_amd/csrc/walktree.hip
--- /dev/null
+++ b/raytracebvh_amd/csrc/walktree.hip
@@ -0,0 +1,384 @@
+#include <algorithm>
+
+#include "rtbvh_internal.h"
+
+namespace rtbvh {
+namespace {
+
+constexpr uint32_t WB = 256;
+constexpr uint32_t NBIN = 16;
+constexpr uint32_t BIN_WORDS = 14;
+constexpr uint32_t TAB_WORDS = 3 * NBIN * BIN_WORDS;
+constexpr uint32_t WT_BIG_SHIFT = 10, WT_BIG = 1u << WT_BIG_SHIFT;
+constexpr uint32_t RANGE_WORDS = 16;
+constexpr uint32_t KEY_PINF = 0xFF800000u, KEY_NINF = 0x007FFFFFu;
+constexpr uint32_t AXIS_HALVES = 3;
+
+__device__ __forceinline__ uint32_t fkey(float f) {
+    const uint32_t b = __float_as_uint(f);
+    return b ^ ((b >> 31) ? 0xFFFFFFFFu : 0x80000000u);
+}
+__device__ __forceinline__ float kfloat(uint32_t k) {
+    return __uint_as_float(k ^ ((k >> 31) ? 0x80000000u : 0xFFFFFFFFu));
+}
+__device__ __forceinline__ uint32_t tab_init_word(uint32_t w) {
+    const uint32_t j = w % BIN_WORDS;
+    return j >= 12 ? 0u : (j % 6) < 3 ? KEY_PINF : KEY_NINF;
+}
+__device__ __forceinline__ void tab_merge(uint32_t* dst, uint32_t w, uint32_t v) {
+    const uint32_t j = w % BIN_WORDS;
+    if (j == 12) atomicAdd(dst + w, v);
+    else if (j == 13 || (j % 6) >= 3) atomicMax(dst + w, v);
+    else atomicMin(dst + w, v);
+}
+__device__ __forceinline__ int wt_bin(float c, float cl, float sc) {
+    return min((int)NBIN - 1, max(0, (int)((c - cl) * sc)));
+}
+
+struct WtItem {
+    float b[6];
+    float E;
+    uint32_t id;
+};
+__device__ __forceinline__ WtItem ld_item(const float4* item, uint32_t pos) {
+    const float4 x = item[2 * (size_t)pos], y = item[2 * (size_t)pos + 1];
+    return WtItem{{x.x, x.y, x.z, x.w, y.x, y.y}, y.z, __float_as_uint(y.w)};
+}
+__device__ __forceinline__ void st_item(float4* item, uint32_t pos, const WtItem& it) {
+    item[2 * (size_t)pos] = make_float4(it.b[0], it.b[1], it.b[2], it.b[3]);
+    item[2 * (size_t)pos + 1] = make_float4(it.b[4], it.b[5], it.E, __uint_as_float(it.id));
+}
+__device__ __forceinline__ float centroid(const WtItem& it, int a) { return 0.5f * (it.b[a] + it.b[3 + a]); }
+
+struct WtFrame {
+    float cl[3], sc[3];
+    bool halves;
+};
+__device__ __forceinline__ WtFrame wt_frame(const uint32_t* R) {
+    WtFrame f;
+    f.halves = true;
+#pragma unroll
+    for (int a = 0; a < 3; a++) {
+        const float cl = kfloat(R[10 + a]), ch = kfloat(R[13 + a]);
+        const bool ext = ch > cl;
+        f.cl[a] = cl;
+        f.sc[a] = ext ? (float)NBIN / (ch - cl) : 0.f;
+        f.halves = f.halves && !ext;
+    }
+    return f;
+}
+__device__ __forceinline__ void tab_add(uint32_t* tab, const WtItem& it, const WtFrame& f, bool first_half) {
+    uint32_t kb[6], kc[3];
+#pragma unroll
+    for (int q = 0; q < 6; q++) kb[q] = fkey(it.b[q]);
+#pragma unroll
+    for (int a = 0; a < 3; a++) kc[a] = fkey(centroid(it, a));
+    const uint32_t eb = __float_as_uint(it.E);
+#pragma unroll
+    for (int a = 0; a < 3; a++) {
+        int k;
+        if (f.halves) {
+            if (a > 0) break;
+            k = first_half ? 0 : 1;
+        } else {
+            if (!(f.sc[a] > 0.f)) continue;
+            k = wt_bin(centroid(it, a), f.cl[a], f.sc[a]);
+        }
+        uint32_t* b = tab + (a * NBIN + k) * BIN_WORDS;
+#pragma unroll
+        for (int q = 0; q < 3; q++) {
+            atomicMin(b + q, kb[q]);
+            atomicMax(b + 3 + q, kb[3 + q]);
+            atomicMin(b + 6 + q, kc[q]);
+            atomicMax(b + 9 + q, kc[q]);
+        }
+        atomicAdd(b + 12, 1u);
+        atomicMax(b + 13, eb);
+    }
+}
+__device__ __forceinline__ void wave_sync() {
+    __builtin_amdgcn_fence(__ATOMIC_SEQ_CST, "wavefront");
+    __builtin_amdgcn_wave_barrier();
+}
+
+__global__ __launch_bounds__(WB) void k_wt_reset(WalkTreeArgs a, uint32_t tables) {
+    const size_t i = (size_t)blockIdx.x * WB + threadIdx.x;
+    if (i < WT_CTL_WORDS) a.ctl[i] = i == WT_NACT ? 1u : 0u;
+    if (i < RANGE_WORDS) a.range[i] = i == 0 ? a.T : i == 1 ? INVALID : i < 4 ? 0u : (i - 4) % 6 < 3 ? KEY_PINF : KEY_NINF;
+    if (i == 0) a.act[0][0] = 0u;
+    if (i < (size_t)tables * TAB_WORDS) a.bins[i] = tab_init_word((uint32_t)(i % TAB_WORDS));
+    if (i < a.T) a.dec[i] = make_uint4(INVALID, INVALID, 0u, 0u);
+}
+
+__global__ __launch_bounds__(WB) void k_wt_leaves(WalkTreeArgs a) {
+    __shared__ uint32_t s_red[13];
+    if (threadIdx.x < 13) s_red[threadIdx.x] = threadIdx.x == 12 ? 0u : threadIdx.x % 6 < 3 ? KEY_PINF : KEY_NINF;
+    __syncthreads();
+    for (size_t j = (size_t)blockIdx.x * WB + threadIdx.x; j < a.T; j += (size_t)gridDim.x * WB) {
+        const float4* r = a.leaf + 4 * j;
+        const float4 w[4] = {r[0], r[1], r[2], r[3]};
+        WtItem it{{w[2].z, w[2].w, w[3].x, w[3].y, w[3].z, w[3].w}, 0.f, (uint32_t)j};
+        float zkey;
+        leaf_margin(w, it.b[2], it.b[5], it.E, zkey);
+        st_item(a.item[0], (uint32_t)j, it);
+        a.own[0][j] = 0u;
+#pragma unroll
+        for (int q = 0; q < 3; q++) {
+            atomicMin(&s_red[q], fkey(it.b[q]));
+            atomicMax(&s_red[3 + q], fkey(it.b[3 + q]));
+            atomicMin(&s_red[6 + q], fkey(centroid(it, q)));
+            atomicMax(&s_red[9 + q], fkey(centroid(it, q)));
+        }
+        atomicMax(&s_red[12], __float_as_uint(it.E));
+    }
+    __syncthreads();
+    if (threadIdx.x < 12) {
+        if (threadIdx.x % 6 < 3) atomicMin(a.range + 4 + threadIdx.x, s_red[threadIdx.x]);
+        else atomicMax(a.range + 4 + threadIdx.x, s_red[threadIdx.x]);
+    } else if (threadIdx.x == 12) {
+        atomicMax(a.range + 2, s_red[12]);
+    }
+}
+
+__global__ __launch_bounds__(WB) void k_wt_bin(WalkTreeArgs a, uint32_t level) {
+    if (a.ctl[WT_NACT + level] == 0) return;
+    __shared__ uint32_t s_tab[TAB_WORDS];
+    const uint32_t* own = a.own[level & 1];
+    const float4* item = a.item[level & 1];
+    const uint32_t tid = threadIdx.x, T = a.T;
+    const uint32_t tiles = (T + WB - 1) / WB, per = (tiles + gridDim.x - 1) / gridDim.x;
+    const uint32_t t0 = blockIdx.x * per, t1 = min(tiles, t0 + per);
+    for (uint32_t w = tid; w < TAB_WORDS; w += WB) s_tab[w] = tab_init_word(w);
+    __syncthreads();
+    uint32_t held = INVALID;
+    const auto flush = [&]() {
+        __syncthreads();
+        uint32_t* g = a.bins + (size_t)(held >> WT_BIG_SHIFT) * TAB_WORDS;
+        for (uint32_t w = tid; w < TAB_WORDS; w += WB) {
+            const uint32_t v = s_tab[w];
+            if (v != tab_init_word(w)) tab_merge(g, w, v);
+            s_tab[w] = tab_init_word(w);
+        }
+        __syncthreads();
+        held = INVALID;
+    };
+    for (uint32_t t = t0; t < t1; t++) {
+        const uint32_t base = t * WB, pos = base + tid;
+        const uint32_t first = own[base], last = own[min(base + WB - 1, T - 1)];
+        const bool uni = first == last;
+        if (held != INVALID && !(uni && first == held)) flush();
+        if (uni && a.range[(size_t)RANGE_WORDS * first] - first > WT_BIG) held = first;
+        if (pos < T) {
+            const uint32_t lo = own[pos];
+            const uint32_t* R = a.range + (size_t)RANGE_WORDS * lo;
+            const uint32_t hi = R[0];
+            if (hi - lo > WT_BIG) {
+                const WtFrame f = wt_frame(R);
+                uint32_t* tab = uni ? s_tab : a.bins + (size_t)(lo >> WT_BIG_SHIFT) * TAB_WORDS;
+                tab_add(tab, ld_item(item, pos), f, pos < lo + (hi - lo) / 2);
+            }
+        }
+    }
+    if (held != INVALID) flush();
+}
+
+__device__ __forceinline__ void bins_union(const uint32_t* tab, int axis, int k0, int k1, uint32_t (&u)[BIN_WORDS]) {
+#pragma unroll
+    for (uint32_t j = 0; j < BIN_WORDS; j++) u[j] = tab_init_word(j);
+    for (int k = k0; k <= k1; k++) {
+        const uint32_t* b = tab + (axis * NBIN + k) * BIN_WORDS;
+#pragma unroll
+        for (uint32_t j = 0; j < BIN_WORDS; j++) {
+            const uint32_t v = b[j];
+            u[j] = j == 12 ? u[j] + v : (j == 13 || (j % 6) >= 3) ? max(u[j], v) : min(u[j], v);
+        }
+    }
+}
+__device__ __forceinline__ double key_area(const uint32_t (&k)[6]) {
+    const double dx = (double)kfloat(k[3]) - kfloat(k[0]), dy = (double)kfloat(k[4]) - kfloat(k[1]),
+                 dz = (double)kfloat(k[5]) - kfloat(k[2]);
+    return dx < 0 ? 0.0 : dx * dy + dy * dz + dz * dx;
+}
+
+__global__ __launch_bounds__(WB) void k_wt_pick(WalkTreeArgs a, uint32_t level) {
+    const uint32_t n_act = a.ctl[WT_NACT + level];
+    if (n_act == 0) return;
+    __shared__ uint32_t s_tab[WB / 64][TAB_WORDS];
+    const uint32_t wv = threadIdx.x >> 6, lane = threadIdx.x & 63u, cur = level & 1;
+    uint32_t* tab = s_tab[wv];
+    const float4* item = a.item[cur];
+    const uint32_t cap_act = a.T / 2 + 1;
+    for (uint32_t k = blockIdx.x * (WB / 64) + wv; k < n_act; k += gridDim.x * (WB / 64)) {
+        const uint32_t lo = a.act[cur][k];
+        uint32_t R[RANGE_WORDS];
+#pragma unroll
+        for (uint32_t j = 0; j < RANGE_WORDS; j++) R[j] = a.range[(size_t)RANGE_WORDS * lo + j];
+        const uint32_t hi = R[0], link = R[1], n = hi - lo, half = lo + n / 2;
+        const WtFrame f = wt_frame(R);
+        if (n > WT_BIG) {
+            uint32_t* g = a.bins + (size_t)(lo >> WT_BIG_SHIFT) * TAB_WORDS;
+            for (uint32_t w = lane; w < TAB_WORDS; w += 64) {
+                tab[w] = g[w];
+                g[w] = tab_init_word(w);
+            }
+        } else {
+            for (uint32_t w = lane; w < TAB_WORDS; w += 64) tab[w] = tab_init_word(w);
+            wave_sync();
+            for (uint32_t i = lo + lane; i < hi; i += 64) tab_add(tab, ld_item(item, i), f, i < half);
+        }
+        wave_sync();
+        double bc = __builtin_inf();
+        int bk = -1;
+        if (lane < 3 && !f.halves && f.sc[lane] > 0.f) {
+            const uint32_t* ax = tab + lane * NBIN * BIN_WORDS;
+            double ra[NBIN];
+            uint32_t rcnt[NBIN];
+            uint32_t acc[6] = {KEY_PINF, KEY_PINF, KEY_PINF, KEY_NINF, KEY_NINF, KEY_NINF};
+            uint32_t rc = 0;
+            for (int b = NBIN - 1; b > 0; b--) {
+                const uint32_t* w = ax + b * BIN_WORDS;
+                for (int q = 0; q < 3; q++) { acc[q] = min(acc[q], w[q]); acc[3 + q] = max(acc[3 + q], w[3 + q]); }
+                rc += w[12];
+                ra[b] = key_area(acc);
+                rcnt[b] = rc;
+            }
+            uint32_t lacc[6] = {KEY_PINF, KEY_PINF, KEY_PINF, KEY_NINF, KEY_NINF, KEY_NINF};
+            uint32_t lc = 0;
+            for (int b = 0; b < (int)NBIN - 1; b++) {
+                const uint32_t* w = ax + b * BIN_WORDS;
+                for (int q = 0; q < 3; q++) { lacc[q] = min(lacc[q], w[q]); lacc[3 + q] = max(lacc[3 + q], w[3 + q]); }
+                lc += w[12];
+                if (lc == 0 || rcnt[b + 1] == 0) continue;
+                const double c = key_area(lacc) * (double)lc + ra[b + 1] * (double)rcnt[b + 1];
+                if (c < bc) { bc = c; bk = b; }
+            }
+        }
+        int ba = -1, bb = 0;
+        double best = __builtin_inf();
+        for (int x = 0; x < 3; x++) {
+            const double cx = __shfl(bc, x);
+            const int kx = __shfl(bk, x);
+            if (kx >= 0 && cx < best) { best = cx; ba = x; bb = kx; }
+        }
+        const bool halves = ba < 0, keep = halves && !f.halves;
+        uint32_t u[BIN_WORDS];
+        if (lane < 2) {
+            if (halves) bins_union(tab, 0, (int)lane, (int)lane, u);
+            else if (lane == 0) bins_union(tab, ba, 0, bb, u);
+            else bins_union(tab, ba, bb + 1, NBIN - 1, u);
+        }
+        const uint32_t nl = __shfl(u[12], 0);
+        const uint32_t mid = halves ? half : lo + nl;
+        const uint32_t id = mid - 1;
+        if (lane < 2 && mid > lo && mid < hi) {
+            const uint32_t clo = lane ? mid : lo, chi = lane ? hi : mid;
+            uint32_t* C = a.range + (size_t)RANGE_WORDS * clo;
+            C[0] = chi;
+            C[1] = id << 1 | lane;
+            C[2] = keep ? R[2] : u[13];
+            C[3] = 0u;
+#pragma unroll
+            for (uint32_t j = 0; j < 12; j++) C[4 + j] = keep ? R[4 + j] : u[j];
+            if (chi - clo >= 2) {
+                const uint32_t slot = atomicAdd(a.ctl + WT_NACT + level + 1, 1u);
+                if (slot < cap_act) a.act[cur ^ 1][slot] = clo;
+            }
+        }
+        if (lane == 0 && mid > lo && mid < hi) {
+            a.wtopo[id] = make_uint4(INVALID, INVALID, link, R[2]);
+            if (link != INVALID) reinterpret_cast<uint32_t*>(a.wtopo + (link >> 1))[link & 1u] = id;
+            else a.ctl[WT_ROOT] = id;
+            float* bx = a.wbox + 6 * (size_t)id;
+#pragma unroll
+            for (int q = 0; q < 6; q++) bx[q] = kfloat(R[4 + q]);
+            const uint32_t ax = halves ? AXIS_HALVES : (uint32_t)ba;
+            a.dec[lo] = make_uint4(mid, level << 16 | (uint32_t)bb << 8 | ax, __float_as_uint(halves ? 0.f : f.cl[ba]),
+                                   __float_as_uint(halves ? 0.f : f.sc[ba]));
+        }
+        wave_sync();
+    }
+}
+
+__device__ __forceinline__ bool wt_decision(const WalkTreeArgs& a, uint32_t level, uint32_t lo, uint4& d) {
+    d = a.dec[lo];
+    return (d.y >> 16) == level;
+}
+__global__ __launch_bounds__(WB) void k_wt_flag(WalkTreeArgs a, uint32_t level) {
+    if (a.ctl[WT_NACT + level] == 0) return;
+    const uint32_t pos = blockIdx.x * WB + threadIdx.x;
+    if (pos >= a.T) return;
+    uint4 d;
+    bool left = false;
+    if (wt_decision(a, level, a.own[level & 1][pos], d)) {
+        const uint32_t ax = d.y & 0xFFu, bb = (d.y >> 8) & 0xFFu;
+        if (ax == AXIS_HALVES) {
+            left = pos < d.x;
+        } else {
+            const WtItem it = ld_item(a.item[level & 1], pos);
+            const float c = ax == 0 ? centroid(it, 0) : ax == 1 ? centroid(it, 1) : centroid(it, 2);
+            left = (uint32_t)wt_bin(c, __uint_as_float(d.z), __uint_as_float(d.w)) <= bb;
+        }
+    }
+    a.flags[pos + 1] = left ? 1ull : 0ull;
+}
+__global__ __launch_bounds__(WB) void k_wt_scatter(WalkTreeArgs a, uint32_t level) {
+    if (a.ctl[WT_NACT + level] == 0) return;
+    const uint32_t pos = blockIdx.x * WB + threadIdx.x, cur = level & 1;
+    if (pos >= a.T) return;
+    const uint32_t lo = a.own[cur][pos];
+    const WtItem it = ld_item(a.item[cur], pos);
+    uint4 d;
+    if (!wt_decision(a, level, lo, d)) {
+        st_item(a.item[cur ^ 1], pos, it);
+        a.own[cur ^ 1][pos] = lo;
+        return;
+    }
+    const uint32_t mid = d.x;
+    const uint32_t before = (uint32_t)(a.flags[pos] - a.flags[lo]);
+    const bool left = a.flags[pos + 1] != a.flags[pos];
+    const uint32_t to = left ? lo + before : mid + (pos - lo - before);
+    const uint32_t clo = left ? lo : mid;
+    if (to >= a.T) return;
+    st_item(a.item[cur ^ 1], to, it);
+    a.own[cur ^ 1][to] = clo;
+    if (a.range[(size_t)RANGE_WORDS * clo] - clo == 1)
+        reinterpret_cast<uint32_t*>(a.wtopo + (mid - 1))[left ? 0 : 1] = LEAF_BIT | it.id;
+}
+
+__global__ void k_wt_verdict(WalkTreeArgs a) {
+    uint32_t depth = 0;
+    while (depth < a.maxdepth && a.ctl[WT_NACT + depth] != 0) ++depth;
+    a.ctl[WT_DEPTH] = depth;
+    a.ctl[WT_STATE] = a.ctl[WT_NACT + a.maxdepth] != 0 ? 2u : 1u;
+}
+__global__ __launch_bounds__(WB) void k_wt_perm(WalkTreeArgs a) {
+    const uint32_t pos = blockIdx.x * WB + threadIdx.x;
+    if (pos < a.T) a.wperm[pos] = ld_item(a.item[a.ctl[WT_DEPTH] & 1], pos).id;
+}
+
+inline uint32_t blocks_for(size_t n) { return (uint32_t)((n + WB - 1) / WB); }
+
+}
+
+uint32_t walk_tree_tables(uint32_t T) { return (T >> WT_BIG_SHIFT) + 1; }
+size_t walk_tree_table_words(uint32_t T) { return (size_t)walk_tree_tables(T) * TAB_WORDS; }
+
+void launch_walk_tree(const WalkTreeArgs& a, hipStream_t s) {
+    if (a.T < 2) return;
+    const uint32_t tables = walk_tree_tables(a.T);
+    const uint32_t per_leaf = blocks_for(a.T);
+    const size_t reset = std::max<size_t>(std::max<size_t>(a.T, (size_t)tables * TAB_WORDS), WT_CTL_WORDS);
+    hipLaunchKernelGGL(k_wt_reset, dim3(blocks_for(reset)), dim3(WB), 0, s, a, tables);
+    hipLaunchKernelGGL(k_wt_leaves, dim3(std::min(per_leaf, 1024u)), dim3(WB), 0, s, a);
+    for (uint32_t level = 0; level < a.maxdepth; level++) {
+        if (a.T > WT_BIG) hipLaunchKernelGGL(k_wt_bin, dim3(std::min(per_leaf, 1024u)), dim3(WB), 0, s, a, level);
+        hipLaunchKernelGGL(k_wt_pick, dim3(std::min((a.T / 2 + 4) / 4, 2048u)), dim3(WB), 0, s, a, level);
+        hipLaunchKernelGGL(k_wt_flag, dim3(per_leaf), dim3(WB), 0, s, a, level);
+        scan_offsets(a.flags, a.T, a.sums, s);
+        hipLaunchKernelGGL(k_wt_scatter, dim3(per_leaf), dim3(WB), 0, s, a, level);
+    }
+    hipLaunchKernelGGL(k_wt_verdict, dim3(1), dim3(1), 0, s, a);
+    hipLaunchKernelGGL(k_wt_perm, dim3(per_leaf), dim3(WB), 0, s, a);
+}
+
+}
diff --git a/raytracebvh_amd/graphics.py b/raytracebvh_amd/graphics.py
--- a/raytracebvh_amd/graphics.py
+++ b/raytracebvh_amd/graphics.py
@@ -1012,6 +1012,15 @@
         self._check(_L.lib().rtbvh_read_qnodes(self._h, _L.ptr(out), len(out)))
         return out
 
+    def read_walk_tree(self) -> dict:
+        n = self.num_tris
+        out = {"children": np.zeros((n - 1, 2), np.uint32), "boxes": np.zeros((n - 1, 6), np.float32),
+               "parents": np.zeros(n - 1, np.uint32), "perm": np.zeros(n, np.uint32),
+               "qnodes": np.zeros((2 * n - 1, 16), np.uint32)}
+        self._check(_L.lib().rtbvh_read_walk_tree(self._h, _L.ptr(out["children"]), _L.ptr(out["boxes"]),
+                                                  _L.ptr(out["parents"]), _L.ptr(out["perm"]), _L.ptr(out["qnodes"])))
+        return out
+
     def read_morton(self) -> np.ndarray:
         out = np.zeros(self.num_tris, np.uint32)
         self._check(_L.lib().rtbvh_read_morton(self._h, _L.ptr(out)))
```

Measured after the change: 5127 Mrays/s. -1.8%, worse.
